# zkonduit/ezkl

Hardware: AMD Instinct MI355X
Metric: BN254 G1 MSM pts/s (2^20 points per GPU; NTT 2^22 elems/s in extra) (higher is better)
Workload: dtype u32x8 (254-bit modular integer, Montgomery); 1 GPU; configs[1]: standalone 2^20-point BN254 G1 MSM (uniform scalars, try-and-increment bases) + 2^22 scalar-field NTT per GPU; parallelism=points sharded across 1 rank(s); all_gather of 64-B partials + host fold

## Files before the change

### ezkl_amd/csrc/curve29.hpp

```cpp
#pragma once
#include "curve.hpp"
#include "field29.hpp"

namespace ezkl {

struct alignas(16) g1x29_t {
    f29_t x, y, zz, zzz;
};
struct g1a29_t {
    f29_t x, y;
};

EZ_D bool g1x29_is_id(const g1x29_t& p) { return Fq29::limbs_zero(p.zz); }
EZ_D g1x29_t g1x29_identity() {
    g1x29_t r;
    r.x = Fq29::zero(); r.y = Fq29::zero(); r.zz = Fq29::zero(); r.zzz = Fq29::zero();
    return r;
}
EZ_D g1a29_t g1a29_unpack(const g1a_t& p) {
    g1a29_t r;
    r.x = Fq29::unpack(p.x);
    r.y = Fq29::unpack(p.y);
    return r;
}
EZ_D bool g1a29_is_id(const g1a29_t& p) {
    uint32_t o = 0;
#pragma unroll
    for (int i = 0; i < 9; i++) o |= p.x.v[i] | p.y.v[i];
    return o == 0;
}

EZ_D g1x29_t g1x29_add_tail(const f29_t& u1, const f29_t& s1, const f29_t& p, const f29_t& r, const f29_t& zz, const f29_t& zzz) {
    g1x29_t o;
    const f29_t pp = Fq29::sqr(p);
    o.zz = Fq29::mul(zz, pp);
    const f29_t ppp = Fq29::mul(p, pp);
    o.zzz = Fq29::mul(zzz, ppp);
    const f29_t q = Fq29::mul(u1, pp);
#if !EZKL_FUSED_Y
    const f29_t e = Fq29::mul(s1, ppp);
#endif
    const f29_t rr = Fq29::sqr(r);
    const f29_t nq = Fq29::neg<1>(q);
    o.x = Fq29::normalize(Fq29::add(Fq29::add(rr, Fq29::neg<1>(ppp)), Fq29::add(nq, nq)));
    const f29_t d = Fq29::sub<3>(q, o.x);
#if EZKL_FUSED_Y
    o.y = Fq29::mul2add(r, d, Fq29::neg<3>(s1), ppp);
#else
    const f29_t rd = Fq29::mul(r, d);
    o.y = Fq29::normalize(Fq29::sub<1>(rd, e));
#endif
    return o;
}
EZ_D g1x29_t g1x29_double_affine(const g1a29_t& p) {
    const f29_t u = Fq29::add(p.y, p.y);
    const f29_t v = Fq29::sqr_cold(u);
    const f29_t w = Fq29::mul_cold(u, v);
    const f29_t s = Fq29::mul_cold(p.x, v);
    const f29_t xx = Fq29::sqr_cold(p.x);
    const f29_t m = Fq29::normalize(Fq29::add(Fq29::add(xx, xx), xx));
    const f29_t ns = Fq29::neg<1>(s);
    g1x29_t r;
    r.x = Fq29::normalize(Fq29::add(Fq29::sqr_cold(m), Fq29::add(ns, ns)));
    const f29_t d = Fq29::sub<3>(s, r.x);
    r.y = Fq29::normalize(Fq29::sub<1>(Fq29::mul_cold(m, d), Fq29::mul_cold(w, p.y)));
    r.zz = v;
    r.zzz = w;
    return r;
}
EZ_D g1x29_t g1x29_double(const g1x29_t& p) {
    if (g1x29_is_id(p)) return p;
    const f29_t u = Fq29::add(p.y, p.y);
    const f29_t v = Fq29::sqr_cold(u);
    const f29_t w = Fq29::mul_cold(u, v);
    const f29_t s = Fq29::mul_cold(p.x, v);
    const f29_t xx = Fq29::sqr_cold(p.x);
    const f29_t m = Fq29::normalize(Fq29::add(Fq29::add(xx, xx), xx));
    const f29_t ns = Fq29::neg<1>(s);
    g1x29_t r;
    r.x = Fq29::normalize(Fq29::add(Fq29::sqr_cold(m), Fq29::add(ns, ns)));
    const f29_t d = Fq29::sub<3>(s, r.x);
    r.y = Fq29::normalize(Fq29::sub<1>(Fq29::mul_cold(m, d), Fq29::mul_cold(w, p.y)));
    r.zz = Fq29::mul_cold(v, p.zz);
    r.zzz = Fq29::mul_cold(w, p.zzz);
    return r;
}
EZ_D g1x29_t g1x29_add_mixed(const g1x29_t& a, const g1a29_t& q, bool negate) {
    if (g1a29_is_id(q)) return a;
    const f29_t qy = negate ? Fq29::neg<0>(q.y) : q.y;
    if (g1x29_is_id(a)) {
        g1x29_t r;
        r.x = q.x;
        r.y = negate ? Fq29::normalize(qy) : q.y;
        r.zz = Fq29::one();
        r.zzz = Fq29::one();
        return r;
    }
    const f29_t u2 = Fq29::mul(q.x, a.zz);
    const f29_t s2 = Fq29::mul(qy, a.zzz);
    const f29_t p = Fq29::normalize(Fq29::sub<3>(u2, a.x));
    const f29_t r = Fq29::normalize(Fq29::sub<3>(s2, a.y));
    if (Fq29::is_zero_mod_p(p)) {
        if (Fq29::is_zero_mod_p(r)) {
            g1a29_t qq = q;
            if (negate) qq.y = Fq29::normalize(qy);
            return g1x29_double_affine(qq);
        }
        return g1x29_identity();
    }
    return g1x29_add_tail(a.x, a.y, p, r, a.zz, a.zzz);
}
EZ_D g1x29_t g1x29_add(const g1x29_t& a, const g1x29_t& b) {
    if (g1x29_is_id(a)) return b;
    if (g1x29_is_id(b)) return a;
    const f29_t u1 = Fq29::mul(a.x, b.zz), u2 = Fq29::mul(b.x, a.zz);
    const f29_t s1 = Fq29::mul(a.y, b.zzz), s2 = Fq29::mul(b.y, a.zzz);
    const f29_t p = Fq29::normalize(Fq29::sub<1>(u2, u1));
    const f29_t r = Fq29::normalize(Fq29::sub<1>(s2, s1));
    if (Fq29::is_zero_mod_p(p)) {
        if (Fq29::is_zero_mod_p(r)) return g1x29_double(a);
        return g1x29_identity();
    }
    return g1x29_add_tail(u1, s1, p, r, Fq29::mul(a.zz, b.zz), Fq29::mul(a.zzz, b.zzz));
}

EZ_D g1x29_t ld_g1x29(const g1x29_t* p) {
    g1x29_t r;
    const uint4* s = reinterpret_cast<const uint4*>(p);
    uint32_t* d = r.x.v;
#pragma unroll
    for (int k = 0; k < 9; k++) {
        const uint4 t = s[k];
        d[4 * k] = t.x; d[4 * k + 1] = t.y; d[4 * k + 2] = t.z; d[4 * k + 3] = t.w;
    }
    return r;
}
EZ_D void st_g1x29(g1x29_t* p, const g1x29_t& v) {
    uint4* d = reinterpret_cast<uint4*>(p);
    const uint32_t* s = v.x.v;
#pragma unroll
    for (int k = 0; k < 9; k++) d[k] = make_uint4(s[4 * k], s[4 * k + 1], s[4 * k + 2], s[4 * k + 3]);
}
EZ_D g1x29_t g1x29_shfl_xor(const g1x29_t& p, uint32_t mask) {
    g1x29_t r;
    const uint32_t* s = p.x.v;
    uint32_t* d = r.x.v;
#pragma unroll
    for (int k = 0; k < 36; k++) d[k] = __shfl_xor(s[k], mask);
    return r;
}
EZ_D g1x29_t g1x29_group_sum(g1x29_t acc, uint32_t width) {
#pragma unroll 1
    for (uint32_t s = width >> 1; s > 0; s >>= 1) acc = g1x29_add(acc, g1x29_shfl_xor(acc, s));
    return acc;
}

template <int S>
EZ_D f29_t f29_quad_bcast(const f29_t& x) {
    f29_t t = x, r;
    asm volatile("s_nop 1" : "+v"(t.v[0]), "+v"(t.v[1]), "+v"(t.v[2]), "+v"(t.v[3]), "+v"(t.v[4]), "+v"(t.v[5]), "+v"(t.v[6]), "+v"(t.v[7]), "+v"(t.v[8]));
#pragma unroll
    for (int i = 0; i < 9; i++) {
        r.v[i] = (uint32_t)__builtin_amdgcn_mov_dpp((int)t.v[i], S * 0x55, 0xf, 0xf, true);
        asm volatile("" : "+v"(r.v[i]));
    }
    return r;
}
EZ_D f29_t f29_sel(bool c, const f29_t& a, const f29_t& b) {
    f29_t r;
#pragma unroll
    for (int i = 0; i < 9; i++) r.v[i] = c ? a.v[i] : b.v[i];
    return r;
}
EZ_D f29_t f29_sel4(uint32_t q, const f29_t& x0, const f29_t& x1, const f29_t& x2, const f29_t& x3) {
    return f29_sel(q < 2, f29_sel(q == 0, x0, x1), f29_sel(q == 2, x2, x3));
}
template <int S>
EZ_D g1x29_t g1x29_quad_bcast(const g1x29_t& p) {
    g1x29_t r;
    r.x = f29_quad_bcast<S>(p.x); r.y = f29_quad_bcast<S>(p.y); r.zz = f29_quad_bcast<S>(p.zz); r.zzz = f29_quad_bcast<S>(p.zzz);
    return r;
}
EZ_D g1x29_t g1x29_add_quad(const g1x29_t& a, const g1x29_t& b, bool& special, uint32_t* dbg = nullptr) {
    const uint32_t q = threadIdx.x & 3u;
    g1x29_t o = a;
    special = __any(g1x29_is_id(a) || g1x29_is_id(b)) != 0;
    if (special) return o;
    const f29_t m1 = Fq29::mul(f29_sel4(q, a.x, b.x, a.y, b.y), f29_sel4(q, b.zz, a.zz, b.zzz, a.zzz));
    const f29_t u1 = f29_quad_bcast<0>(m1), s1 = f29_quad_bcast<2>(m1);
    const f29_t p = Fq29::normalize(Fq29::sub<1>(f29_quad_bcast<1>(m1), u1));
    const f29_t r = Fq29::normalize(Fq29::sub<1>(f29_quad_bcast<3>(m1), s1));
    special = __any(Fq29::is_zero_mod_p(p)) != 0;
    if (special) return o;
    const f29_t m2 = Fq29::mul(f29_sel4(q, a.zz, a.zzz, p, r), f29_sel4(q, b.zz, b.zzz, p, r));
    const f29_t pp = f29_quad_bcast<2>(m2), rr = f29_quad_bcast<3>(m2);
    const f29_t m3 = Fq29::mul(f29_sel(q == 1, p, f29_sel(q == 2, u1, m2)), pp);
    const f29_t ppp = f29_quad_bcast<1>(m3), qq = f29_quad_bcast<2>(m3);
    const f29_t nq = Fq29::neg<1>(qq);
    o.x = Fq29::normalize(Fq29::add(Fq29::add(rr, Fq29::neg<1>(ppp)), Fq29::add(nq, nq)));
    const f29_t d = Fq29::sub<3>(qq, o.x);
    const f29_t m4 = Fq29::mul(f29_sel(q == 2, r, f29_sel(q == 3, s1, m2)), f29_sel(q == 2, d, ppp));
    o.zz = f29_quad_bcast<0>(m3);
    o.zzz = f29_quad_bcast<1>(m4);
    o.y = Fq29::normalize(Fq29::sub<1>(f29_quad_bcast<2>(m4), f29_quad_bcast<3>(m4)));
    if (dbg) {
        const f29_t* t[14] = {&m1, &u1, &s1, &p, &r, &m2, &pp, &rr, &m3, &ppp, &qq, &o.x, &d, &m4};
        for (int k = 0; k < 14; k++)
            for (int i = 0; i < 9; i++) dbg[9 * k + i] = t[k]->v[i];
    }
    return o;
}
EZ_D g1x29_t g1x29_group_sum_coop(g1x29_t acc, uint32_t width) {
    const uint32_t nsteps = 3u + (31u - (uint32_t)__clz(width)) - 2u;
    g1x29_t t0 = acc;
#pragma unroll 1
    for (uint32_t k = 0; k < nsteps; k++) {
        g1x29_t a, b;
        if (k == 0) { a = g1x29_quad_bcast<0>(acc); b = g1x29_quad_bcast<1>(acc); }
        else if (k == 1) { a = g1x29_quad_bcast<2>(acc); b = g1x29_quad_bcast<3>(acc); }
        else if (k == 2) { a = t0; b = acc; }
        else { a = acc; b = g1x29_shfl_xor(acc, 4u << (k - 3u)); }
        bool special;
        g1x29_t r = g1x29_add_quad(a, b, special);
        if (special) r = g1x29_add(a, b);
        if (k == 0) t0 = r; else acc = r;
    }
    return acc;
}
EZ_D g1x29_t g1x29_block256_sum(g1x29_t acc, uint4* sh) {
    acc = g1x29_group_sum(acc, 64);
    if ((threadIdx.x & 63) == 0) {
        const uint32_t* s = acc.x.v;
#pragma unroll
        for (int k = 0; k < 9; k++) sh[k * 4 + (threadIdx.x >> 6)] = make_uint4(s[4 * k], s[4 * k + 1], s[4 * k + 2], s[4 * k + 3]);
    }
    __syncthreads();
    {
        uint32_t* d = acc.x.v;
#pragma unroll
        for (int k = 0; k < 9; k++) {
            const uint4 t = sh[k * 4 + (threadIdx.x & 3)];
            d[4 * k] = t.x; d[4 * k + 1] = t.y; d[4 * k + 2] = t.z; d[4 * k + 3] = t.w;
        }
    }
    __syncthreads();
    return g1x29_group_sum(acc, 4);
}
EZ_D g1x29_t g1x29_block256_sum_coop(const g1x29_t& acc0, uint4* sh) {
    g1x29_t acc = g1x29_group_sum_coop(acc0, 64);
    if ((threadIdx.x & 63) == 0) {
        const uint32_t* s = acc.x.v;
#pragma unroll
        for (int k = 0; k < 9; k++) sh[k * 4 + (threadIdx.x >> 6)] = make_uint4(s[4 * k], s[4 * k + 1], s[4 * k + 2], s[4 * k + 3]);
    }
    __syncthreads();
    {
        uint32_t* d = acc.x.v;
#pragma unroll
        for (int k = 0; k < 9; k++) {
            const uint4 t = sh[k * 4 + (threadIdx.x & 3)];
            d[4 * k] = t.x; d[4 * k + 1] = t.y; d[4 * k + 2] = t.z; d[4 * k + 3] = t.w;
        }
    }
// ... 27 lines not shown
```

### ezkl_amd/csrc/field29.hpp

```cpp
#pragma once
#include "field.hpp"
#include "montmul29_gen.hpp"

#ifndef EZKL_FQ29_ILP
#define EZKL_FQ29_ILP 0
#endif
#ifndef EZKL_FUSED_Y
#define EZKL_FUSED_Y 1
#endif
namespace ezkl {

struct f29_t {
    uint32_t v[9];
};
static constexpr uint32_t M29 = (1u << 29) - 1;

template <class CT, bool IS_FQ>
struct Field29 {
    typedef CT C;
    typedef uint32_t u32x9 __attribute__((ext_vector_type(9)));
    EZ_D static void mul_asm(const uint32_t (&a)[9], const uint32_t (&b)[9], uint32_t (&r)[9]) {
        if (IS_FQ) {
#if EZKL_FQ29_ILP
            mont_mul29i_fq(a, b, r);
#else
            mont_mul29_fq(a, b, r);
#endif
        } else mont_mul29_fr(a, b, r);
    }

    EZ_D static f29_t zero() {
        f29_t r;
#pragma unroll
        for (int i = 0; i < 9; i++) r.v[i] = 0;
        return r;
    }
    EZ_D static f29_t one() {
        f29_t r;
#pragma unroll
        for (int i = 0; i < 9; i++) r.v[i] = C::ONE[i];
        return r;
    }
    EZ_D static bool limbs_zero(const f29_t& a) {
        uint32_t o = 0;
#pragma unroll
        for (int i = 0; i < 9; i++) o |= a.v[i];
        return o == 0;
    }
    __device__ __attribute__((noinline)) static u32x9 mul_call(u32x9 a, u32x9 b) {
        uint32_t x[9], y[9], r[9];
#pragma unroll
        for (int i = 0; i < 9; i++) { x[i] = a[i]; y[i] = b[i]; }
        mul_asm(x, y, r);
        u32x9 o;
#pragma unroll
        for (int i = 0; i < 9; i++) o[i] = r[i];
        return o;
    }
    EZ_D static f29_t mul(const f29_t& a, const f29_t& b) {
        f29_t r;
        mul_asm(a.v, b.v, r.v);
        return r;
    }
    EZ_D static f29_t mul2add(const f29_t& a, const f29_t& b, const f29_t& c, const f29_t& d) {
        static_assert(IS_FQ, "generated for Fq only");
        f29_t r;
        mont_mul2add29_fq(a.v, b.v, c.v, d.v, r.v);
        return r;
    }
    EZ_D static f29_t mul_cold(const f29_t& a, const f29_t& b) {
        u32x9 x, y;
#pragma unroll
        for (int i = 0; i < 9; i++) { x[i] = a.v[i]; y[i] = b.v[i]; }
        u32x9 o = mul_call(x, y);
        f29_t r;
#pragma unroll
        for (int i = 0; i < 9; i++) r.v[i] = o[i];
        return r;
    }
    EZ_D static f29_t sqr(const f29_t& a) {
        f29_t r;
        if (IS_FQ) {
#if EZKL_FQ29_ILP
            mont_sqr29i_fq(a.v, r.v);
#else
            mont_sqr29_fq(a.v, r.v);
#endif
        } else mont_sqr29_fr(a.v, r.v);
        return r;
    }
    EZ_D static f29_t sqr_cold(const f29_t& a) { return mul_cold(a, a); }
    EZ_D static f29_t add(const f29_t& a, const f29_t& b) {
        f29_t r;
#pragma unroll
        for (int i = 0; i < 9; i++) r.v[i] = a.v[i] + b.v[i];
        return r;
    }
    template <int KI>
    EZ_D static f29_t sub(const f29_t& a, const f29_t& b) {
        f29_t r;
#pragma unroll
        for (int i = 0; i < 9; i++) r.v[i] = a.v[i] + (C::SUBC[KI][i] - b.v[i]);
        return r;
    }
    template <int KI>
    EZ_D static f29_t neg(const f29_t& b) {
        f29_t r;
#pragma unroll
        for (int i = 0; i < 9; i++) r.v[i] = C::SUBC[KI][i] - b.v[i];
        return r;
    }
    EZ_D static f29_t normalize(const f29_t& a) {
        f29_t r = a;
#pragma unroll
        for (int i = 0; i < 8; i++) {
            r.v[i + 1] += r.v[i] >> 29;
            r.v[i] &= M29;
        }
        return r;
    }
    EZ_D static bool is_zero_mod_p(const f29_t& a) {
        const uint32_t j = (a.v[0] * C::P0INV) & M29;
        if (j >= 32) return false;
        uint32_t carry = 0, diff = 0;
#pragma unroll
        for (int i = 0; i < 9; i++) {
            const uint64_t t = (uint64_t)j * C::P[i] + carry;
            const uint32_t limb = i < 8 ? ((uint32_t)t & M29) : (uint32_t)t;
            carry = i < 8 ? (uint32_t)(t >> 29) : 0;
            diff |= limb ^ a.v[i];
        }
        return diff == 0;
    }
    template <int KI>
    EZ_D static f29_t cond_sub(const f29_t& x) {
        f29_t t;
#pragma unroll
        for (int i = 0; i < 9; i++) t.v[i] = x.v[i] + C::CSUB[KI][i];
        t = normalize(t);
        const bool ge = (t.v[8] >> 29) != 0;
        t.v[8] &= M29;
        f29_t r;
#pragma unroll
        for (int i = 0; i < 9; i++) r.v[i] = ge ? t.v[i] : x.v[i];
        return r;
    }
    EZ_D static f29_t canonical(const f29_t& x) {
        constexpr uint32_t D = (uint32_t)(C::P[8] + 1u);
        constexpr uint64_t MAGIC = (((uint64_t)1 << 51) + D - 1) / D;
        const uint32_t q = (uint32_t)(((uint64_t)x.v[8] * MAGIC) >> 51);
        f29_t r;
        uint64_t acc = 0;
#pragma unroll
        for (int i = 0; i < 9; i++) {
            acc += (uint64_t)q * C::CSUB[0][i] + x.v[i];
            r.v[i] = (uint32_t)acc & M29;
            acc >>= 29;
        }
        return cond_sub<0>(r);
    }
    EZ_D static fe_t pack(const f29_t& a) {
        fe_t w;
#pragma unroll
        for (int j = 0; j < 8; j++) {
            const int bit = 32 * j, lo = bit / 29, sh = bit - 29 * lo;
            uint32_t acc = a.v[lo] >> sh;
            const int have = 29 - sh;
            if (lo + 1 < 9) acc |= a.v[lo + 1] << have;
            if (have + 29 < 32 && lo + 2 < 9) acc |= a.v[lo + 2] << (have + 29);
            w.v[j] = acc;
        }
        return w;
    }
    EZ_D static f29_t unpack(const fe_t& w) {
        f29_t r;
#pragma unroll
        for (int i = 0; i < 8; i++) {
            const int bit = 29 * i, word = bit >> 5, sh = bit & 31;
            const uint32_t lo = w.v[word], hi = word + 1 < 8 ? w.v[word + 1] : 0u;
            r.v[i] = (sh ? __builtin_amdgcn_alignbit(hi, lo, sh) : lo) & M29;
        }
        r.v[8] = w.v[7] >> 8;
        return r;
    }
};

typedef Field29<Fq29C, true> Fq29;
typedef Field29<Fr29C, false> Fr29;

EZ_D f29_t ld_f29(const f29_t* p) {
    f29_t r;
#pragma unroll
    for (int i = 0; i < 9; i++) r.v[i] = p->v[i];
    return r;
}
EZ_D void st_f29(f29_t* p, const f29_t& a) {
#pragma unroll
    for (int i = 0; i < 9; i++) p->v[i] = a.v[i];
}

}
```

### ezkl_amd/csrc/montmul29_gen.hpp

```cpp
#pragma once
#ifndef __HIPCC_RTC__
#include <stdint.h>
#endif
namespace ezkl {
struct Fq29C {
    static constexpr uint32_t P[9] = {0x187cfd47u, 0x010460b6u, 0x1c72a34fu, 0x02d522d0u, 0x1585d978u, 0x02db40c0u, 0x00a6e141u, 0x0e5c2634u, 0x0030644eu};
    static constexpr uint32_t ONE[9] = {0x157ccc21u, 0x141c2758u, 0x185230d3u, 0x014c0419u, 0x0aa36fb9u, 0x1d4240ceu, 0x11d54c07u, 0x052ac7a8u, 0x000dc836u};
    static constexpr uint32_t P0INV = 0x1b799c77u;
    static constexpr uint32_t SUBC[7][9] = {
        {0x30f9fa8eu, 0x2208c16cu, 0x38e5469du, 0x25aa45a0u, 0x2b0bb2efu, 0x25b68180u, 0x214dc281u, 0x3cb84c67u, 0x0060c89bu},
        {0x21f3f51cu, 0x241182dau, 0x31ca8d3bu, 0x2b548b42u, 0x361765dfu, 0x2b6d0301u, 0x229b8503u, 0x397098cfu, 0x00c19138u},
        {0x23e7ea38u, 0x282305b5u, 0x23951a77u, 0x36a91686u, 0x2c2ecbbfu, 0x36da0604u, 0x25370a07u, 0x32e1319fu, 0x01832272u},
        {0x27cfd470u, 0x30460b6bu, 0x272a34efu, 0x2d522d0du, 0x385d9780u, 0x2db40c09u, 0x2a6e1410u, 0x25c2633fu, 0x030644e6u},
        {0x2f9fa8e0u, 0x208c16d7u, 0x2e5469e0u, 0x3aa45a1bu, 0x30bb2f01u, 0x3b681814u, 0x34dc2821u, 0x2b84c67fu, 0x060c89cdu},
        {0x3f3f51c0u, 0x21182dafu, 0x3ca8d3c1u, 0x3548b437u, 0x21765e04u, 0x36d0302au, 0x29b85044u, 0x37098d00u, 0x0c19139bu},
        {0x3e7ea380u, 0x22305b60u, 0x3951a783u, 0x2a916870u, 0x22ecbc0au, 0x2da06055u, 0x3370a08au, 0x2e131a01u, 0x18322738u},
    };
    static constexpr uint32_t CSUB[4][9] = {
        {0x078302b9u, 0x1efb9f49u, 0x038d5cb0u, 0x1d2add2fu, 0x0a7a2687u, 0x1d24bf3fu, 0x1f591ebeu, 0x11a3d9cbu, 0x1fcf9bb1u},
        {0x0f060572u, 0x1df73e92u, 0x071ab961u, 0x1a55ba5eu, 0x14f44d0fu, 0x1a497e7eu, 0x1eb23d7du, 0x0347b397u, 0x1f9f3763u},
        {0x1e0c0ae4u, 0x1bee7d24u, 0x0e3572c3u, 0x14ab74bcu, 0x09e89a1fu, 0x1492fcfdu, 0x1d647afbu, 0x068f672fu, 0x1f3e6ec6u},
        {0x1c1815c8u, 0x17dcfa49u, 0x1c6ae587u, 0x0956e978u, 0x13d1343fu, 0x0925f9fau, 0x1ac8f5f7u, 0x0d1ece5fu, 0x1e7cdd8cu},
    };
    static constexpr uint32_t R261_32[8] = {0x157ccc21u, 0x4e8384ebu, 0x0ce148c3u, 0xfb90a602u, 0x819caa36u, 0x5301fa84u, 0x563d4475u, 0x0dc83629u};
};
struct Fr29C {
    static constexpr uint32_t P[9] = {0x10000001u, 0x1f0fac9fu, 0x0e5c2450u, 0x07d090f3u, 0x1585d283u, 0x02db40c0u, 0x00a6e141u, 0x0e5c2634u, 0x0030644eu};
    static constexpr uint32_t ONE[9] = {0x0fffff57u, 0x1ea70ab4u, 0x052c068bu, 0x17504f49u, 0x0aa8075bu, 0x1d4240ceu, 0x11d54c07u, 0x052ac7a8u, 0x000dc836u};
    static constexpr uint32_t P0INV = 0x10000001u;
    static constexpr uint32_t SUBC[7][9] = {
        {0x20000002u, 0x3e1f593eu, 0x3cb848a0u, 0x2fa121e5u, 0x2b0ba505u, 0x25b68180u, 0x214dc281u, 0x3cb84c67u, 0x0060c89bu},
        {0x20000004u, 0x3c3eb27du, 0x39709142u, 0x3f4243ccu, 0x36174a0bu, 0x2b6d0301u, 0x229b8503u, 0x397098cfu, 0x00c19138u},
        {0x20000008u, 0x387d64fbu, 0x32e12286u, 0x3e84879au, 0x2c2e9418u, 0x36da0604u, 0x25370a07u, 0x32e1319fu, 0x01832272u},
        {0x20000010u, 0x30fac9f7u, 0x25c2450eu, 0x3d090f36u, 0x385d2832u, 0x2db40c09u, 0x2a6e1410u, 0x25c2633fu, 0x030644e6u},
        {0x20000020u, 0x21f593efu, 0x2b848a1eu, 0x3a121e6du, 0x30ba5066u, 0x3b681814u, 0x34dc2821u, 0x2b84c67fu, 0x060c89cdu},
        {0x20000040u, 0x23eb27dfu, 0x3709143du, 0x34243cdbu, 0x2174a0ceu, 0x36d0302au, 0x29b85044u, 0x37098d00u, 0x0c19139bu},
        {0x20000080u, 0x27d64fbfu, 0x2e12287bu, 0x284879b8u, 0x22e9419eu, 0x2da06055u, 0x3370a08au, 0x2e131a01u, 0x18322738u},
    };
    static constexpr uint32_t CSUB[4][9] = {
        {0x0fffffffu, 0x00f05360u, 0x11a3dbafu, 0x182f6f0cu, 0x0a7a2d7cu, 0x1d24bf3fu, 0x1f591ebeu, 0x11a3d9cbu, 0x1fcf9bb1u},
        {0x1ffffffeu, 0x01e0a6c0u, 0x0347b75eu, 0x105ede19u, 0x14f45af9u, 0x1a497e7eu, 0x1eb23d7du, 0x0347b397u, 0x1f9f3763u},
        {0x1ffffffcu, 0x03c14d81u, 0x068f6ebcu, 0x00bdbc32u, 0x09e8b5f3u, 0x1492fcfdu, 0x1d647afbu, 0x068f672fu, 0x1f3e6ec6u},
        {0x1ffffff8u, 0x07829b03u, 0x0d1edd78u, 0x017b7864u, 0x13d16be6u, 0x0925f9fau, 0x1ac8f5f7u, 0x0d1ece5fu, 0x1e7cdd8cu},
    };
    static constexpr uint32_t R261_32[8] = {0x8fffff57u, 0x2fd4e156u, 0xa494b01au, 0x75bba827u, 0x819caa80u, 0x5301fa84u, 0x563d4475u, 0x0dc83629u};
};
__device__ __forceinline__ void mont_mul29_fq(const uint32_t (&a)[9], const uint32_t (&b)[9], uint32_t (&r)[9]) {
    asm("s_mov_b32 s16, 0x187cfd47\n\t"
        "s_mov_b32 s17, 0x010460b6\n\t"
        "s_mov_b32 s18, 0x1c72a34f\n\t"
        "s_mov_b32 s19, 0x02d522d0\n\t"
        "s_mov_b32 s20, 0x1585d978\n\t"
        "s_mov_b32 s21, 0x02db40c0\n\t"
        "s_mov_b32 s22, 0x00a6e141\n\t"
        "s_mov_b32 s23, 0x0e5c2634\n\t"
        "s_mov_b32 s24, 0x0030644e\n\t"
        "s_mov_b32 s25, 0x04866389\n\t"
        "s_mov_b32 s26, 0x1fffffff\n\t"
        "v_mad_u64_u32 v[16:17], vcc, %[a0], %[b0], 0\n\t"
        "v_mul_lo_u32 %[r0], v16, s25\n\t"
        "v_and_b32 %[r0], s26, %[r0]\n\t"
        "v_mad_u64_u32 v[16:17], vcc, %[r0], s16, v[16:17]\n\t"
        "v_lshrrev_b64 v[16:17], 29, v[16:17]\n\t"
        "v_mad_u64_u32 v[16:17], vcc, %[a0], %[b1], v[16:17]\n\t"
        "v_mad_u64_u32 v[16:17], vcc, %[a1], %[b0], v[16:17]\n\t"
        "v_mad_u64_u32 v[16:17], vcc, %[r0], s17, v[16:17]\n\t"
        "v_mul_lo_u32 %[r1], v16, s25\n\t"
        "v_and_b32 %[r1], s26, %[r1]\n\t"
        "v_mad_u64_u32 v[16:17], vcc, %[r1], s16, v[16:17]\n\t"
        "v_lshrrev_b64 v[16:17], 29, v[16:17]\n\t"
        "v_mad_u64_u32 v[16:17], vcc, %[a0], %[b2], v[16:17]\n\t"
        "v_mad_u64_u32 v[16:17], vcc, %[a1], %[b1], v[16:17]\n\t"
        "v_mad_u64_u32 v[16:17], vcc, %[a2], %[b0], v[16:17]\n\t"
        "v_mad_u64_u32 v[16:17], vcc, %[r0], s18, v[16:17]\n\t"
        "v_mad_u64_u32 v[16:17], vcc, %[r1], s17, v[16:17]\n\t"
        "v_mul_lo_u32 %[r2], v16, s25\n\t"
        "v_and_b32 %[r2], s26, %[r2]\n\t"
        "v_mad_u64_u32 v[16:17], vcc, %[r2], s16, v[16:17]\n\t"
        "v_lshrrev_b64 v[16:17], 29, v[16:17]\n\t"
        "v_mad_u64_u32 v[16:17], vcc, %[a0], %[b3], v[16:17]\n\t"
        "v_mad_u64_u32 v[16:17], vcc, %[a1], %[b2], v[16:17]\n\t"
        "v_mad_u64_u32 v[16:17], vcc, %[a2], %[b1], v[16:17]\n\t"
        "v_mad_u64_u32 v[16:17], vcc, %[a3], %[b0], v[16:17]\n\t"
        "v_mad_u64_u32 v[16:17], vcc, %[r0], s19, v[16:17]\n\t"
        "v_mad_u64_u32 v[16:17], vcc, %[r1], s18, v[16:17]\n\t"
        "v_mad_u64_u32 v[16:17], vcc, %[r2], s17, v[16:17]\n\t"
        "v_mul_lo_u32 %[r3], v16, s25\n\t"
        "v_and_b32 %[r3], s26, %[r3]\n\t"
        "v_mad_u64_u32 v[16:17], vcc, %[r3], s16, v[16:17]\n\t"
        "v_lshrrev_b64 v[16:17], 29, v[16:17]\n\t"
        "v_mad_u64_u32 v[16:17], vcc, %[a0], %[b4], v[16:17]\n\t"
        "v_mad_u64_u32 v[16:17], vcc, %[a1], %[b3], v[16:17]\n\t"
        "v_mad_u64_u32 v[16:17], vcc, %[a2], %[b2], v[16:17]\n\t"
        "v_mad_u64_u32 v[16:17], vcc, %[a3], %[b1], v[16:17]\n\t"
        "v_mad_u64_u32 v[16:17], vcc, %[a4], %[b0], v[16:17]\n\t"
        "v_mad_u64_u32 v[16:17], vcc, %[r0], s20, v[16:17]\n\t"
        "v_mad_u64_u32 v[16:17], vcc, %[r1], s19, v[16:17]\n\t"
        "v_mad_u64_u32 v[16:17], vcc, %[r2], s18, v[16:17]\n\t"
        "v_mad_u64_u32 v[16:17], vcc, %[r3], s17, v[16:17]\n\t"
        "v_mul_lo_u32 %[r4], v16, s25\n\t"
        "v_and_b32 %[r4], s26, %[r4]\n\t"
        "v_mad_u64_u32 v[16:17], vcc, %[r4], s16, v[16:17]\n\t"
        "v_lshrrev_b64 v[16:17], 29, v[16:17]\n\t"
        "v_mad_u64_u32 v[16:17], vcc, %[a0], %[b5], v[16:17]\n\t"
        "v_mad_u64_u32 v[16:17], vcc, %[a1], %[b4], v[16:17]\n\t"
        "v_mad_u64_u32 v[16:17], vcc, %[a2], %[b3], v[16:17]\n\t"
        "v_mad_u64_u32 v[16:17], vcc, %[a3], %[b2], v[16:17]\n\t"
        "v_mad_u64_u32 v[16:17], vcc, %[a4], %[b1], v[16:17]\n\t"
        "v_mad_u64_u32 v[16:17], vcc, %[a5], %[b0], v[16:17]\n\t"
        "v_mad_u64_u32 v[16:17], vcc, %[r0], s21, v[16:17]\n\t"
        "v_mad_u64_u32 v[16:17], vcc, %[r1], s20, v[16:17]\n\t"
        "v_mad_u64_u32 v[16:17], vcc, %[r2], s19, v[16:17]\n\t"
        "v_mad_u64_u32 v[16:17], vcc, %[r3], s18, v[16:17]\n\t"
        "v_mad_u64_u32 v[16:17], vcc, %[r4], s17, v[16:17]\n\t"
        "v_mul_lo_u32 %[r5], v16, s25\n\t"
        "v_and_b32 %[r5], s26, %[r5]\n\t"
        "v_mad_u64_u32 v[16:17], vcc, %[r5], s16, v[16:17]\n\t"
        "v_lshrrev_b64 v[16:17], 29, v[16:17]\n\t"
        "v_mad_u64_u32 v[16:17], vcc, %[a0], %[b6], v[16:17]\n\t"
        "v_mad_u64_u32 v[16:17], vcc, %[a1], %[b5], v[16:17]\n\t"
        "v_mad_u64_u32 v[16:17], vcc, %[a2], %[b4], v[16:17]\n\t"
        "v_mad_u64_u32 v[16:17], vcc, %[a3], %[b3], v[16:17]\n\t"
        "v_mad_u64_u32 v[16:17], vcc, %[a4], %[b2], v[16:17]\n\t"
        "v_mad_u64_u32 v[16:17], vcc, %[a5], %[b1], v[16:17]\n\t"
        "v_mad_u64_u32 v[16:17], vcc, %[a6], %[b0], v[16:17]\n\t"
        "v_mad_u64_u32 v[16:17], vcc, %[r0], s22, v[16:17]\n\t"
        "v_mad_u64_u32 v[16:17], vcc, %[r1], s21, v[16:17]\n\t"
        "v_mad_u64_u32 v[16:17], vcc, %[r2], s20, v[16:17]\n\t"
        "v_mad_u64_u32 v[16:17], vcc, %[r3], s19, v[16:17]\n\t"
        "v_mad_u64_u32 v[16:17], vcc, %[r4], s18, v[16:17]\n\t"
        "v_mad_u64_u32 v[16:17], vcc, %[r5], s17, v[16:17]\n\t"
        "v_mul_lo_u32 %[r6], v16, s25\n\t"
        "v_and_b32 %[r6], s26, %[r6]\n\t"
        "v_mad_u64_u32 v[16:17], vcc, %[r6], s16, v[16:17]\n\t"
        "v_lshrrev_b64 v[16:17], 29, v[16:17]\n\t"
        "v_mad_u64_u32 v[16:17], vcc, %[a0], %[b7], v[16:17]\n\t"
        "v_mad_u64_u32 v[16:17], vcc, %[a1], %[b6], v[16:17]\n\t"
        "v_mad_u64_u32 v[16:17], vcc, %[a2], %[b5], v[16:17]\n\t"
        "v_mad_u64_u32 v[16:17], vcc, %[a3], %[b4], v[16:17]\n\t"
        "v_mad_u64_u32 v[16:17], vcc, %[a4], %[b3], v[16:17]\n\t"
        "v_mad_u64_u32 v[16:17], vcc, %[a5], %[b2], v[16:17]\n\t"
        "v_mad_u64_u32 v[16:17], vcc, %[a6], %[b1], v[16:17]\n\t"
        "v_mad_u64_u32 v[16:17], vcc, %[a7], %[b0], v[16:17]\n\t"
        "v_mad_u64_u32 v[16:17], vcc, %[r0], s23, v[16:17]\n\t"
        "v_mad_u64_u32 v[16:17], vcc, %[r1], s22, v[16:17]\n\t"
        "v_mad_u64_u32 v[16:17], vcc, %[r2], s21, v[16:17]\n\t"
        "v_mad_u64_u32 v[16:17], vcc, %[r3], s20, v[16:17]\n\t"
        "v_mad_u64_u32 v[16:17], vcc, %[r4], s19, v[16:17]\n\t"
        "v_mad_u64_u32 v[16:17], vcc, %[r5], s18, v[16:17]\n\t"
        "v_mad_u64_u32 v[16:17], vcc, %[r6], s17, v[16:17]\n\t"
        "v_mul_lo_u32 %[r7], v16, s25\n\t"
        "v_and_b32 %[r7], s26, %[r7]\n\t"
        "v_mad_u64_u32 v[16:17], vcc, %[r7], s16, v[16:17]\n\t"
        "v_lshrrev_b64 v[16:17], 29, v[16:17]\n\t"
        "v_mad_u64_u32 v[16:17], vcc, %[a0], %[b8], v[16:17]\n\t"
        "v_mad_u64_u32 v[16:17], vcc, %[a1], %[b7], v[16:17]\n\t"
        "v_mad_u64_u32 v[16:17], vcc, %[a2], %[b6], v[16:17]\n\t"
        "v_mad_u64_u32 v[16:17], vcc, %[a3], %[b5], v[16:17]\n\t"
        "v_mad_u64_u32 v[16:17], vcc, %[a4], %[b4], v[16:17]\n\t"
        "v_mad_u64_u32 v[16:17], vcc, %[a5], %[b3], v[16:17]\n\t"
        "v_mad_u64_u32 v[16:17], vcc, %[a6], %[b2], v[16:17]\n\t"
        "v_mad_u64_u32 v[16:17], vcc, %[a7], %[b1], v[16:17]\n\t"
        "v_mad_u64_u32 v[16:17], vcc, %[a8], %[b0], v[16:17]\n\t"
        "v_mad_u64_u32 v[16:17], vcc, %[r0], s24, v[16:17]\n\t"
        "v_mad_u64_u32 v[16:17], vcc, %[r1], s23, v[16:17]\n\t"
        "v_mad_u64_u32 v[16:17], vcc, %[r2], s22, v[16:17]\n\t"
        "v_mad_u64_u32 v[16:17], vcc, %[r3], s21, v[16:17]\n\t"
        "v_mad_u64_u32 v[16:17], vcc, %[r4], s20, v[16:17]\n\t"
        "v_mad_u64_u32 v[16:17], vcc, %[r5], s19, v[16:17]\n\t"
        "v_mad_u64_u32 v[16:17], vcc, %[r6], s18, v[16:17]\n\t"
        "v_mad_u64_u32 v[16:17], vcc, %[r7], s17, v[16:17]\n\t"
        "v_mul_lo_u32 %[r8], v16, s25\n\t"
        "v_and_b32 %[r8], s26, %[r8]\n\t"
        "v_mad_u64_u32 v[16:17], vcc, %[r8], s16, v[16:17]\n\t"
        "v_lshrrev_b64 v[16:17], 29, v[16:17]\n\t"
        "v_mad_u64_u32 v[16:17], vcc, %[a1], %[b8], v[16:17]\n\t"
        "v_mad_u64_u32 v[16:17], vcc, %[a2], %[b7], v[16:17]\n\t"
        "v_mad_u64_u32 v[16:17], vcc, %[a3], %[b6], v[16:17]\n\t"
        "v_mad_u64_u32 v[16:17], vcc, %[a4], %[b5], v[16:17]\n\t"
        "v_mad_u64_u32 v[16:17], vcc, %[a5], %[b4], v[16:17]\n\t"
        "v_mad_u64_u32 v[16:17], vcc, %[a6], %[b3], v[16:17]\n\t"
        "v_mad_u64_u32 v[16:17], vcc, %[a7], %[b2], v[16:17]\n\t"
        "v_mad_u64_u32 v[16:17], vcc, %[a8], %[b1], v[16:17]\n\t"
        "v_mad_u64_u32 v[16:17], vcc, %[r1], s24, v[16:17]\n\t"
        "v_mad_u64_u32 v[16:17], vcc, %[r2], s23, v[16:17]\n\t"
        "v_mad_u64_u32 v[16:17], vcc, %[r3], s22, v[16:17]\n\t"
        "v_mad_u64_u32 v[16:17], vcc, %[r4], s21, v[16:17]\n\t"
        "v_mad_u64_u32 v[16:17], vcc, %[r5], s20, v[16:17]\n\t"
        "v_mad_u64_u32 v[16:17], vcc, %[r6], s19, v[16:17]\n\t"
        "v_mad_u64_u32 v[16:17], vcc, %[r7], s18, v[16:17]\n\t"
        "v_mad_u64_u32 v[16:17], vcc, %[r8], s17, v[16:17]\n\t"
// ... 1532 lines not shown
        "v_mad_u64_u32 v[18:19], vcc, %[a0], %[b7], 0\n\t"
        "v_mad_u64_u32 v[16:17], vcc, %[r0], s22, v[16:17]\n\t"
        "v_mad_u64_u32 v[18:19], vcc, %[a1], %[b6], v[18:19]\n\t"
        "v_mad_u64_u32 v[16:17], vcc, %[r1], s21, v[16:17]\n\t"
        "v_mad_u64_u32 v[18:19], vcc, %[a2], %[b5], v[18:19]\n\t"
        "v_mad_u64_u32 v[16:17], vcc, %[r2], s20, v[16:17]\n\t"
        "v_mad_u64_u32 v[18:19], vcc, %[a3], %[b4], v[18:19]\n\t"
        "v_mad_u64_u32 v[16:17], vcc, %[r3], s19, v[16:17]\n\t"
        "v_mad_u64_u32 v[18:19], vcc, %[a4], %[b3], v[18:19]\n\t"
        "v_mad_u64_u32 v[16:17], vcc, %[r4], s18, v[16:17]\n\t"
        "v_mad_u64_u32 v[18:19], vcc, %[a5], %[b2], v[18:19]\n\t"
        "v_mad_u64_u32 v[16:17], vcc, %[r5], s17, v[16:17]\n\t"
        "v_mad_u64_u32 v[18:19], vcc, %[a6], %[b1], v[18:19]\n\t"
        "v_mul_lo_u32 %[r6], v16, s25\n\t"
        "v_mad_u64_u32 v[18:19], vcc, %[a7], %[b0], v[18:19]\n\t"
        "v_and_b32 %[r6], s26, %[r6]\n\t"
        "v_mad_u64_u32 v[16:17], vcc, %[r6], s16, v[16:17]\n\t"
        "v_lshrrev_b64 v[16:17], 29, v[16:17]\n\t"
        "v_lshl_add_u64 v[16:17], v[18:19], 0, v[16:17]\n\t"
        "v_mad_u64_u32 v[18:19], vcc, %[a0], %[b8], 0\n\t"
        "v_mad_u64_u32 v[16:17], vcc, %[r0], s23, v[16:17]\n\t"
        "v_mad_u64_u32 v[18:19], vcc, %[a1], %[b7], v[18:19]\n\t"
        "v_mad_u64_u32 v[16:17], vcc, %[r1], s22, v[16:17]\n\t"
        "v_mad_u64_u32 v[18:19], vcc, %[a2], %[b6], v[18:19]\n\t"
        "v_mad_u64_u32 v[16:17], vcc, %[r2], s21, v[16:17]\n\t"
        "v_mad_u64_u32 v[18:19], vcc, %[a3], %[b5], v[18:19]\n\t"
        "v_mad_u64_u32 v[16:17], vcc, %[r3], s20, v[16:17]\n\t"
        "v_mad_u64_u32 v[18:19], vcc, %[a4], %[b4], v[18:19]\n\t"
        "v_mad_u64_u32 v[16:17], vcc, %[r4], s19, v[16:17]\n\t"
        "v_mad_u64_u32 v[18:19], vcc, %[a5], %[b3], v[18:19]\n\t"
        "v_mad_u64_u32 v[16:17], vcc, %[r5], s18, v[16:17]\n\t"
        "v_mad_u64_u32 v[18:19], vcc, %[a6], %[b2], v[18:19]\n\t"
        "v_mad_u64_u32 v[16:17], vcc, %[r6], s17, v[16:17]\n\t"
        "v_mad_u64_u32 v[18:19], vcc, %[a7], %[b1], v[18:19]\n\t"
        "v_mul_lo_u32 %[r7], v16, s25\n\t"
        "v_mad_u64_u32 v[18:19], vcc, %[a8], %[b0], v[18:19]\n\t"
        "v_and_b32 %[r7], s26, %[r7]\n\t"
        "v_mad_u64_u32 v[16:17], vcc, %[r7], s16, v[16:17]\n\t"
        "v_lshrrev_b64 v[16:17], 29, v[16:17]\n\t"
        "v_lshl_add_u64 v[16:17], v[18:19], 0, v[16:17]\n\t"
        "v_mad_u64_u32 v[18:19], vcc, %[a1], %[b8], 0\n\t"
        "v_mad_u64_u32 v[16:17], vcc, %[r0], s24, v[16:17]\n\t"
        "v_mad_u64_u32 v[18:19], vcc, %[a2], %[b7], v[18:19]\n\t"
        "v_mad_u64_u32 v[16:17], vcc, %[r1], s23, v[16:17]\n\t"
        "v_mad_u64_u32 v[18:19], vcc, %[a3], %[b6], v[18:19]\n\t"
        "v_mad_u64_u32 v[16:17], vcc, %[r2], s22, v[16:17]\n\t"
        "v_mad_u64_u32 v[18:19], vcc, %[a4], %[b5], v[18:19]\n\t"
        "v_mad_u64_u32 v[16:17], vcc, %[r3], s21, v[16:17]\n\t"
        "v_mad_u64_u32 v[18:19], vcc, %[a5], %[b4], v[18:19]\n\t"
        "v_mad_u64_u32 v[16:17], vcc, %[r4], s20, v[16:17]\n\t"
        "v_mad_u64_u32 v[18:19], vcc, %[a6], %[b3], v[18:19]\n\t"
        "v_mad_u64_u32 v[16:17], vcc, %[r5], s19, v[16:17]\n\t"
        "v_mad_u64_u32 v[18:19], vcc, %[a7], %[b2], v[18:19]\n\t"
        "v_mad_u64_u32 v[16:17], vcc, %[r6], s18, v[16:17]\n\t"
        "v_mad_u64_u32 v[18:19], vcc, %[a8], %[b1], v[18:19]\n\t"
        "v_mad_u64_u32 v[16:17], vcc, %[r7], s17, v[16:17]\n\t"
        "v_mul_lo_u32 %[r8], v16, s25\n\t"
        "v_and_b32 %[r8], s26, %[r8]\n\t"
        "v_mad_u64_u32 v[16:17], vcc, %[r8], s16, v[16:17]\n\t"
        "v_lshrrev_b64 v[16:17], 29, v[16:17]\n\t"
        "v_lshl_add_u64 v[16:17], v[18:19], 0, v[16:17]\n\t"
        "v_mad_u64_u32 v[18:19], vcc, %[a2], %[b8], 0\n\t"
        "v_mad_u64_u32 v[16:17], vcc, %[r1], s24, v[16:17]\n\t"
        "v_mad_u64_u32 v[18:19], vcc, %[a3], %[b7], v[18:19]\n\t"
        "v_mad_u64_u32 v[16:17], vcc, %[r2], s23, v[16:17]\n\t"
        "v_mad_u64_u32 v[18:19], vcc, %[a4], %[b6], v[18:19]\n\t"
        "v_mad_u64_u32 v[16:17], vcc, %[r3], s22, v[16:17]\n\t"
        "v_mad_u64_u32 v[18:19], vcc, %[a5], %[b5], v[18:19]\n\t"
        "v_mad_u64_u32 v[16:17], vcc, %[r4], s21, v[16:17]\n\t"
        "v_mad_u64_u32 v[18:19], vcc, %[a6], %[b4], v[18:19]\n\t"
        "v_mad_u64_u32 v[16:17], vcc, %[r5], s20, v[16:17]\n\t"
        "v_mad_u64_u32 v[18:19], vcc, %[a7], %[b3], v[18:19]\n\t"
        "v_mad_u64_u32 v[16:17], vcc, %[r6], s19, v[16:17]\n\t"
        "v_mad_u64_u32 v[18:19], vcc, %[a8], %[b2], v[18:19]\n\t"
        "v_mad_u64_u32 v[16:17], vcc, %[r7], s18, v[16:17]\n\t"
        "v_mad_u64_u32 v[16:17], vcc, %[r8], s17, v[16:17]\n\t"
        "v_and_b32 %[r0], s26, v16\n\t"
        "v_lshrrev_b64 v[16:17], 29, v[16:17]\n\t"
        "v_lshl_add_u64 v[16:17], v[18:19], 0, v[16:17]\n\t"
        "v_mad_u64_u32 v[18:19], vcc, %[a3], %[b8], 0\n\t"
        "v_mad_u64_u32 v[16:17], vcc, %[r2], s24, v[16:17]\n\t"
        "v_mad_u64_u32 v[18:19], vcc, %[a4], %[b7], v[18:19]\n\t"
        "v_mad_u64_u32 v[16:17], vcc, %[r3], s23, v[16:17]\n\t"
        "v_mad_u64_u32 v[18:19], vcc, %[a5], %[b6], v[18:19]\n\t"
        "v_mad_u64_u32 v[16:17], vcc, %[r4], s22, v[16:17]\n\t"
        "v_mad_u64_u32 v[18:19], vcc, %[a6], %[b5], v[18:19]\n\t"
        "v_mad_u64_u32 v[16:17], vcc, %[r5], s21, v[16:17]\n\t"
        "v_mad_u64_u32 v[18:19], vcc, %[a7], %[b4], v[18:19]\n\t"
        "v_mad_u64_u32 v[16:17], vcc, %[r6], s20, v[16:17]\n\t"
        "v_mad_u64_u32 v[18:19], vcc, %[a8], %[b3], v[18:19]\n\t"
        "v_mad_u64_u32 v[16:17], vcc, %[r7], s19, v[16:17]\n\t"
        "v_mad_u64_u32 v[16:17], vcc, %[r8], s18, v[16:17]\n\t"
        "v_and_b32 %[r1], s26, v16\n\t"
        "v_lshrrev_b64 v[16:17], 29, v[16:17]\n\t"
        "v_lshl_add_u64 v[16:17], v[18:19], 0, v[16:17]\n\t"
        "v_mad_u64_u32 v[18:19], vcc, %[a4], %[b8], 0\n\t"
        "v_mad_u64_u32 v[16:17], vcc, %[r3], s24, v[16:17]\n\t"
        "v_mad_u64_u32 v[18:19], vcc, %[a5], %[b7], v[18:19]\n\t"
        "v_mad_u64_u32 v[16:17], vcc, %[r4], s23, v[16:17]\n\t"
        "v_mad_u64_u32 v[18:19], vcc, %[a6], %[b6], v[18:19]\n\t"
        "v_mad_u64_u32 v[16:17], vcc, %[r5], s22, v[16:17]\n\t"
        "v_mad_u64_u32 v[18:19], vcc, %[a7], %[b5], v[18:19]\n\t"
        "v_mad_u64_u32 v[16:17], vcc, %[r6], s21, v[16:17]\n\t"
        "v_mad_u64_u32 v[18:19], vcc, %[a8], %[b4], v[18:19]\n\t"
        "v_mad_u64_u32 v[16:17], vcc, %[r7], s20, v[16:17]\n\t"
        "v_mad_u64_u32 v[16:17], vcc, %[r8], s19, v[16:17]\n\t"
        "v_and_b32 %[r2], s26, v16\n\t"
        "v_lshrrev_b64 v[16:17], 29, v[16:17]\n\t"
        "v_lshl_add_u64 v[16:17], v[18:19], 0, v[16:17]\n\t"
        "v_mad_u64_u32 v[18:19], vcc, %[a5], %[b8], 0\n\t"
        "v_mad_u64_u32 v[16:17], vcc, %[r4], s24, v[16:17]\n\t"
        "v_mad_u64_u32 v[18:19], vcc, %[a6], %[b7], v[18:19]\n\t"
        "v_mad_u64_u32 v[16:17], vcc, %[r5], s23, v[16:17]\n\t"
        "v_mad_u64_u32 v[18:19], vcc, %[a7], %[b6], v[18:19]\n\t"
        "v_mad_u64_u32 v[16:17], vcc, %[r6], s22, v[16:17]\n\t"
        "v_mad_u64_u32 v[18:19], vcc, %[a8], %[b5], v[18:19]\n\t"
        "v_mad_u64_u32 v[16:17], vcc, %[r7], s21, v[16:17]\n\t"
        "v_mad_u64_u32 v[16:17], vcc, %[r8], s20, v[16:17]\n\t"
        "v_and_b32 %[r3], s26, v16\n\t"
        "v_lshrrev_b64 v[16:17], 29, v[16:17]\n\t"
        "v_lshl_add_u64 v[16:17], v[18:19], 0, v[16:17]\n\t"
        "v_mad_u64_u32 v[18:19], vcc, %[a6], %[b8], 0\n\t"
        "v_mad_u64_u32 v[16:17], vcc, %[r5], s24, v[16:17]\n\t"
        "v_mad_u64_u32 v[18:19], vcc, %[a7], %[b7], v[18:19]\n\t"
        "v_mad_u64_u32 v[16:17], vcc, %[r6], s23, v[16:17]\n\t"
        "v_mad_u64_u32 v[18:19], vcc, %[a8], %[b6], v[18:19]\n\t"
        "v_mad_u64_u32 v[16:17], vcc, %[r7], s22, v[16:17]\n\t"
        "v_mad_u64_u32 v[16:17], vcc, %[r8], s21, v[16:17]\n\t"
        "v_and_b32 %[r4], s26, v16\n\t"
        "v_lshrrev_b64 v[16:17], 29, v[16:17]\n\t"
        "v_lshl_add_u64 v[16:17], v[18:19], 0, v[16:17]\n\t"
        "v_mad_u64_u32 v[18:19], vcc, %[a7], %[b8], 0\n\t"
        "v_mad_u64_u32 v[16:17], vcc, %[r6], s24, v[16:17]\n\t"
        "v_mad_u64_u32 v[18:19], vcc, %[a8], %[b7], v[18:19]\n\t"
        "v_mad_u64_u32 v[16:17], vcc, %[r7], s23, v[16:17]\n\t"
        "v_mad_u64_u32 v[16:17], vcc, %[r8], s22, v[16:17]\n\t"
        "v_and_b32 %[r5], s26, v16\n\t"
        "v_lshrrev_b64 v[16:17], 29, v[16:17]\n\t"
        "v_lshl_add_u64 v[16:17], v[18:19], 0, v[16:17]\n\t"
        "v_mad_u64_u32 v[18:19], vcc, %[a8], %[b8], 0\n\t"
        "v_mad_u64_u32 v[16:17], vcc, %[r7], s24, v[16:17]\n\t"
        "v_mad_u64_u32 v[16:17], vcc, %[r8], s23, v[16:17]\n\t"
        "v_and_b32 %[r6], s26, v16\n\t"
        "v_lshrrev_b64 v[16:17], 29, v[16:17]\n\t"
        "v_lshl_add_u64 v[16:17], v[18:19], 0, v[16:17]\n\t"
        "v_mad_u64_u32 v[16:17], vcc, %[r8], s24, v[16:17]\n\t"
        "v_and_b32 %[r7], s26, v16\n\t"
        "v_lshrrev_b64 v[16:17], 29, v[16:17]\n\t"
        "v_mov_b32 %[r8], v16\n\t"
        : [r0] "=&v"(r[0]), [r1] "=&v"(r[1]), [r2] "=&v"(r[2]), [r3] "=&v"(r[3]), [r4] "=&v"(r[4]), [r5] "=&v"(r[5]), [r6] "=&v"(r[6]), [r7] "=&v"(r[7]), [r8] "=&v"(r[8])
        : [a0] "v"(a[0]), [a1] "v"(a[1]), [a2] "v"(a[2]), [a3] "v"(a[3]), [a4] "v"(a[4]), [a5] "v"(a[5]), [a6] "v"(a[6]), [a7] "v"(a[7]), [a8] "v"(a[8]), [b0] "v"(b[0]), [b1] "v"(b[1]), [b2] "v"(b[2]), [b3] "v"(b[3]), [b4] "v"(b[4]), [b5] "v"(b[5]), [b6] "v"(b[6]), [b7] "v"(b[7]), [b8] "v"(b[8])
        : "v16", "v17", "v18", "v19", "s16", "s17", "s18", "s19", "s20", "s21", "s22", "s23", "s24", "s25", "s26", "vcc");
}
}
```

### ezkl_amd/csrc/msm.hip

```cpp
#include "common.hpp"
#include <deque>
#include <thread>
#include <chrono>
#include "curve.hpp"
#include "curve29.hpp"
#include "host64.hpp"
#include <string.h>

namespace ezkl {

static constexpr uint32_t MSM_MAX_PART_BITS = 12;
static constexpr uint32_t MSM_SPAN_HEAVY = 16;
static constexpr uint32_t MSM_PART_STAGE = 13312;
static constexpr uint32_t MSM_BINSORT_STAGE = 15360;
static constexpr uint32_t MSM_HEAVY_CHUNK = 256;
static constexpr uint32_t MSM_DIGIT_E = 8;
static constexpr uint32_t MSM_LMIN = 8;
static constexpr uint32_t MSM_MAX_BIG = 64;
static constexpr uint32_t MSM_BIG_BLOCKS = 64;
static constexpr uint32_t MSM_BIG_ROWS = 8;

__device__ __forceinline__ uint32_t msm_part_of(uint32_t bucket, uint32_t NP) { return bucket ? 1u + (bucket & (NP - 1u)) : 0u; }
__device__ __forceinline__ uint32_t msm_lane_len(const uint32_t* offsets, uint32_t nb, uint32_t nlanes, uint32_t lmin) {
    const uint32_t l = (uint32_t)(((uint64_t)offsets[nb] + nlanes - 1) / nlanes);
// ... 387 lines not shown
    uint32_t total;
    uint32_t run = msm_block_scan(s, tsum, total) - s;
#pragma unroll
    for (int q = 0; q < 4; q++) {
        uint32_t j = t * 4 + q;
        if (j < nbins) {
            cnt[j] = run;
            if (emit) {
                const bool b0 = (p == 0 && j == 0);
                offsets[(size_t)p * nbins + j] = b0 ? part_base[0] : beg + run;
                if (b0 ? part_base[1] == part_base[0] : loc[q] == 0) st_f29(&buckets[(size_t)p * nbins + j].zz, Fq29::zero());
            }
        }
        run += loc[q];
    }
    __syncthreads();
}
__device__ __forceinline__ void msm_bigsort_count_body(const uint2* entries, const uint32_t* part_base, uint32_t LB, const uint32_t* big_list,
                                                       const uint32_t* big_count, uint32_t* bin_total, uint32_t* block_off, uint32_t* cnt, uint32_t bx,
                                                       uint32_t by, uint32_t rows);
__global__ __launch_bounds__(512) void msm_binsort_kernel(const uint2* entries, const uint32_t* part_base, uint32_t LB, uint32_t NP,
                                                          const uint32_t* big_flag, uint32_t* offsets, uint32_t* vals, g1x29_t* buckets,
                                                          const uint32_t* big_list, const uint32_t* big_count, uint32_t* bin_total, uint32_t* block_off,
                                                          size_t bstride) {
    BOFF(); BSH(entries); BSH(part_base); BSH(big_flag); BSH(offsets); BSH(vals); BSH(buckets);
    __shared__ uint32_t cnt[2048];
    __shared__ uint32_t tsum[512];
    extern __shared__ uint32_t stage[];
    if (blockIdx.x >= NP) {
        BSH(big_list); BSH(big_count); BSH(bin_total); BSH(block_off);
        const uint32_t w = blockIdx.x - NP;
        msm_bigsort_count_body(entries, part_base, LB, big_list, big_count, bin_total, block_off, cnt, w % MSM_BIG_BLOCKS, w / MSM_BIG_BLOCKS, MSM_BIG_ROWS);
        return;
    }
    const uint32_t p = blockIdx.x, t = threadIdx.x, nbins = 1u << LB;
    const uint32_t beg = part_base[p + 1], end = part_base[p + 2];
    if (p == NP - 1 && t == 0) offsets[(size_t)NP * nbins] = end;
    if (big_flag[p]) return;
    const bool staged = (end - beg) <= MSM_BINSORT_STAGE;
    for (uint32_t j = t; j < nbins; j += 512) cnt[j] = 0;
    __syncthreads();
    if (staged) {
        constexpr int PER = MSM_BINSORT_STAGE / 512;
        uint2 v[PER];
#pragma unroll
        for (int q = 0; q < PER; q++) {
            const uint32_t e = beg + t + (uint32_t)q * 512u;
            v[q] = e < end ? entries[e] : make_uint2(0u, 0xffffffffu);
        }
#pragma unroll
        for (int q = 0; q < PER; q++)
            if (v[q].y != 0xffffffffu) atomicAdd(&cnt[v[q].y], 1u);
        __syncthreads();
        msm_bins_scan(cnt, tsum, nbins, p, beg, part_base, true, offsets, buckets);
#pragma unroll
        for (int q = 0; q < PER; q++)
            if (v[q].y != 0xffffffffu) stage[atomicAdd(&cnt[v[q].y], 1u)] = v[q].x;
        __syncthreads();
        for (uint32_t i = t; i < end - beg; i += 512) vals[beg + i] = stage[i];
    } else {
        for (uint32_t e = beg + t; e < end; e += 512) (void)msm_wave_rank(cnt, entries[e].y);
        __syncthreads();
        msm_bins_scan(cnt, tsum, nbins, p, beg, part_base, true, offsets, buckets);
        for (uint32_t e = beg + t; e < end; e += 512) {
            const uint2 v = entries[e];
            vals[beg + msm_wave_rank(cnt, v.y)] = v.x;
        }
    }
}
__device__ __forceinline__ void msm_big_slice(uint32_t beg, uint32_t end, uint32_t& s0, uint32_t& s1, uint32_t bx) {
    const uint32_t chunk = (end - beg + MSM_BIG_BLOCKS - 1) / MSM_BIG_BLOCKS;
    s0 = beg + bx * chunk;
    s1 = s0 + chunk < end ? s0 + chunk : end;
    if (s0 > end) s0 = end;
}
__device__ __forceinline__ void msm_bigsort_count_body(const uint2* entries, const uint32_t* part_base, uint32_t LB, const uint32_t* big_list,
                                                       const uint32_t* big_count, uint32_t* bin_total, uint32_t* block_off, uint32_t* cnt, uint32_t bx,
                                                       uint32_t by, uint32_t rows) {
    const uint32_t t = threadIdx.x, nbins = 1u << LB;
    const uint32_t nbig = big_count[0] < MSM_MAX_BIG ? big_count[0] : MSM_MAX_BIG;
    for (uint32_t y = by; y < nbig; y += rows) {
        const uint32_t p = big_list[y];
        uint32_t s0, s1;
        msm_big_slice(part_base[p + 1], part_base[p + 2], s0, s1, bx);
        for (uint32_t j = t; j < nbins; j += 512) cnt[j] = 0;
        __syncthreads();
        for (uint32_t e = s0 + t; e < s1; e += 512) (void)msm_wave_rank(cnt, entries[e].y);
        __syncthreads();
        for (uint32_t j = t; j < nbins; j += 512)
            block_off[((size_t)y * MSM_BIG_BLOCKS + bx) * nbins + j] = cnt[j] ? atomicAdd(&bin_total[(size_t)y * nbins + j], cnt[j]) : 0u;
        __syncthreads();
    }
}
__global__ __launch_bounds__(512) void msm_bigsort_scatter_kernel(const uint2* entries, const uint32_t* part_base, uint32_t LB, const uint32_t* big_list,
                                                                  const uint32_t* big_count, const uint32_t* bin_total, const uint32_t* block_off,
                                                                  uint32_t* offsets, uint32_t* vals, g1x29_t* buckets, size_t bstride) {
    BOFF(); BSH(entries); BSH(part_base); BSH(big_list); BSH(big_count); BSH(bin_total); BSH(block_off); BSH(offsets); BSH(vals); BSH(buckets);
    __shared__ uint32_t cnt[2048];
    __shared__ uint32_t tsum[512];
    const uint32_t t = threadIdx.x, nbins = 1u << LB;
    const uint32_t nbig = big_count[0] < MSM_MAX_BIG ? big_count[0] : MSM_MAX_BIG;
    for (uint32_t y = blockIdx.y; y < nbig; y += gridDim.y) {
        const uint32_t p = big_list[y], beg = part_base[p + 1];
        uint32_t s0, s1;
        msm_big_slice(beg, part_base[p + 2], s0, s1, blockIdx.x);
        for (uint32_t j = t; j < nbins; j += 512) cnt[j] = bin_total[(size_t)y * nbins + j];
        __syncthreads();
        msm_bins_scan(cnt, tsum, nbins, p, beg, part_base, blockIdx.x == 0, offsets, buckets);
        const uint32_t* mine = block_off + ((size_t)y * MSM_BIG_BLOCKS + blockIdx.x) * nbins;
        for (uint32_t j = t; j < nbins; j += 512) cnt[j] += mine[j];
        __syncthreads();
        for (uint32_t e = s0 + t; e < s1; e += 512) {
            const uint2 v = entries[e];
            vals[beg + msm_wave_rank(cnt, v.y)] = v.x;
        }
        __syncthreads();
    }
}

struct MsmRec {
    g1a_t p;
    bool neg;
};
__device__ __forceinline__ MsmRec msm_fetch(const g1a_t* tab, uint32_t v) {
    MsmRec r;
    r.p = ld_g1a(tab + (v & 0x7fffffffu));
    r.neg = (v >> 31) != 0;
    return r;
}
__global__ __launch_bounds__(256, 3) void msm_accumulate_kernel(const g1a_t* tab, const uint32_t* offsets, const uint32_t* vals,
                                                             uint32_t nb, uint32_t nlanes, g1x29_t* buckets, g1x29_t* head, g1x29_t* tail,
                                                             uint32_t* lane_first, uint32_t lmin, size_t bstride) {
    BOFF(); BSH(offsets); BSH(vals); BSH(buckets); BSH(head); BSH(tail); BSH(lane_first);
    const uint32_t t = blockIdx.x * blockDim.x + threadIdx.x;
    const uint32_t total = offsets[nb], L = msm_lane_len(offsets, nb, nlanes, lmin);
    const uint64_t k0w = (uint64_t)t * L;
    if (k0w >= total) return;
    const uint32_t k0 = (uint32_t)k0w;
    const uint32_t k1 = (uint64_t)k0 + L < total ? k0 + L : total;
    uint32_t lo = 0, hi = nb;
    while (hi - lo > 1) {
        uint32_t mid = (lo + hi) >> 1;
        if (offsets[mid] <= k0) lo = mid; else hi = mid;
    }
    uint32_t b = lo, bin_end = offsets[b + 1];
    uint32_t end_next = offsets[b + 2 <= nb ? b + 2 : nb];
    lane_first[t] = b;
    bool started_before = offsets[b] < k0;
    g1x29_t acc = g1x29_identity();
    MsmRec nxt = msm_fetch(tab, vals[k0]);
    uint32_t vn = k0 + 1 < k1 ? vals[k0 + 1] : 0u;
    for (uint32_t k = k0; k < k1; k++) {
        if (k == bin_end) {
            if (started_before) st_g1x29(head + t, acc); else st_g1x29(buckets + b, acc);
            acc.zz = Fq29::zero();
            started_before = false;
            b++;
            bin_end = end_next;
            if (bin_end == k) {
                uint32_t probes = 1;
                while (bin_end == k && probes < 4) { b++; bin_end = offsets[b + 1]; probes++; }
                if (bin_end == k) {
                    uint32_t lo2 = b + 1, hi2 = nb;
                    while (hi2 - lo2 > 1) {
                        uint32_t mid = (lo2 + hi2) >> 1;
                        if (offsets[mid] <= k) lo2 = mid; else hi2 = mid;
                    }
                    b = lo2;
                    bin_end = offsets[b + 1];
                }
            }
            end_next = offsets[b + 2 <= nb ? b + 2 : nb];
        }
        const MsmRec cur = nxt;
        nxt = msm_fetch(tab, vn);
        vn = k + 2 < k1 ? vals[k + 2] : 0u;
        acc = g1x29_add_mixed(acc, g1a29_unpack(cur.p), cur.neg);
    }
    if (k1 == bin_end) {
        if (started_before) st_g1x29(head + t, acc); else st_g1x29(buckets + b, acc);
    } else {
        if (started_before) st_g1x29(head + t, acc); else st_g1x29(tail + t, acc);
    }
}
EZ_D g1x29_t g1x29_shfl_down(const g1x29_t& p, uint32_t d) {
    g1x29_t r;
    const uint32_t* s = p.x.v;
    uint32_t* o = r.x.v;
#pragma unroll
    for (int k = 0; k < 36; k++) o[k] = __shfl_down(s[k], d);
    return r;
}
__global__ __launch_bounds__(256) void msm_fixup_boundary_tree_kernel(const uint32_t* offsets, uint32_t nb, uint32_t nlanes,
                                                                      const uint32_t* lane_first, const g1x29_t* head, const g1x29_t* tail, g1x29_t* buckets,
                                                                      uint32_t* heavy_list, uint32_t* heavy_count, uint32_t* chunk_list, uint32_t lmin,
                                                                      uint32_t span_heavy, size_t bstride) {
    BOFF(); BSH(offsets); BSH(lane_first); BSH(head); BSH(tail); BSH(buckets); BSH(heavy_list); BSH(heavy_count); BSH(chunk_list);
    const uint32_t t = blockIdx.x * blockDim.x + threadIdx.x + 1;
    const uint32_t lane = threadIdx.x & 63u;
    const uint32_t L = msm_lane_len(offsets, nb, nlanes, lmin);
    const uint64_t k0 = (uint64_t)t * L;
    bool cut = t < nlanes && k0 < offsets[nb];
    uint32_t b = 0, t1 = 0, t2 = 0;
    if (cut) {
        b = lane_first[t];
        const uint32_t beg = offsets[b], end = offsets[b + 1];
        cut = beg < k0;
        t1 = beg / L; t2 = (end - 1) / L;
    }
    if (cut && t2 - t1 > span_heavy) {
        if (t == t1 + 1 && t2 - t1 > MSM_HEAVY_CHUNK) heavy_list[atomicAdd(heavy_count, 1u)] = b;
        if ((t - t1 - 1) % MSM_HEAVY_CHUNK == 0) chunk_list[atomicAdd(heavy_count + 1, 1u)] = t;
        cut = false;
    }
    const uint32_t wave_last = t + (63u - lane);
    const uint32_t run = cut ? (t2 < wave_last ? t2 : wave_last) - t + 1u : 0u;
    uint32_t longest = run;
#pragma unroll
    for (uint32_t o = 32; o > 0; o >>= 1) {
        const uint32_t m = __shfl_xor(longest, o);
        longest = m > longest ? m : longest;
    }
    if (longest == 0) return;
    if (longest <= 2) {
        if (!cut || t != t1 + 1) return;
        g1x29_t acc = g1x29_add(ld_g1x29(tail + t1), ld_g1x29(head + t));
        for (uint32_t u = t + 1; u <= t2; u++) acc = g1x29_add(acc, ld_g1x29(head + u));
        st_g1x29(buckets + b, acc);
        return;
    }
    g1x29_t v = cut ? ld_g1x29(head + t) : g1x29_identity();
    uint32_t have = cut ? 1u : 0u;
#pragma unroll 1
    for (uint32_t d = 1; d < longest; d <<= 1) {
        const g1x29_t w = g1x29_shfl_down(v, d);
        const uint32_t hw = __shfl_down(have, d);
        if (have == d && run > d) {
            v = g1x29_add(v, w);
            have += hw;
        }
    }
    if (!cut || t != t1 + 1) return;
    g1x29_t acc = g1x29_add(ld_g1x29(tail + t1), v);
    for (uint32_t u = t + run; u <= t2; u++) acc = g1x29_add(acc, ld_g1x29(head + u));
    st_g1x29(buckets + b, acc);
}
__global__ __launch_bounds__(256) void msm_fixup_heavy1_kernel(const uint32_t* offsets, uint32_t nb, uint32_t nlanes, const uint32_t* lane_first, g1x29_t* head,
                                                               const g1x29_t* tail, g1x29_t* buckets, const uint32_t* chunk_list, const uint32_t* counts, uint32_t lmin,
                                                               uint32_t coop, size_t bstride) {
    BOFF(); BSH(offsets); BSH(lane_first); BSH(head); BSH(tail); BSH(buckets); BSH(chunk_list); BSH(counts);
    const uint32_t nchunks = counts[1], L = msm_lane_len(offsets, nb, nlanes, lmin);
    const uint32_t wave = threadIdx.x >> 6, lane = threadIdx.x & 63u;
    for (uint32_t ci = blockIdx.x * 4u + wave; ci < nchunks; ci += gridDim.x * 4u) {
        const uint32_t start = chunk_list[ci], b = lane_first[start];
        const uint32_t t2 = (offsets[b + 1] - 1) / L;
        const uint32_t stop = start + MSM_HEAVY_CHUNK - 1 < t2 ? start + MSM_HEAVY_CHUNK - 1 : t2;
        const uint32_t t1 = offsets[b] / L;
        const bool whole = t2 - t1 <= MSM_HEAVY_CHUNK;
        g1x29_t acc = (whole && lane == 63u) ? ld_g1x29(tail + t1) : g1x29_identity();
        for (uint32_t t = start + lane; t <= stop; t += 64) acc = g1x29_add(acc, ld_g1x29(head + t));
        acc = coop ? g1x29_group_sum_coop(acc, 64) : g1x29_group_sum(acc, 64);
        if (lane == 0) st_g1x29(whole ? buckets + b : head + start, acc);
    }
}
__global__ __launch_bounds__(256) void msm_fixup_heavy2_kernel(const uint32_t* offsets, uint32_t nb, uint32_t nlanes, const g1x29_t* head, const g1x29_t* tail,
                                                               const uint32_t* heavy_list, const uint32_t* counts, g1x29_t* buckets, uint32_t lmin, uint32_t coop, size_t bstride) {
    BOFF(); BSH(offsets); BSH(head); BSH(tail); BSH(heavy_list); BSH(counts); BSH(buckets);
    const uint32_t L = msm_lane_len(offsets, nb, nlanes, lmin);
    const uint32_t wave = threadIdx.x >> 6, lane = threadIdx.x & 63u;
    for (uint32_t h = blockIdx.x * 4u + wave; h < counts[0]; h += gridDim.x * 4u) {
        const uint32_t b = heavy_list[h];
        const uint32_t t1 = offsets[b] / L, t2 = (offsets[b + 1] - 1) / L;
        g1x29_t acc = lane == 63u ? ld_g1x29(tail + t1) : g1x29_identity();
        for (uint32_t t = t1 + 1 + lane * MSM_HEAVY_CHUNK; t <= t2; t += 64 * MSM_HEAVY_CHUNK) acc = g1x29_add(acc, ld_g1x29(head + t));
        acc = coop ? g1x29_group_sum_coop(acc, 64) : g1x29_group_sum(acc, 64);
        if (lane == 0) st_g1x29(buckets + b, acc);
    }
}

struct ReduceGeom {
    uint32_t wA, wB, wC;
    uint32_t wsA, wsB, wsC;
    uint32_t EA, GA, ET, GT;
};
__global__ __launch_bounds__(256, 2) void msm_reduce1_kernel(const g1x29_t* buckets, ReduceGeom g, g1x29_t* partA, g1x29_t* partT, size_t bstride) {
    BOFF(); BSH(buckets); BSH(partA); BSH(partT);
    const uint32_t idx = blockIdx.x * blockDim.x + threadIdx.x;
    g1x29_t acc = g1x29_identity();
    if (blockIdx.y == 0) {
        if (idx >= (g.GA << g.wA)) return;
        const uint32_t dA = idx & ((1u << g.wA) - 1u), grp = idx >> g.wA;
        for (uint32_t e = 0; e < g.EA; e++) acc = g1x29_add(acc, ld_g1x29(buckets + ((((size_t)grp * g.EA + e) << g.wA) | dA)));
        st_g1x29(partA + (size_t)dA * g.GA + grp, acc);
    } else {
        const uint32_t nT = 1u << (g.wB + g.wC);
        if (idx >= nT * g.GT) return;
        const uint32_t grp = idx % g.GT, t = idx / g.GT;
        for (uint32_t e = 0; e < g.ET; e++) acc = g1x29_add(acc, ld_g1x29(buckets + (((size_t)t << g.wA) | (e * g.GT + grp))));
        st_g1x29(partT + (size_t)t * g.GT + grp, acc);
    }
}
__global__ __launch_bounds__(64) void msm_reduce2_kernel(const g1x29_t* partA, const g1x29_t* partT, ReduceGeom g, g1x29_t* SA, g1x29_t* T, uint32_t lanesA,
                                                         uint32_t lanesT, uint32_t blocksA, uint32_t coop, size_t bstride) {
    BOFF(); BSH(partA); BSH(partT); BSH(SA); BSH(T);
    const bool isA = blockIdx.x < blocksA;
    const uint32_t lanes = isA ? lanesA : lanesT, per = 64 / lanes;
    const uint32_t o = (isA ? blockIdx.x : blockIdx.x - blocksA) * per + threadIdx.x / lanes, j = threadIdx.x % lanes;
    const uint32_t nout = isA ? (1u << g.wA) : (1u << (g.wB + g.wC)), G = isA ? g.GA : g.GT;
    g1x29_t acc = g1x29_identity();
    if (o < nout) {
        const g1x29_t* src = (isA ? partA : partT) + (size_t)o * G;
        for (uint32_t i = j; i < G; i += lanes) acc = g1x29_add(acc, ld_g1x29(src + i));
    }
    acc = (coop && lanes >= 4) ? g1x29_group_sum_coop(acc, lanes) : g1x29_group_sum(acc, lanes);
    if (j == 0 && o < nout) st_g1x29((isA ? SA : T) + o, acc);
}
__global__ __launch_bounds__(256) void msm_planes_kernel(const g1x29_t* SA, const g1x29_t* T, ReduceGeom g, g1x29_t* planes, g1x29_t* planes_host, uint32_t coop,
                                                         size_t bstride) {
    BOFF(); BSH(SA); BSH(T); BSH(planes);
    __shared__ uint4 sh[9 * 4];
    uint32_t id = blockIdx.x, field = 0, j = 0;
    if (id > 0) {
        id -= 1;
        if (id < g.wA) { field = 1; j = id; }
        else if (id < g.wA + g.wB) { field = 2; j = id - g.wA; }
        else { field = 3; j = id - g.wA - g.wB; }
    }
    const uint32_t nA = 1u << g.wA, nT = 1u << (g.wB + g.wC);
    g1x29_t acc = g1x29_identity();
    auto with_bit = [](uint32_t k, uint32_t bit) { return ((k >> bit) << (bit + 1)) | (1u << bit) | (k & ((1u << bit) - 1u)); };
// ... 798 lines not shown
```

### ezkl_amd/csrc/ubench.hip

```cpp
#include "common.hpp"
#include "curve.hpp"
#include "montmul29_gen.hpp"
#include "curve29.hpp"
#include "host64.hpp"
#include <string.h>
#include <vector>
#include <stdlib.h>

namespace ezkl {

template <int VARIANT>
__global__ __launch_bounds__(256) void ub_modmul_kernel(fe_t* io, int iters) {
    size_t i = (size_t)blockIdx.x * blockDim.x + threadIdx.x;
    fe_t a = ld_fe(io + i), b = a, c = Fr::add(a, a), d = c;
    b.v[0] ^= 5;  b = Fr::reduce_once(b);
    for (int k = 0; k < iters; k++) {
        if (VARIANT == 0) { a = Fr::mul(a, b); c = Fr::mul(c, d); b = Fr::mul(b, a); d = Fr::mul(d, c); }
        else if (VARIANT == 1) { a = Fr::mul_portable(a, b); c = Fr::mul_portable(c, d); b = Fr::mul_portable(b, a); d = Fr::mul_portable(d, c); }
        else { a = Fr::mul_inl(a, b); c = Fr::mul_inl(c, d); b = Fr::mul_inl(b, a); d = Fr::mul_inl(d, c); }
    }
    st_fe(io + i, Fr::add(Fr::add(a, b), Fr::add(c, d)));
}
__global__ __launch_bounds__(256) void ub_waveinv_kernel(fe_t* io, int iters) {
    size_t i = (size_t)blockIdx.x * blockDim.x + threadIdx.x;
// ... 26 lines not shown
        for (int q = 0; q < 8; q++) { before.v[q] = __shfl_up(pre.v[q], 1); after.v[q] = __shfl_down(suf.v[q], 1); }
        fe_t r = inv;
        if (lane > 0) r = Fr::mul(r, before);
        if (lane < 63) r = Fr::mul(r, after);
        x = Fr::add(r, x);
        if (Fr::is_zero(x)) x = Fr::one();
    }
    st_fe(io + i, x);
}
__global__ __launch_bounds__(256) void ub_addsub_kernel(fe_t* io, int iters) {
    size_t i = (size_t)blockIdx.x * blockDim.x + threadIdx.x;
    fe_t a = ld_fe(io + i), b = Fr::reduce_once(a), c = Fr::add(b, b), d = c;
    for (int k = 0; k < iters; k++) { b = Fr::add(b, c); c = Fr::sub(c, d); d = Fr::add(d, b); c = Fr::sub(c, b); }
    st_fe(io + i, Fr::add(Fr::add(a, b), Fr::add(c, d)));
}
__global__ __launch_bounds__(256) void ub_mad64_kernel(uint64_t* io, int iters) {
    size_t i = (size_t)blockIdx.x * blockDim.x + threadIdx.x;
    uint64_t x = io[i];
    uint64_t a0 = x, a1 = x + 1, a2 = x + 2, a3 = x + 3, a4 = x + 4, a5 = x + 5, a6 = x + 6, a7 = x + 7;
    uint32_t m = (uint32_t)x | 1u, q = (uint32_t)(x >> 32) | 3u;
    for (int k = 0; k < iters; k++) {
        a0 = mad_wide(m, (uint32_t)a0, a0); a1 = mad_wide(q, (uint32_t)a1, a1);
        a2 = mad_wide(m, (uint32_t)a2, a2); a3 = mad_wide(q, (uint32_t)a3, a3);
        a4 = mad_wide(m, (uint32_t)a4, a4); a5 = mad_wide(q, (uint32_t)a5, a5);
        a6 = mad_wide(m, (uint32_t)a6, a6); a7 = mad_wide(q, (uint32_t)a7, a7);
    }
    io[i] = a0 ^ a1 ^ a2 ^ a3 ^ a4 ^ a5 ^ a6 ^ a7;
}
__global__ __launch_bounds__(256) void ub_mullo_kernel(uint64_t* io, int iters) {
    size_t i = (size_t)blockIdx.x * blockDim.x + threadIdx.x;
    uint32_t x = (uint32_t)io[i];
    uint32_t a0 = x, a1 = x + 1, a2 = x + 2, a3 = x + 3, a4 = x + 4, a5 = x + 5, a6 = x + 6, a7 = x + 7, m = x | 1u;
    for (int k = 0; k < iters; k++) {
        asm volatile("v_mul_lo_u32 %0, %0, %8\n\tv_mul_lo_u32 %1, %1, %8\n\tv_mul_lo_u32 %2, %2, %8\n\tv_mul_lo_u32 %3, %3, %8\n\t"
                     "v_mul_lo_u32 %4, %4, %8\n\tv_mul_lo_u32 %5, %5, %8\n\tv_mul_lo_u32 %6, %6, %8\n\tv_mul_lo_u32 %7, %7, %8"
                     : "+v"(a0), "+v"(a1), "+v"(a2), "+v"(a3), "+v"(a4), "+v"(a5), "+v"(a6), "+v"(a7) : "v"(m));
    }
    io[i] = a0 ^ a1 ^ a2 ^ a3 ^ a4 ^ a5 ^ a6 ^ a7;
}
__global__ __launch_bounds__(256) void ub_dfma_kernel(double* io, int iters) {
    size_t i = (size_t)blockIdx.x * blockDim.x + threadIdx.x;
    double x = io[i];
    double a0 = x, a1 = x + 1, a2 = x + 2, a3 = x + 3, a4 = x + 4, a5 = x + 5, a6 = x + 6, a7 = x + 7;
    const double m = 1.0000001, q = 0.9999999;
    for (int k = 0; k < iters; k++) {
        a0 = __builtin_fma(a0, m, q); a1 = __builtin_fma(a1, q, m);
        a2 = __builtin_fma(a2, m, q); a3 = __builtin_fma(a3, q, m);
        a4 = __builtin_fma(a4, m, q); a5 = __builtin_fma(a5, q, m);
        a6 = __builtin_fma(a6, m, q); a7 = __builtin_fma(a7, q, m);
    }
    io[i] = a0 + a1 + a2 + a3 + a4 + a5 + a6 + a7;
}
__global__ __launch_bounds__(256) void ub_copy_kernel(const uint4* in, uint4* out, size_t n) {
    for (size_t i = (size_t)blockIdx.x * blockDim.x + threadIdx.x; i < n; i += (size_t)gridDim.x * blockDim.x) out[i] = in[i];
}

__global__ __launch_bounds__(256) void ub_gather_kernel(const uint4* table, uint32_t mask, uint4* out, int iters) {
    uint32_t tid = blockIdx.x * blockDim.x + threadIdx.x;
    uint32_t x = tid * 2654435761u + 12345u;
    uint4 acc = make_uint4(0, 0, 0, 0);
    for (int k = 0; k < iters; k++) {
        x ^= x << 13; x ^= x >> 17; x ^= x << 5;
        const uint4* p = table + (size_t)(x & mask) * 4;
        uint4 a = p[0], b = p[1], c = p[2], d = p[3];
        acc.x ^= a.x ^ b.y ^ c.z ^ d.w; acc.y += a.y + b.x; acc.z ^= c.x + d.y; acc.w += a.w ^ d.z;
    }
    out[tid] = acc;
}

__device__ __forceinline__ void mont_mul29_ref_fq(const uint32_t (&a)[9], const uint32_t (&b)[9], uint32_t (&r)[9]) {
    const uint32_t MASK = (1u << 29) - 1;
    uint32_t p[9];
    {
        uint64_t acc = 0; int bits = 0, w = 0;
        for (int i = 0; i < 9; i++) {
            while (bits < 29 && w < 8) { acc |= (uint64_t)FqP::MOD[w++] << bits; bits += 32; }
            p[i] = (uint32_t)acc & MASK; acc >>= 29; bits -= 29;
        }
    }
    uint32_t pinv = 1;
    for (int i = 0; i < 5; i++) pinv *= 2u - p[0] * pinv;
    pinv = (0u - pinv) & MASK;
    uint32_t m[9];
    uint64_t acc = 0;
    for (int k = 0; k < 17; k++) {
        for (int i = (k > 8 ? k - 8 : 0); i <= (k < 8 ? k : 8); i++) acc += (uint64_t)a[i] * b[k - i];
        for (int i = (k > 8 ? k - 8 : 0); i <= (k < 8 ? k : 8); i++)
            if (i < k || k >= 9) { if (i != k) acc += (uint64_t)m[i] * p[k - i]; }
        if (k < 9) {
            m[k] = ((uint32_t)acc * pinv) & MASK;
            acc += (uint64_t)m[k] * p[0];
        } else r[k - 9] = (uint32_t)acc & MASK;
        acc >>= 29;
    }
    r[8] = (uint32_t)acc;
}
__global__ __launch_bounds__(256) void ub_modmul29i_kernel(uint32_t* io, int iters, uint32_t* mismatches) {
    size_t t = (size_t)blockIdx.x * blockDim.x + threadIdx.x;
    uint32_t a[9], b[9], c[9], d[9], r[9];
    for (int i = 0; i < 9; i++) {
        uint32_t x = io[t * 8 + (i & 7)] * 2654435761u + i;
        a[i] = x & 0x1fffffffu; b[i] = (x >> 3) & 0x1fffffffu; c[i] = (x * 7u) & 0x1fffffffu; d[i] = (x * 13u) & 0x1fffffffu;
    }
    a[8] &= 0x3fffu; b[8] &= 0x3fffu; c[8] &= 0x3fffu; d[8] &= 0x3fffu;
    if (mismatches) {
        uint32_t want[9];
        bool bad = false;
        mont_mul29i_fq(a, b, r);
        mont_mul29_ref_fq(a, b, want);
        for (int i = 0; i < 9; i++) bad |= r[i] != want[i];
        mont_sqr29i_fq(c, r);
        mont_mul29_ref_fq(c, c, want);
        for (int i = 0; i < 9; i++) bad |= r[i] != want[i];
        mont_mul29i_fr(a, d, r);
        mont_mul29_fr(a, d, want);
        for (int i = 0; i < 9; i++) bad |= r[i] != want[i];
        if (bad) atomicAdd(mismatches, 1u);
    }
    for (int k = 0; k < iters; k++) {
        mont_mul29i_fq(a, b, r); for (int i = 0; i < 9; i++) a[i] = r[i];
        mont_mul29i_fq(c, d, r); for (int i = 0; i < 9; i++) c[i] = r[i];
        mont_mul29i_fq(b, a, r); for (int i = 0; i < 9; i++) b[i] = r[i];
        mont_mul29i_fq(d, c, r); for (int i = 0; i < 9; i++) d[i] = r[i];
    }
    uint32_t x = 0;
    for (int i = 0; i < 9; i++) x ^= a[i] ^ b[i] ^ c[i] ^ d[i];
    io[t * 8] = x;
}
__global__ __launch_bounds__(256) void ub_modmul29_kernel(uint32_t* io, int iters, uint32_t* mismatches) {
    size_t t = (size_t)blockIdx.x * blockDim.x + threadIdx.x;
    uint32_t a[9], b[9], c[9], d[9], r[9];
    for (int i = 0; i < 9; i++) {
        uint32_t x = io[t * 8 + (i & 7)] * 2654435761u + i;
        a[i] = x & 0x1fffffffu; b[i] = (x >> 3) & 0x1fffffffu; c[i] = (x * 7u) & 0x1fffffffu; d[i] = (x * 13u) & 0x1fffffffu;
    }
    a[8] &= 0x3fffu; b[8] &= 0x3fffu; c[8] &= 0x3fffu; d[8] &= 0x3fffu;
    if (mismatches) {
        uint32_t want[9];
        mont_mul29_fq(a, b, r);
        mont_mul29_ref_fq(a, b, want);
        bool bad = false;
        for (int i = 0; i < 9; i++) bad |= r[i] != want[i];
        if (bad) atomicAdd(mismatches, 1u);
    }
    for (int k = 0; k < iters; k++) {
        mont_mul29_fq(a, b, r); for (int i = 0; i < 9; i++) a[i] = r[i];
        mont_mul29_fq(c, d, r); for (int i = 0; i < 9; i++) c[i] = r[i];
        mont_mul29_fq(b, a, r); for (int i = 0; i < 9; i++) b[i] = r[i];
        mont_mul29_fq(d, c, r); for (int i = 0; i < 9; i++) d[i] = r[i];
    }
    uint32_t x = 0;
    for (int i = 0; i < 9; i++) x ^= a[i] ^ b[i] ^ c[i] ^ d[i];
    io[t * 8] = x;
}

template <int MODE>
__global__ __launch_bounds__(256) void ub_mix_kernel(uint64_t* io, int iters) {
    size_t i = (size_t)blockIdx.x * blockDim.x + threadIdx.x;
    uint64_t x = io[i];
    uint64_t a0 = x, a1 = x + 1, a2 = x + 2, a3 = x + 3, a4 = x + 4, a5 = x + 5, a6 = x + 6, a7 = x + 7;
    double d0 = (double)(x & 1023), d1 = d0 + 1, d2 = d0 + 2, d3 = d0 + 3, d4 = d0 + 4, d5 = d0 + 5, d6 = d0 + 6, d7 = d0 + 7;
    const double m = 1.0000001, q = 0.9999999;
    uint32_t mi = (uint32_t)x | 1u, qi = (uint32_t)(x >> 32) | 3u;
    for (int k = 0; k < iters; k++) {
        if (MODE == 0) {
            a0 = mad_wide(mi, (uint32_t)a0, a0); a1 = mad_wide(qi, (uint32_t)a1, a1); a2 = mad_wide(mi, (uint32_t)a2, a2); a3 = mad_wide(qi, (uint32_t)a3, a3);
            a4 = mad_wide(mi, (uint32_t)a4, a4); a5 = mad_wide(qi, (uint32_t)a5, a5); a6 = mad_wide(mi, (uint32_t)a6, a6); a7 = mad_wide(qi, (uint32_t)a7, a7);
        } else if (MODE == 1) {
            d0 = __builtin_fma(d0, m, q); d1 = __builtin_fma(d1, q, m); d2 = __builtin_fma(d2, m, q); d3 = __builtin_fma(d3, q, m);
            d4 = __builtin_fma(d4, m, q); d5 = __builtin_fma(d5, q, m); d6 = __builtin_fma(d6, m, q); d7 = __builtin_fma(d7, q, m);
        } else if (MODE == 2) {
            a0 = mad_wide(mi, (uint32_t)a0, a0); d4 = __builtin_fma(d4, m, q); a1 = mad_wide(qi, (uint32_t)a1, a1); d5 = __builtin_fma(d5, q, m);
            a2 = mad_wide(mi, (uint32_t)a2, a2); d6 = __builtin_fma(d6, m, q); a3 = mad_wide(qi, (uint32_t)a3, a3); d7 = __builtin_fma(d7, q, m);
        } else if (MODE == 3) {
            asm volatile("v_lshl_add_u64 %0, %0, 0, %1\n\tv_lshl_add_u64 %1, %1, 0, %2\n\tv_lshl_add_u64 %2, %2, 0, %3\n\tv_lshl_add_u64 %3, %3, 0, %4\n\t"
                         "v_lshl_add_u64 %4, %4, 0, %5\n\tv_lshl_add_u64 %5, %5, 0, %6\n\tv_lshl_add_u64 %6, %6, 0, %7\n\tv_lshl_add_u64 %7, %7, 0, %0"
                         : "+v"(a0), "+v"(a1), "+v"(a2), "+v"(a3), "+v"(a4), "+v"(a5), "+v"(a6), "+v"(a7));
        } else {
            asm volatile("v_add_f64 %0, %0, %8\n\tv_add_f64 %1, %1, %9\n\tv_add_f64 %2, %2, %8\n\tv_add_f64 %3, %3, %9\n\t"
                         "v_add_f64 %4, %4, %8\n\tv_add_f64 %5, %5, %9\n\tv_add_f64 %6, %6, %8\n\tv_add_f64 %7, %7, %9"
                         : "+v"(d0), "+v"(d1), "+v"(d2), "+v"(d3), "+v"(d4), "+v"(d5), "+v"(d6), "+v"(d7) : "v"(m), "v"(q));
        }
    }
    io[i] = a0 ^ a1 ^ a2 ^ a3 ^ a4 ^ a5 ^ a6 ^ a7 ^ (uint64_t)(d0 + d1 + d2 + d3 + d4 + d5 + d6 + d7);
}

struct Dfma52 {
    static constexpr uint64_t M52 = (1ull << 52) - 1;
    EZ_HD static constexpr uint64_t limb(int i) {
        uint64_t v = 0;
        for (int b = 0; b < 52; b++) {
            const int bit = 52 * i + b;
            if (bit < 256 && ((FqP::MOD[bit >> 5] >> (bit & 31)) & 1u)) v |= 1ull << b;
        }
        return v;
    }
    EZ_HD static constexpr uint64_t pinv() {
        uint64_t x = 1;
        for (int i = 0; i < 6; i++) x *= 2 - limb(0) * x;
        return (0 - x) & M52;
    }
};
__device__ __forceinline__ void dfma_hilo(double a, double b, uint64_t& hi_raw, uint64_t& lo_raw) {
    const double C1 = 0x1p104, C2 = 0x1p104 + 0x1p52;
    const double h = __builtin_fma(a, b, C1);
    const double s = C2 - h;
    const double l = __builtin_fma(a, b, s);
    hi_raw = (uint64_t)__double_as_longlong(h);
    lo_raw = (uint64_t)__double_as_longlong(l);
}
__device__ __forceinline__ void mont_mul52_dfma_fq(const double (&a)[5], const double (&b)[5], double (&r)[5]) {
    constexpr uint64_t HI_PAT = 0x4670000000000000ull, LO_PAT = 0x4330000000000000ull, M52 = Dfma52::M52;
    double m[5];
    double pd[5];
#pragma unroll
    for (int i = 0; i < 5; i++) pd[i] = (double)Dfma52::limb(i);
    const double pinv = (double)Dfma52::pinv();
    uint64_t carry = 0, nxt = 0;
#pragma unroll
    for (int k = 0; k < 10; k++) {
        uint64_t acc = carry + nxt, hi, lo;
        nxt = 0;
        int cnt = 0;
#pragma unroll
        for (int i = 0; i < 5; i++) {
            const int j = k - i;
            if (j < 0 || j > 4) continue;
            dfma_hilo(a[i], b[j], hi, lo);
            acc += lo; nxt += hi; cnt++;
            if (i < k && i < 5 && k < 5) {}
        }
#pragma unroll
        for (int i = 0; i < 5; i++) {
            const int j = k - i;
            if (j < 0 || j > 4) continue;
            if (k < 5 && i == k) continue;
            dfma_hilo(m[i], pd[j], hi, lo);
            acc += lo; nxt += hi; cnt++;
        }
        acc -= (uint64_t)cnt * LO_PAT;
        nxt -= (uint64_t)cnt * HI_PAT;
        if (k < 5) {
            const double t = __longlong_as_double((long long)(LO_PAT | (acc & M52))) - 0x1p52;
            dfma_hilo(t, pinv, hi, lo);
            m[k] = __longlong_as_double((long long)(LO_PAT | (lo & M52))) - 0x1p52;
            dfma_hilo(m[k], pd[0], hi, lo);
            acc += lo - LO_PAT; nxt += hi - HI_PAT;
            carry = acc >> 52;
        } else {
            r[k - 5] = __longlong_as_double((long long)(LO_PAT | (acc & M52))) - 0x1p52;
            carry = acc >> 52;
        }
    }
}
__device__ inline void mont_mul52_ref_fq(const uint64_t (&a)[5], const uint64_t (&b)[5], uint64_t (&r)[5]) {
    constexpr uint64_t M52 = Dfma52::M52;
    uint64_t m[5], p[5];
    for (int i = 0; i < 5; i++) p[i] = Dfma52::limb(i);
    const uint64_t pinv = Dfma52::pinv();
    unsigned __int128 acc = 0;
    for (int k = 0; k < 10; k++) {
        for (int i = 0; i < 5; i++) {
            const int j = k - i;
            if (j < 0 || j > 4) continue;
            acc += (unsigned __int128)a[i] * b[j];
            if (!(k < 5 && i == k)) acc += (unsigned __int128)m[i] * p[j];
        }
        if (k < 5) {
            m[k] = (((uint64_t)acc & M52) * pinv) & M52;
            acc += (unsigned __int128)m[k] * p[0];
        } else r[k - 5] = (uint64_t)acc & M52;
        acc >>= 52;
    }
}
__global__ __launch_bounds__(256) void ub_dfma52_kernel(uint32_t* io, int iters, uint32_t* mismatches) {
    asm volatile("s_setreg_imm32_b32 hwreg(HW_REG_MODE, 2, 2), 3");
    size_t t = (size_t)blockIdx.x * blockDim.x + threadIdx.x;
    uint64_t ai[5], bi[5], ci[5], di[5];
    for (int i = 0; i < 5; i++) {
        uint64_t x = ((uint64_t)io[t * 8 + (i & 7)] * 2654435761u + i) * 0x9e3779b97f4a7c15ull;
        ai[i] = x & Dfma52::M52; bi[i] = (x >> 7) & Dfma52::M52; ci[i] = (x * 7u) & Dfma52::M52; di[i] = (x * 13u) & Dfma52::M52;
    }
    ai[4] &= (1ull << 44) - 1; bi[4] &= (1ull << 44) - 1; ci[4] &= (1ull << 44) - 1; di[4] &= (1ull << 44) - 1;
    double a[5], b[5], c[5], d[5], r[5];
    for (int i = 0; i < 5; i++) { a[i] = (double)ai[i]; b[i] = (double)bi[i]; c[i] = (double)ci[i]; d[i] = (double)di[i]; }
    if (mismatches) {
        uint64_t want[5];
        bool bad = false;
        mont_mul52_dfma_fq(a, b, r);
        mont_mul52_ref_fq(ai, bi, want);
        for (int i = 0; i < 5; i++) bad |= (uint64_t)r[i] != want[i];
        mont_mul52_dfma_fq(c, d, r);
        mont_mul52_ref_fq(ci, di, want);
        for (int i = 0; i < 5; i++) bad |= (uint64_t)r[i] != want[i];
        if (bad) atomicAdd(mismatches, 1u);
    }
    for (int k = 0; k < iters; k++) {
        mont_mul52_dfma_fq(a, b, r); for (int i = 0; i < 5; i++) a[i] = r[i];
        mont_mul52_dfma_fq(c, d, r); for (int i = 0; i < 5; i++) c[i] = r[i];
        mont_mul52_dfma_fq(b, a, r); for (int i = 0; i < 5; i++) b[i] = r[i];
        mont_mul52_dfma_fq(d, c, r); for (int i = 0; i < 5; i++) d[i] = r[i];
    }
    double x = 0;
    for (int i = 0; i < 5; i++) x += a[i] + b[i] + c[i] + d[i];
    io[t * 8] = (uint32_t)(uint64_t)x;
}
// ... 40 lines not shown
    const g1x29_t a = g1x29_quad_bcast<0>(x), b = g1x29_quad_bcast<1>(x);
    const g1x29_t plain = g1x29_add(a, b);
    bool special;
    const g1x29_t coop = g1x29_add_quad(a, b, special, out + 64 * 160 + (size_t)l * 128);
    o[4] = special ? 1u : 0u;
    {
        const f29_t v = x.y;
        const f29_t b2 = f29_quad_bcast<2>(v), b3 = f29_quad_bcast<3>(v);
        const f29_t y1 = Fq29::sub<1>(b2, b3);
        f29_t c2 = b2, c3 = b3;
        for (int i = 0; i < 9; i++) { asm volatile("" : "+v"(c2.v[i])); asm volatile("" : "+v"(c3.v[i])); }
        const f29_t y2 = Fq29::sub<1>(c2, c3);
        f29_t s2, s3;
        for (int i = 0; i < 9; i++) { s2.v[i] = __shfl(v.v[i], (l & ~3u) | 2u); s3.v[i] = __shfl(v.v[i], (l & ~3u) | 3u); }
        const f29_t y3 = Fq29::sub<1>(s2, s3);
        uint32_t* e = out + 64 * 360 + (size_t)l * 36;
        for (int i = 0; i < 9; i++) { e[i] = y1.v[i]; e[9 + i] = y2.v[i]; e[18 + i] = y3.v[i]; e[27 + i] = v.v[i]; }
    }
    for (int i = 0; i < 36; i++) { out[64 * 160 + 64 * 128 + (size_t)l * 72 + i] = a.x.v[i]; out[64 * 160 + 64 * 128 + (size_t)l * 72 + 36 + i] = b.x.v[i]; }
    for (int i = 0; i < 36; i++) { o[8 + i] = plain.x.v[i]; o[44 + i] = coop.x.v[i]; }
    const g1x29_t s0 = g1x29_group_sum(x, 64), s1 = g1x29_group_sum_coop(x, 64);
    for (int i = 0; i < 36; i++) { o[80 + i] = s0.x.v[i]; o[116 + i] = s1.x.v[i]; }
}

__global__ __launch_bounds__(256) void ub_coopcheck2_kernel(const g1a_t* pts, uint32_t* out, int with_identities) {
    __shared__ uint4 sh[9 * 4];
    const uint32_t t = threadIdx.x;
    g1x29_t x = g1x29_add_mixed(g1x29_identity(), g1a29_unpack(ld_g1a(pts + t)), false);
    x = g1x29_add(x, g1x29_add_mixed(g1x29_identity(), g1a29_unpack(ld_g1a(pts + 256 + t)), false));
    if (with_identities && (t % 5 == 1 || (t >= 64 && t < 72))) x = g1x29_identity();
    uint32_t* o = out + (size_t)t * 216;
    const g1x29_t a0 = g1x29_group_sum(x, 32), a1 = g1x29_group_sum_coop(x, 32);
    const g1x29_t b0 = g1x29_group_sum(x, 8), b1 = g1x29_group_sum_coop(x, 8);
    if (t < 36) sh[t] = make_uint4(0, 0, 0, 0);
    __syncthreads();
    const g1x29_t c1 = g1x29_block256_sum_coop(x, sh);
    const g1x29_t c0 = g1x29_block256_sum(x, sh);
    for (int i = 0; i < 36; i++) { o[i] = a0.x.v[i]; o[36 + i] = a1.x.v[i]; o[72 + i] = b0.x.v[i]; o[108 + i] = b1.x.v[i]; o[144 + i] = c0.x.v[i]; o[180 + i] = c1.x.v[i]; }
}

int ubench(Ctx* c, const char* which, double* out) {
    hipStream_t st = c->stream;
    hipEvent_t e0, e1;
    int rc = ev_pair(c, "ubench", &e0, &e1);
    if (rc) return rc;
    const int blocks = c->num_cus * 16, threads = 256;
    const size_t nthreads = (size_t)blocks * threads;
    float ms = 0.f;
    const bool is_mm = !strncmp(which, "modmul", 6) && strncmp(which, "modmul29", 8);
    if (is_mm || !strcmp(which, "mad64") || !strcmp(which, "mullo") || !strcmp(which, "dfma") || !strcmp(which, "addsub")) {
        void* buf = nullptr;
        EZ_HIP(hipMalloc(&buf, nthreads * 32));
        EZ_HIP(hipMemsetAsync(buf, 0x11, nthreads * 32, st));
        const int iters = is_mm ? 256 : 4096;
        int blocks = c->num_cus * 16;
        if (const char* o = strstr(which, "_o")) blocks = c->num_cus * atoi(o + 2);
        const size_t nthreads = (size_t)blocks * threads;
        for (int rep = 0; rep < 2; rep++) {
            EZ_HIP(hipEventRecord(e0, st));
            if (!strncmp(which, "modmul_o", 8) || !strcmp(which, "modmul")) hipLaunchKernelGGL(ub_modmul_kernel<0>, dim3(blocks), dim3(threads), 0, st, (fe_t*)buf, iters);
            else if (!strcmp(which, "modmul_c")) hipLaunchKernelGGL(ub_modmul_kernel<1>, dim3(blocks), dim3(threads), 0, st, (fe_t*)buf, iters);
            else if (!strcmp(which, "modmul_inl")) hipLaunchKernelGGL(ub_modmul_kernel<2>, dim3(blocks), dim3(threads), 0, st, (fe_t*)buf, iters);
            else if (!strcmp(which, "addsub")) hipLaunchKernelGGL(ub_addsub_kernel, dim3(blocks), dim3(threads), 0, st, (fe_t*)buf, iters);
            else if (!strcmp(which, "mullo")) hipLaunchKernelGGL(ub_mullo_kernel, dim3(blocks), dim3(threads), 0, st, (uint64_t*)buf, iters);
            else if (!strcmp(which, "mad64")) hipLaunchKernelGGL(ub_mad64_kernel, dim3(blocks), dim3(threads), 0, st, (uint64_t*)buf, iters);
            else hipLaunchKernelGGL(ub_dfma_kernel, dim3(blocks), dim3(threads), 0, st, (double*)buf, iters);
            EZ_HIP(hipEventRecord(e1, st));
            EZ_HIP(hipStreamSynchronize(st));
            EZ_HIP(hipEventElapsedTime(&ms, e0, e1));
        }
        EZ_HIP(hipFree(buf));
        const double per_thread = (is_mm || !strcmp(which, "addsub")) ? 4.0 * iters : 8.0 * iters;
        *out = per_thread * (double)nthreads / (ms * 1e-3);
        return EZKL_OK;
    }
    if (!strcmp(which, "waveinv")) {
        const int threads = 256, blocks = c->num_cus * 16, iters = 16;
        const size_t nthreads = (size_t)threads * blocks;
        void* buf = nullptr;
        EZ_HIP(hipMalloc(&buf, nthreads * sizeof(fe_t)));
        std::vector<fe_t> init(nthreads);
        for (size_t t = 0; t < nthreads; t++) { init[t] = Fr::one(); init[t].v[0] = (uint32_t)(t * 2654435761u) | 1u; init[t].v[7] = 0; }
        EZ_HIP(hipMemcpy(buf, init.data(), nthreads * sizeof(fe_t), hipMemcpyHostToDevice));
        hipEvent_t e0, e1;
        EZ_HIP(hipEventCreate(&e0)); EZ_HIP(hipEventCreate(&e1));
        float ms = 0;
        for (int rep = 0; rep < 2; rep++) {
            EZ_HIP(hipEventRecord(e0, st));
            hipLaunchKernelGGL(ub_waveinv_kernel, dim3(blocks), dim3(threads), 0, st, (fe_t*)buf, iters);
            EZ_HIP(hipEventRecord(e1, st));
            EZ_HIP(hipEventSynchronize(e1));
            EZ_HIP(hipEventElapsedTime(&ms, e0, e1));
        }
        (void)hipEventDestroy(e0); (void)hipEventDestroy(e1);
        (void)hipFree(buf);
        *out = (double)nthreads * iters / (ms * 1e-3);
        return EZKL_OK;
    }
    if (!strncmp(which, "mix_", 4)) {
        void* buf = nullptr;
        int blocks = c->num_cus * 16;
        if (const char* o = strstr(which, "_o")) blocks = c->num_cus * atoi(o + 2);
        const size_t nthreads = (size_t)blocks * threads;
        EZ_HIP(hipMalloc(&buf, nthreads * 8));
        EZ_HIP(hipMemsetAsync(buf, 0x11, nthreads * 8, st));
        const int iters = 4096;
        for (int rep = 0; rep < 2; rep++) {
            EZ_HIP(hipEventRecord(e0, st));
            if (!strncmp(which, "mix_mad", 7)) hipLaunchKernelGGL(ub_mix_kernel<0>, dim3(blocks), dim3(threads), 0, st, (uint64_t*)buf, iters);
            else if (!strncmp(which, "mix_dfma", 8)) hipLaunchKernelGGL(ub_mix_kernel<1>, dim3(blocks), dim3(threads), 0, st, (uint64_t*)buf, iters);
            else if (!strncmp(which, "mix_both", 8)) hipLaunchKernelGGL(ub_mix_kernel<2>, dim3(blocks), dim3(threads), 0, st, (uint64_t*)buf, iters);
            else if (!strncmp(which, "mix_add64", 9)) hipLaunchKernelGGL(ub_mix_kernel<3>, dim3(blocks), dim3(threads), 0, st, (uint64_t*)buf, iters);
            else hipLaunchKernelGGL(ub_mix_kernel<4>, dim3(blocks), dim3(threads), 0, st, (uint64_t*)buf, iters);
            EZ_HIP(hipEventRecord(e1, st));
            EZ_HIP(hipStreamSynchronize(st));
            EZ_HIP(hipEventElapsedTime(&ms, e0, e1));
        }
        EZ_HIP(hipFree(buf));
        *out = 8.0 * iters * (double)nthreads / (ms * 1e-3);
        return EZKL_OK;
    }
    if (!strncmp(which, "dfma52", 6)) {
        void* buf = nullptr;
        uint32_t* mis = nullptr;
        const bool chk = strstr(which, "check") != nullptr;
        const int iters = chk ? 1 : 256;
        int blocks = c->num_cus * 16;
        if (const char* o = strstr(which, "_o")) blocks = c->num_cus * atoi(o + 2);
        const size_t nthreads = (size_t)blocks * threads;
        EZ_HIP(hipMalloc(&buf, nthreads * 32));
        EZ_HIP(hipMalloc((void**)&mis, 4));
        {
            std::vector<uint32_t> h(nthreads * 8);
            uint64_t x = 0x9e3779b97f4a7c15ull;
            for (auto& w : h) { x ^= x << 13; x ^= x >> 7; x ^= x << 17; w = (uint32_t)(x >> 16); }
            EZ_HIP(hipMemcpyAsync(buf, h.data(), nthreads * 32, hipMemcpyHostToDevice, st));
            EZ_HIP(hipStreamSynchronize(st));
        }
        EZ_HIP(hipMemsetAsync(mis, 0, 4, st));
        for (int rep = 0; rep < 2; rep++) {
            EZ_HIP(hipEventRecord(e0, st));
            hipLaunchKernelGGL(ub_dfma52_kernel, dim3(blocks), dim3(threads), 0, st, (uint32_t*)buf, iters, chk ? mis : nullptr);
            EZ_HIP(hipEventRecord(e1, st));
            EZ_HIP(hipStreamSynchronize(st));
            EZ_HIP(hipEventElapsedTime(&ms, e0, e1));
        }
        uint32_t hm = 0;
        EZ_HIP(hipMemcpy(&hm, mis, 4, hipMemcpyDeviceToHost));
        EZ_HIP(hipFree(buf));
        EZ_HIP(hipFree(mis));
        *out = chk ? (double)hm : 4.0 * iters * (double)nthreads / (ms * 1e-3);
        return EZKL_OK;
    }
    if (!strncmp(which, "modmul29", 8)) {
        void* buf = nullptr;
        uint32_t* mis = nullptr;
        EZ_HIP(hipMalloc(&buf, nthreads * 32));
        EZ_HIP(hipMalloc((void**)&mis, 4));
        EZ_HIP(hipMemsetAsync(buf, 0x5b, nthreads * 32, st));
        EZ_HIP(hipMemsetAsync(mis, 0, 4, st));
        const bool chk = strstr(which, "check") != nullptr;
        const int iters = chk ? 1 : 256;
        int blocks = c->num_cus * 16;
        if (const char* o = strstr(which, "_o")) blocks = c->num_cus * atoi(o + 2);
        const size_t nthreads = (size_t)blocks * threads;
        for (int rep = 0; rep < 2; rep++) {
            EZ_HIP(hipEventRecord(e0, st));
            if (!strncmp(which, "modmul29i", 9)) hipLaunchKernelGGL(ub_modmul29i_kernel, dim3(blocks), dim3(threads), 0, st, (uint32_t*)buf, iters, chk ? mis : nullptr);
            else hipLaunchKernelGGL(ub_modmul29_kernel, dim3(blocks), dim3(threads), 0, st, (uint32_t*)buf, iters, chk ? mis : nullptr);
            EZ_HIP(hipEventRecord(e1, st));
            EZ_HIP(hipStreamSynchronize(st));
            EZ_HIP(hipEventElapsedTime(&ms, e0, e1));
        }
        uint32_t hm = 0;
        EZ_HIP(hipMemcpy(&hm, mis, 4, hipMemcpyDeviceToHost));
        EZ_HIP(hipFree(buf));
        EZ_HIP(hipFree(mis));
        *out = chk ? (double)hm : 4.0 * iters * (double)nthreads / (ms * 1e-3);
        return EZKL_OK;
    }
    if (!strncmp(which, "ecadd", 5)) {
        const int iters = atoi(which + 5);
        const char mode = which[strlen(which) - 1];
        const bool full = mode == 'f';
        const int eb = full ? c->num_cus * 4 : mode == 'h' ? c->num_cus * 4 : mode == 'q' ? c->num_cus : 1, et = full ? 256 : 64;
        void* buf = nullptr;
        const size_t cnt = (size_t)eb * et + 1;
        EZ_HIP(hipMalloc(&buf, cnt * sizeof(g1x_t)));
        EZ_HIP(hipMemsetAsync(buf, 0, cnt * sizeof(g1x_t), st));
        {
            std::vector<g1x_t> h(cnt);
            g1x_t g;
            g.x = Fq::one(); g.y = Fq::add(Fq::one(), Fq::one()); g.zz = Fq::one(); g.zzz = Fq::one();
            for (size_t i = 0; i < cnt; i++) h[i] = g;
            for (size_t i = 0; i + 1 < cnt; i += 2) h[i] = g1x_double(g);
            EZ_HIP(hipMemcpyAsync(buf, h.data(), cnt * sizeof(g1x_t), hipMemcpyHostToDevice, st));
            EZ_HIP(hipStreamSynchronize(st));
        }
        for (int rep = 0; rep < 4; rep++) {
            EZ_HIP(hipEventRecord(e0, st));
            if (which[5] == 't') hipLaunchKernelGGL(ub_ectree_kernel, dim3(eb), dim3(64), 0, st, (g1x_t*)buf);
            else if (which[5] == 'u') hipLaunchKernelGGL(ub_ectree_u_kernel, dim3(eb), dim3(64), 0, st, (g1x_t*)buf);
            else if (which[5] == 'v') hipLaunchKernelGGL(ub_ectree_v_kernel, dim3(eb), dim3(64), 0, st, (g1x_t*)buf, 0u);
            else if (which[5] == 'x') hipLaunchKernelGGL(ub_ectree_v_kernel, dim3(eb), dim3(64), 0, st, (g1x_t*)buf, 64u);
            else hipLaunchKernelGGL(ub_ecadd_kernel, dim3(eb), dim3(et), 0, st, (g1x_t*)buf, iters);
            EZ_HIP(hipEventRecord(e1, st));
            EZ_HIP(hipStreamSynchronize(st));
            EZ_HIP(hipEventElapsedTime(&ms, e0, e1));
        }
        EZ_HIP(hipFree(buf));
        *out = ms * 1e3;
        return EZKL_OK;
    }
    if (!strcmp(which, "coopcheck")) {
        const Bases* dummy = nullptr; (void)dummy;
        g1a_t* pts = nullptr;
        uint32_t* o = nullptr;
        EZ_HIP(hipMalloc(&pts, 512 * sizeof(g1a_t)));
        EZ_HIP(hipMalloc(&o, 64 * (160 + 128 + 72 + 36) * 4));
        EZ_HIP(hipMemsetAsync(o, 0, 64 * (160 + 128 + 72 + 36) * 4, st));
        {
            std::vector<g1a_t> h(512);
            h64::aff g;
            memset(&g, 0, sizeof g);
            h64::fe one; { uint32_t w[8]; for (int q = 0; q < 8; q++) w[q] = Fq::one().v[q]; one = h64::from32(w); }
            g.x = one; g.y = h64::add(one, one);
            h64::xyzz acc = h64::from_affine(g), G = acc;
            h64::fe k261; { uint32_t w[8]; for (int q = 0; q < 8; q++) w[q] = Fq29C::R261_32[q]; k261 = h64::from32(w); }
            for (int i = 0; i < 512; i++) {
                h64::aff a = h64::to_affine(acc);
                h64::fe tx = h64::mul(a.x, k261), ty = h64::mul(a.y, k261);
                memcpy(&h[i].x, &tx, 32); memcpy(&h[i].y, &ty, 32);
                acc = h64::add(acc, G);
                acc = h64::add(acc, G);
                acc = h64::add(acc, G);
            }
            EZ_HIP(hipMemcpy(pts, h.data(), 512 * sizeof(g1a_t), hipMemcpyHostToDevice));
        }
        hipLaunchKernelGGL(ub_coopcheck_kernel, dim3(1), dim3(64), 0, st, pts, o);
        EZ_HIP(hipStreamSynchronize(st));
        std::vector<uint32_t> h(64 * (160 + 128 + 72 + 36));
        EZ_HIP(hipMemcpy(h.data(), o, h.size() * 4, hipMemcpyDeviceToHost));
        uint32_t mask = 0;
        {
            uint32_t* o2 = nullptr;
            EZ_HIP(hipMalloc(&o2, 256 * 216 * 4));
            std::vector<uint32_t> h2(256 * 216);
            for (int ident = 0; ident < 2; ident++) {
                hipLaunchKernelGGL(ub_coopcheck2_kernel, dim3(1), dim3(256), 0, st, pts, o2, ident);
                EZ_HIP(hipStreamSynchronize(st));
                EZ_HIP(hipMemcpy(h2.data(), o2, h2.size() * 4, hipMemcpyDeviceToHost));
                int bad[3] = {0, 0, 0};
                for (uint32_t t = 0; t < 256; t++)
                    for (int f = 0; f < 3; f++) {
                        const h64::aff p0 = h64::to_affine(h64::from_limbs29_point(h2.data() + (size_t)t * 216 + 72 * f));
                        const h64::aff p1 = h64::to_affine(h64::from_limbs29_point(h2.data() + (size_t)t * 216 + 72 * f + 36));
                        if (memcmp(&p0, &p1, 64)) { if (!bad[f]) fprintf(stderr, "[coopcheck] identities=%d form %d (0: width 32, 1: width 8, 2: block): thread %u differs\n", ident, f, t); bad[f]++; }
                    }
                fprintf(stderr, "[coopcheck] identities=%d: width 32: %d bad, width 8: %d bad, block of 256: %d bad\n", ident, bad[0], bad[1], bad[2]);
                if (bad[0] || bad[1] || bad[2]) mask |= 16u << ident;
            }
            EZ_HIP(hipFree(o2));
        }
        EZ_HIP(hipFree(pts)); EZ_HIP(hipFree(o));
        for (uint32_t l = 0; l < 64; l++) {
            const uint32_t* r = h.data() + (size_t)l * 160;
            for (uint32_t sidx = 0; sidx < 4; sidx++)
                if (r[sidx] != (l & ~3u) + sidx) { if (!(mask & 1)) fprintf(stderr, "[coopcheck] bcast<%u> lane %u got %u\n", sidx, l, r[sidx]); mask |= 1; }
            if (r[4]) { if (!(mask & 2)) fprintf(stderr, "[coopcheck] lane %u: special flag set\n", l); mask |= 2; }
            const h64::aff p0 = h64::to_affine(h64::from_limbs29_point(r + 8)), p1 = h64::to_affine(h64::from_limbs29_point(r + 44));
            if (memcmp(&p0, &p1, 64)) {
                if (!(mask & 4)) {
                    fprintf(stderr, "[coopcheck] lane %u: add_quad != add (x %s, y %s)\n", l, memcmp(&p0.x, &p1.x, 32) ? "differs" : "same", memcmp(&p0.y, &p1.y, 32) ? "differs" : "same");
                    for (int q = 0; q < 4; q++) {
                        const h64::fe c0 = h64::from_limbs29(r + 8 + 9 * q), c1 = h64::from_limbs29(r + 44 + 9 * q);
                        fprintf(stderr, "[coopcheck]   coordinate %d: %s\n", q, memcmp(&c0, &c1, 32) ? "differs" : "same residue");
                    }
                }
                mask |= 4;
            }
            const h64::aff t0 = h64::to_affine(h64::from_limbs29_point(r + 80)), t1 = h64::to_affine(h64::from_limbs29_point(r + 116));
            if (memcmp(&t0, &t1, 64)) { if (!(mask & 8)) fprintf(stderr, "[coopcheck] lane %u: cooperative butterfly sum != plain\n", l); mask |= 8; }
        }
        {
            int bad[3] = {0, 0, 0};
            static const uint32_t SUBC1[9] = {0x21f3f51cu, 0x241182dau, 0x31ca8d3bu, 0x2b548b42u, 0x361765dfu, 0x2b6d0301u, 0x229b8503u, 0x397098cfu, 0x00c19138u};
            for (uint32_t l = 0; l < 64; l++) {
                const uint32_t* e = h.data() + 64 * 360 + (size_t)l * 36;
                const uint32_t* v2 = h.data() + 64 * 360 + (size_t)((l & ~3u) | 2u) * 36 + 27;
                const uint32_t* v3 = h.data() + 64 * 360 + (size_t)((l & ~3u) | 3u) * 36 + 27;
                for (int f = 0; f < 3; f++)
                    for (int i = 0; i < 9; i++)
                        if (e[9 * f + i] != v2[i] + (SUBC1[i] - v3[i])) { if (!bad[f]) fprintf(stderr, "[coopcheck] form %d lane %u limb %d: got %08x want %08x\n", f, l, i, e[9 * f + i], v2[i] + (SUBC1[i] - v3[i])); bad[f]++; }
            }
            fprintf(stderr, "[coopcheck] broadcast-subtract: combined %d bad, kept apart %d bad, shfl %d bad\n", bad[0], bad[1], bad[2]);
        }
        if (mask & 4) {
            const uint32_t* r0 = h.data();
            fprintf(stderr, "[coopcheck] plain.y:"); for (int i = 0; i < 9; i++) fprintf(stderr, " %08x", r0[8 + 9 + i]); fprintf(stderr, "\n");
            fprintf(stderr, "[coopcheck] coop.y: "); for (int i = 0; i < 9; i++) fprintf(stderr, " %08x", r0[44 + 9 + i]); fprintf(stderr, "\n");
            for (uint32_t q = 0; q < 4; q++) { fprintf(stderr, "[coopcheck] lane %u coop.y:", q); for (int i = 0; i < 9; i++) fprintf(stderr, " %08x", h[(size_t)q * 160 + 44 + 9 + i]); fprintf(stderr, "\n"); }
            for (int k = 0; k < 14; k++) for (uint32_t q = 0; q < 4; q++) { fprintf(stderr, "[coopcheck] t%d[q%u]: ", k, q); for (int i = 0; i < 9; i++) fprintf(stderr, " %08x", h[64 * 160 + q * 128 + 9 * k + i]); fprintf(stderr, "\n"); }
            for (uint32_t q = 0; q < 4; q++) { fprintf(stderr, "[coopcheck] m4[q%u]: ", q); for (int i = 0; i < 9; i++) fprintf(stderr, " %08x", h[64 * 160 + q * 128 + 9 * 13 + i]); fprintf(stderr, "\n"); }
        }
        if (mask & 4) {
            static const char* names[14] = {"m1", "u1", "s1", "p", "r", "m2", "pp", "rr", "m3", "ppp", "qq", "x3", "d", "m4"};
// ... 63 lines not shown
```

Before: 800.8 million pts/s.

## Fuse add/sub into Montgomery multiply asm for in-place mixed bucket accumulation

```diff
diff --git a/ezkl_amd/csrc/curve29.hpp b/ezkl_amd/csrc/curve29.hpp
--- a/ezkl_amd/csrc/curve29.hpp
+++ b/ezkl_amd/csrc/curve29.hpp
@@ -85,30 +85,41 @@
     r.zzz = Fq29::mul_cold(w, p.zzz);
     return r;
 }
+EZ_D void g1x29_acc_mixed(g1x29_t& acc, const g1a29_t& q, bool negate) {
+    if (g1a29_is_id(q)) return;
+    const f29_t qy = negate ? Fq29::neg<0>(q.y) : q.y;
+    uint32_t rare = 1;
+    if (!g1x29_is_id(acc)) {
+        const f29_t tx = Fq29::neg<3>(acc.x);
+        const f29_t ty = Fq29::neg<3>(acc.y);
+        const f29_t p = Fq29::muladd(q.x, acc.zz, tx);
+        const f29_t r = Fq29::muladd(qy, acc.zzz, ty);
+        rare = 0;
+        if (Fq29::is_zero_mod_p(p)) rare = Fq29::is_zero_mod_p(r) ? 2 : 3;
+        else {
+            const f29_t pp = Fq29::sqr(p);
+            Fq29::mul_into(acc.zz, pp);
+            const f29_t ppp = Fq29::mul(p, pp);
+            Fq29::mul_into(acc.zzz, ppp);
+            const f29_t nq = Fq29::mul(tx, pp);
+            acc.x = Fq29::sqradd(r, Fq29::add(Fq29::neg<1>(ppp), Fq29::add(nq, nq)));
+            const f29_t d = Fq29::neg2_16p(nq, acc.x);
+            acc.y = Fq29::mul2add(r, d, ty, ppp);
+        }
+    }
+    if (rare) {
+        g1a29_t qq = q;
+        if (negate) qq.y = Fq29::normalize(qy);
+        if (rare == 1) {
+            acc.x = qq.x; acc.y = qq.y; acc.zz = Fq29::one(); acc.zzz = Fq29::one();
+        } else if (rare == 2) acc = g1x29_double_affine(qq);
+        else acc = g1x29_identity();
+    }
+}
 EZ_D g1x29_t g1x29_add_mixed(const g1x29_t& a, const g1a29_t& q, bool negate) {
-    if (g1a29_is_id(q)) return a;
-    const f29_t qy = negate ? Fq29::neg<0>(q.y) : q.y;
-    if (g1x29_is_id(a)) {
-        g1x29_t r;
-        r.x = q.x;
-        r.y = negate ? Fq29::normalize(qy) : q.y;
-        r.zz = Fq29::one();
-        r.zzz = Fq29::one();
-        return r;
-    }
-    const f29_t u2 = Fq29::mul(q.x, a.zz);
-    const f29_t s2 = Fq29::mul(qy, a.zzz);
-    const f29_t p = Fq29::normalize(Fq29::sub<3>(u2, a.x));
-    const f29_t r = Fq29::normalize(Fq29::sub<3>(s2, a.y));
-    if (Fq29::is_zero_mod_p(p)) {
-        if (Fq29::is_zero_mod_p(r)) {
-            g1a29_t qq = q;
-            if (negate) qq.y = Fq29::normalize(qy);
-            return g1x29_double_affine(qq);
-        }
-        return g1x29_identity();
-    }
-    return g1x29_add_tail(a.x, a.y, p, r, a.zz, a.zzz);
+    g1x29_t r = a;
+    g1x29_acc_mixed(r, q, negate);
+    return r;
 }
 EZ_D g1x29_t g1x29_add(const g1x29_t& a, const g1x29_t& b) {
     if (g1x29_is_id(a)) return b;
diff --git a/ezkl_amd/csrc/field29.hpp b/ezkl_amd/csrc/field29.hpp
--- a/ezkl_amd/csrc/field29.hpp
+++ b/ezkl_amd/csrc/field29.hpp
@@ -68,6 +68,22 @@
         mont_mul2add29_fq(a.v, b.v, c.v, d.v, r.v);
         return r;
     }
+    EZ_D static f29_t muladd(const f29_t& a, const f29_t& b, const f29_t& t) {
+        static_assert(IS_FQ, "generated for Fq only");
+        f29_t r;
+        mont_muladd29_fq(a.v, b.v, t.v, r.v);
+        return r;
+    }
+    EZ_D static f29_t sqradd(const f29_t& a, const f29_t& t) {
+        static_assert(IS_FQ, "generated for Fq only");
+        f29_t r;
+        mont_sqradd29_fq(a.v, t.v, r.v);
+        return r;
+    }
+    EZ_D static void mul_into(f29_t& b, const f29_t& a) {
+        static_assert(IS_FQ, "generated for Fq only");
+        mont_mulip29_fq(a.v, b.v);
+    }
     EZ_D static f29_t mul_cold(const f29_t& a, const f29_t& b) {
         u32x9 x, y;
 #pragma unroll
@@ -101,6 +117,12 @@
         f29_t r;
 #pragma unroll
         for (int i = 0; i < 9; i++) r.v[i] = a.v[i] + (C::SUBC[KI][i] - b.v[i]);
+        return r;
+    }
+    EZ_D static f29_t neg2_16p(const f29_t& b, const f29_t& c) {
+        f29_t r;
+#pragma unroll
+        for (int i = 0; i < 9; i++) r.v[i] = C::SUBC2_16P[i] - b.v[i] - c.v[i];
         return r;
     }
     template <int KI>
diff --git a/ezkl_amd/csrc/montmul29_gen.hpp b/ezkl_amd/csrc/montmul29_gen.hpp
--- a/ezkl_amd/csrc/montmul29_gen.hpp
+++ b/ezkl_amd/csrc/montmul29_gen.hpp
@@ -16,6 +16,7 @@
         {0x3f3f51c0u, 0x21182dafu, 0x3ca8d3c1u, 0x3548b437u, 0x21765e04u, 0x36d0302au, 0x29b85044u, 0x37098d00u, 0x0c19139bu},
         {0x3e7ea380u, 0x22305b60u, 0x3951a783u, 0x2a916870u, 0x22ecbc0au, 0x2da06055u, 0x3370a08au, 0x2e131a01u, 0x18322738u},
     };
+    static constexpr uint32_t SUBC2_16P[9] = {0x47cfd470u, 0x50460b6au, 0x472a34eeu, 0x4d522d0cu, 0x585d977fu, 0x4db40c08u, 0x4a6e140fu, 0x45c2633eu, 0x030644e5u};
     static constexpr uint32_t CSUB[4][9] = {
         {0x078302b9u, 0x1efb9f49u, 0x038d5cb0u, 0x1d2add2fu, 0x0a7a2687u, 0x1d24bf3fu, 0x1f591ebeu, 0x11a3d9cbu, 0x1fcf9bb1u},
         {0x0f060572u, 0x1df73e92u, 0x071ab961u, 0x1a55ba5eu, 0x14f44d0fu, 0x1a497e7eu, 0x1eb23d7du, 0x0347b397u, 0x1f9f3763u},
@@ -37,6 +38,7 @@
         {0x20000040u, 0x23eb27dfu, 0x3709143du, 0x34243cdbu, 0x2174a0ceu, 0x36d0302au, 0x29b85044u, 0x37098d00u, 0x0c19139bu},
         {0x20000080u, 0x27d64fbfu, 0x2e12287bu, 0x284879b8u, 0x22e9419eu, 0x2da06055u, 0x3370a08au, 0x2e131a01u, 0x18322738u},
     };
+    static constexpr uint32_t SUBC2_16P[9] = {0x40000010u, 0x50fac9f6u, 0x45c2450du, 0x5d090f35u, 0x585d2831u, 0x4db40c08u, 0x4a6e140fu, 0x45c2633eu, 0x030644e5u};
     static constexpr uint32_t CSUB[4][9] = {
         {0x0fffffffu, 0x00f05360u, 0x11a3dbafu, 0x182f6f0cu, 0x0a7a2d7cu, 0x1d24bf3fu, 0x1f591ebeu, 0x11a3d9cbu, 0x1fcf9bb1u},
         {0x1ffffffeu, 0x01e0a6c0u, 0x0347b75eu, 0x105ede19u, 0x14f45af9u, 0x1a497e7eu, 0x1eb23d7du, 0x0347b397u, 0x1f9f3763u},
@@ -1875,4 +1877,659 @@
         : [a0] "v"(a[0]), [a1] "v"(a[1]), [a2] "v"(a[2]), [a3] "v"(a[3]), [a4] "v"(a[4]), [a5] "v"(a[5]), [a6] "v"(a[6]), [a7] "v"(a[7]), [a8] "v"(a[8]), [b0] "v"(b[0]), [b1] "v"(b[1]), [b2] "v"(b[2]), [b3] "v"(b[3]), [b4] "v"(b[4]), [b5] "v"(b[5]), [b6] "v"(b[6]), [b7] "v"(b[7]), [b8] "v"(b[8])
         : "v16", "v17", "v18", "v19", "s16", "s17", "s18", "s19", "s20", "s21", "s22", "s23", "s24", "s25", "s26", "vcc");
 }
+__device__ __forceinline__ void mont_muladd29_fq(const uint32_t (&a)[9], const uint32_t (&b)[9], const uint32_t (&t)[9], uint32_t (&r)[9]) {
+    asm("s_mov_b32 s16, 0x187cfd47\n\t"
+        "s_mov_b32 s17, 0x010460b6\n\t"
+        "s_mov_b32 s18, 0x1c72a34f\n\t"
+        "s_mov_b32 s19, 0x02d522d0\n\t"
+        "s_mov_b32 s20, 0x1585d978\n\t"
+        "s_mov_b32 s21, 0x02db40c0\n\t"
+        "s_mov_b32 s22, 0x00a6e141\n\t"
+        "s_mov_b32 s23, 0x0e5c2634\n\t"
+        "s_mov_b32 s24, 0x0030644e\n\t"
+        "s_mov_b32 s25, 0x04866389\n\t"
+        "s_mov_b32 s26, 0x1fffffff\n\t"
+        "v_mad_u64_u32 v[16:17], vcc, %[a0], %[b0], 0\n\t"
+        "v_mul_lo_u32 %[r0], v16, s25\n\t"
+        "v_and_b32 %[r0], s26, %[r0]\n\t"
+        "v_mad_u64_u32 v[16:17], vcc, %[r0], s16, v[16:17]\n\t"
+        "v_lshrrev_b64 v[16:17], 29, v[16:17]\n\t"
+        "v_mad_u64_u32 v[16:17], vcc, %[a0], %[b1], v[16:17]\n\t"
+        "v_mad_u64_u32 v[16:17], vcc, %[a1], %[b0], v[16:17]\n\t"
+        "v_mad_u64_u32 v[16:17], vcc, %[r0], s17, v[16:17]\n\t"
+        "v_mul_lo_u32 %[r1], v16, s25\n\t"
+        "v_and_b32 %[r1], s26, %[r1]\n\t"
+        "v_mad_u64_u32 v[16:17], vcc, %[r1], s16, v[16:17]\n\t"
+        "v_lshrrev_b64 v[16:17], 29, v[16:17]\n\t"
+        "v_mad_u64_u32 v[16:17], vcc, %[a0], %[b2], v[16:17]\n\t"
+        "v_mad_u64_u32 v[16:17], vcc, %[a1], %[b1], v[16:17]\n\t"
+        "v_mad_u64_u32 v[16:17], vcc, %[a2], %[b0], v[16:17]\n\t"
+        "v_mad_u64_u32 v[16:17], vcc, %[r0], s18, v[16:17]\n\t"
+        "v_mad_u64_u32 v[16:17], vcc, %[r1], s17, v[16:17]\n\t"
+        "v_mul_lo_u32 %[r2], v16, s25\n\t"
+        "v_and_b32 %[r2], s26, %[r2]\n\t"
+        "v_mad_u64_u32 v[16:17], vcc, %[r2], s16, v[16:17]\n\t"
+        "v_lshrrev_b64 v[16:17], 29, v[16:17]\n\t"
+        "v_mad_u64_u32 v[16:17], vcc, %[a0], %[b3], v[16:17]\n\t"
+        "v_mad_u64_u32 v[16:17], vcc, %[a1], %[b2], v[16:17]\n\t"
+        "v_mad_u64_u32 v[16:17], vcc, %[a2], %[b1], v[16:17]\n\t"
+        "v_mad_u64_u32 v[16:17], vcc, %[a3], %[b0], v[16:17]\n\t"
+        "v_mad_u64_u32 v[16:17], vcc, %[r0], s19, v[16:17]\n\t"
+        "v_mad_u64_u32 v[16:17], vcc, %[r1], s18, v[16:17]\n\t"
+        "v_mad_u64_u32 v[16:17], vcc, %[r2], s17, v[16:17]\n\t"
+        "v_mul_lo_u32 %[r3], v16, s25\n\t"
+        "v_and_b32 %[r3], s26, %[r3]\n\t"
+        "v_mad_u64_u32 v[16:17], vcc, %[r3], s16, v[16:17]\n\t"
+        "v_lshrrev_b64 v[16:17], 29, v[16:17]\n\t"
+        "v_mad_u64_u32 v[16:17], vcc, %[a0], %[b4], v[16:17]\n\t"
+        "v_mad_u64_u32 v[16:17], vcc, %[a1], %[b3], v[16:17]\n\t"
+        "v_mad_u64_u32 v[16:17], vcc, %[a2], %[b2], v[16:17]\n\t"
+        "v_mad_u64_u32 v[16:17], vcc, %[a3], %[b1], v[16:17]\n\t"
+        "v_mad_u64_u32 v[16:17], vcc, %[a4], %[b0], v[16:17]\n\t"
+        "v_mad_u64_u32 v[16:17], vcc, %[r0], s20, v[16:17]\n\t"
+        "v_mad_u64_u32 v[16:17], vcc, %[r1], s19, v[16:17]\n\t"
+        "v_mad_u64_u32 v[16:17], vcc, %[r2], s18, v[16:17]\n\t"
+        "v_mad_u64_u32 v[16:17], vcc, %[r3], s17, v[16:17]\n\t"
+        "v_mul_lo_u32 %[r4], v16, s25\n\t"
+        "v_and_b32 %[r4], s26, %[r4]\n\t"
+        "v_mad_u64_u32 v[16:17], vcc, %[r4], s16, v[16:17]\n\t"
+        "v_lshrrev_b64 v[16:17], 29, v[16:17]\n\t"
+        "v_mad_u64_u32 v[16:17], vcc, %[a0], %[b5], v[16:17]\n\t"
+        "v_mad_u64_u32 v[16:17], vcc, %[a1], %[b4], v[16:17]\n\t"
+        "v_mad_u64_u32 v[16:17], vcc, %[a2], %[b3], v[16:17]\n\t"
+        "v_mad_u64_u32 v[16:17], vcc, %[a3], %[b2], v[16:17]\n\t"
+        "v_mad_u64_u32 v[16:17], vcc, %[a4], %[b1], v[16:17]\n\t"
+        "v_mad_u64_u32 v[16:17], vcc, %[a5], %[b0], v[16:17]\n\t"
+        "v_mad_u64_u32 v[16:17], vcc, %[r0], s21, v[16:17]\n\t"
+        "v_mad_u64_u32 v[16:17], vcc, %[r1], s20, v[16:17]\n\t"
+        "v_mad_u64_u32 v[16:17], vcc, %[r2], s19, v[16:17]\n\t"
+        "v_mad_u64_u32 v[16:17], vcc, %[r3], s18, v[16:17]\n\t"
+        "v_mad_u64_u32 v[16:17], vcc, %[r4], s17, v[16:17]\n\t"
+        "v_mul_lo_u32 %[r5], v16, s25\n\t"
+        "v_and_b32 %[r5], s26, %[r5]\n\t"
+        "v_mad_u64_u32 v[16:17], vcc, %[r5], s16, v[16:17]\n\t"
+        "v_lshrrev_b64 v[16:17], 29, v[16:17]\n\t"
+        "v_mad_u64_u32 v[16:17], vcc, %[a0], %[b6], v[16:17]\n\t"
+        "v_mad_u64_u32 v[16:17], vcc, %[a1], %[b5], v[16:17]\n\t"
+        "v_mad_u64_u32 v[16:17], vcc, %[a2], %[b4], v[16:17]\n\t"
+        "v_mad_u64_u32 v[16:17], vcc, %[a3], %[b3], v[16:17]\n\t"
+        "v_mad_u64_u32 v[16:17], vcc, %[a4], %[b2], v[16:17]\n\t"
+        "v_mad_u64_u32 v[16:17], vcc, %[a5], %[b1], v[16:17]\n\t"
+        "v_mad_u64_u32 v[16:17], vcc, %[a6], %[b0], v[16:17]\n\t"
+        "v_mad_u64_u32 v[16:17], vcc, %[r0], s22, v[16:17]\n\t"
+        "v_mad_u64_u32 v[16:17], vcc, %[r1], s21, v[16:17]\n\t"
+        "v_mad_u64_u32 v[16:17], vcc, %[r2], s20, v[16:17]\n\t"
+        "v_mad_u64_u32 v[16:17], vcc, %[r3], s19, v[16:17]\n\t"
+        "v_mad_u64_u32 v[16:17], vcc, %[r4], s18, v[16:17]\n\t"
+        "v_mad_u64_u32 v[16:17], vcc, %[r5], s17, v[16:17]\n\t"
+        "v_mul_lo_u32 %[r6], v16, s25\n\t"
+        "v_and_b32 %[r6], s26, %[r6]\n\t"
+        "v_mad_u64_u32 v[16:17], vcc, %[r6], s16, v[16:17]\n\t"
+        "v_lshrrev_b64 v[16:17], 29, v[16:17]\n\t"
+        "v_mad_u64_u32 v[16:17], vcc, %[a0], %[b7], v[16:17]\n\t"
+        "v_mad_u64_u32 v[16:17], vcc, %[a1], %[b6], v[16:17]\n\t"
+        "v_mad_u64_u32 v[16:17], vcc, %[a2], %[b5], v[16:17]\n\t"
+        "v_mad_u64_u32 v[16:17], vcc, %[a3], %[b4], v[16:17]\n\t"
+        "v_mad_u64_u32 v[16:17], vcc, %[a4], %[b3], v[16:17]\n\t"
+        "v_mad_u64_u32 v[16:17], vcc, %[a5], %[b2], v[16:17]\n\t"
+        "v_mad_u64_u32 v[16:17], vcc, %[a6], %[b1], v[16:17]\n\t"
+        "v_mad_u64_u32 v[16:17], vcc, %[a7], %[b0], v[16:17]\n\t"
+        "v_mad_u64_u32 v[16:17], vcc, %[r0], s23, v[16:17]\n\t"
+        "v_mad_u64_u32 v[16:17], vcc, %[r1], s22, v[16:17]\n\t"
+        "v_mad_u64_u32 v[16:17], vcc, %[r2], s21, v[16:17]\n\t"
+        "v_mad_u64_u32 v[16:17], vcc, %[r3], s20, v[16:17]\n\t"
+        "v_mad_u64_u32 v[16:17], vcc, %[r4], s19, v[16:17]\n\t"
+        "v_mad_u64_u32 v[16:17], vcc, %[r5], s18, v[16:17]\n\t"
+        "v_mad_u64_u32 v[16:17], vcc, %[r6], s17, v[16:17]\n\t"
+        "v_mul_lo_u32 %[r7], v16, s25\n\t"
+        "v_and_b32 %[r7], s26, %[r7]\n\t"
+        "v_mad_u64_u32 v[16:17], vcc, %[r7], s16, v[16:17]\n\t"
+        "v_lshrrev_b64 v[16:17], 29, v[16:17]\n\t"
+        "v_mad_u64_u32 v[16:17], vcc, %[a0], %[b8], v[16:17]\n\t"
+        "v_mad_u64_u32 v[16:17], vcc, %[a1], %[b7], v[16:17]\n\t"
+        "v_mad_u64_u32 v[16:17], vcc, %[a2], %[b6], v[16:17]\n\t"
+        "v_mad_u64_u32 v[16:17], vcc, %[a3], %[b5], v[16:17]\n\t"
+        "v_mad_u64_u32 v[16:17], vcc, %[a4], %[b4], v[16:17]\n\t"
+        "v_mad_u64_u32 v[16:17], vcc, %[a5], %[b3], v[16:17]\n\t"
+        "v_mad_u64_u32 v[16:17], vcc, %[a6], %[b2], v[16:17]\n\t"
+        "v_mad_u64_u32 v[16:17], vcc, %[a7], %[b1], v[16:17]\n\t"
+        "v_mad_u64_u32 v[16:17], vcc, %[a8], %[b0], v[16:17]\n\t"
+        "v_mad_u64_u32 v[16:17], vcc, %[r0], s24, v[16:17]\n\t"
+        "v_mad_u64_u32 v[16:17], vcc, %[r1], s23, v[16:17]\n\t"
+        "v_mad_u64_u32 v[16:17], vcc, %[r2], s22, v[16:17]\n\t"
+        "v_mad_u64_u32 v[16:17], vcc, %[r3], s21, v[16:17]\n\t"
+        "v_mad_u64_u32 v[16:17], vcc, %[r4], s20, v[16:17]\n\t"
+        "v_mad_u64_u32 v[16:17], vcc, %[r5], s19, v[16:17]\n\t"
+        "v_mad_u64_u32 v[16:17], vcc, %[r6], s18, v[16:17]\n\t"
+        "v_mad_u64_u32 v[16:17], vcc, %[r7], s17, v[16:17]\n\t"
+        "v_mul_lo_u32 %[r8], v16, s25\n\t"
+        "v_and_b32 %[r8], s26, %[r8]\n\t"
+        "v_mad_u64_u32 v[16:17], vcc, %[r8], s16, v[16:17]\n\t"
+        "v_lshrrev_b64 v[16:17], 29, v[16:17]\n\t"
+        "v_mad_u64_u32 v[16:17], vcc, %[a1], %[b8], v[16:17]\n\t"
+        "v_mad_u64_u32 v[16:17], vcc, %[a2], %[b7], v[16:17]\n\t"
+        "v_mad_u64_u32 v[16:17], vcc, %[a3], %[b6], v[16:17]\n\t"
+        "v_mad_u64_u32 v[16:17], vcc, %[a4], %[b5], v[16:17]\n\t"
+        "v_mad_u64_u32 v[16:17], vcc, %[a5], %[b4], v[16:17]\n\t"
+        "v_mad_u64_u32 v[16:17], vcc, %[a6], %[b3], v[16:17]\n\t"
+        "v_mad_u64_u32 v[16:17], vcc, %[a7], %[b2], v[16:17]\n\t"
+        "v_mad_u64_u32 v[16:17], vcc, %[a8], %[b1], v[16:17]\n\t"
+        "v_mad_u64_u32 v[16:17], vcc, %[r1], s24, v[16:17]\n\t"
+        "v_mad_u64_u32 v[16:17], vcc, %[r2], s23, v[16:17]\n\t"
+        "v_mad_u64_u32 v[16:17], vcc, %[r3], s22, v[16:17]\n\t"
+        "v_mad_u64_u32 v[16:17], vcc, %[r4], s21, v[16:17]\n\t"
+        "v_mad_u64_u32 v[16:17], vcc, %[r5], s20, v[16:17]\n\t"
+        "v_mad_u64_u32 v[16:17], vcc, %[r6], s19, v[16:17]\n\t"
+        "v_mad_u64_u32 v[16:17], vcc, %[r7], s18, v[16:17]\n\t"
+        "v_mad_u64_u32 v[16:17], vcc, %[r8], s17, v[16:17]\n\t"
+        "v_mad_u64_u32 v[16:17], vcc, %[t0], 1, v[16:17]\n\t"
+        "v_and_b32 %[r0], s26, v16\n\t"
+        "v_lshrrev_b64 v[16:17], 29, v[16:17]\n\t"
+        "v_mad_u64_u32 v[16:17], vcc, %[a2], %[b8], v[16:17]\n\t"
+        "v_mad_u64_u32 v[16:17], vcc, %[a3], %[b7], v[16:17]\n\t"
+        "v_mad_u64_u32 v[16:17], vcc, %[a4], %[b6], v[16:17]\n\t"
+        "v_mad_u64_u32 v[16:17], vcc, %[a5], %[b5], v[16:17]\n\t"
+        "v_mad_u64_u32 v[16:17], vcc, %[a6], %[b4], v[16:17]\n\t"
+        "v_mad_u64_u32 v[16:17], vcc, %[a7], %[b3], v[16:17]\n\t"
+        "v_mad_u64_u32 v[16:17], vcc, %[a8], %[b2], v[16:17]\n\t"
+        "v_mad_u64_u32 v[16:17], vcc, %[r2], s24, v[16:17]\n\t"
+        "v_mad_u64_u32 v[16:17], vcc, %[r3], s23, v[16:17]\n\t"
+        "v_mad_u64_u32 v[16:17], vcc, %[r4], s22, v[16:17]\n\t"
+        "v_mad_u64_u32 v[16:17], vcc, %[r5], s21, v[16:17]\n\t"
+        "v_mad_u64_u32 v[16:17], vcc, %[r6], s20, v[16:17]\n\t"
+        "v_mad_u64_u32 v[16:17], vcc, %[r7], s19, v[16:17]\n\t"
+        "v_mad_u64_u32 v[16:17], vcc, %[r8], s18, v[16:17]\n\t"
+        "v_mad_u64_u32 v[16:17], vcc, %[t1], 1, v[16:17]\n\t"
+        "v_and_b32 %[r1], s26, v16\n\t"
+        "v_lshrrev_b64 v[16:17], 29, v[16:17]\n\t"
+        "v_mad_u64_u32 v[16:17], vcc, %[a3], %[b8], v[16:17]\n\t"
+        "v_mad_u64_u32 v[16:17], vcc, %[a4], %[b7], v[16:17]\n\t"
+        "v_mad_u64_u32 v[16:17], vcc, %[a5], %[b6], v[16:17]\n\t"
+        "v_mad_u64_u32 v[16:17], vcc, %[a6], %[b5], v[16:17]\n\t"
+        "v_mad_u64_u32 v[16:17], vcc, %[a7], %[b4], v[16:17]\n\t"
+        "v_mad_u64_u32 v[16:17], vcc, %[a8], %[b3], v[16:17]\n\t"
+        "v_mad_u64_u32 v[16:17], vcc, %[r3], s24, v[16:17]\n\t"
+        "v_mad_u64_u32 v[16:17], vcc, %[r4], s23, v[16:17]\n\t"
+        "v_mad_u64_u32 v[16:17], vcc, %[r5], s22, v[16:17]\n\t"
+        "v_mad_u64_u32 v[16:17], vcc, %[r6], s21, v[16:17]\n\t"
+        "v_mad_u64_u32 v[16:17], vcc, %[r7], s20, v[16:17]\n\t"
+        "v_mad_u64_u32 v[16:17], vcc, %[r8], s19, v[16:17]\n\t"
+        "v_mad_u64_u32 v[16:17], vcc, %[t2], 1, v[16:17]\n\t"
+        "v_and_b32 %[r2], s26, v16\n\t"
+        "v_lshrrev_b64 v[16:17], 29, v[16:17]\n\t"
+        "v_mad_u64_u32 v[16:17], vcc, %[a4], %[b8], v[16:17]\n\t"
+        "v_mad_u64_u32 v[16:17], vcc, %[a5], %[b7], v[16:17]\n\t"
+        "v_mad_u64_u32 v[16:17], vcc, %[a6], %[b6], v[16:17]\n\t"
+        "v_mad_u64_u32 v[16:17], vcc, %[a7], %[b5], v[16:17]\n\t"
+        "v_mad_u64_u32 v[16:17], vcc, %[a8], %[b4], v[16:17]\n\t"
+        "v_mad_u64_u32 v[16:17], vcc, %[r4], s24, v[16:17]\n\t"
+        "v_mad_u64_u32 v[16:17], vcc, %[r5], s23, v[16:17]\n\t"
+        "v_mad_u64_u32 v[16:17], vcc, %[r6], s22, v[16:17]\n\t"
+        "v_mad_u64_u32 v[16:17], vcc, %[r7], s21, v[16:17]\n\t"
+        "v_mad_u64_u32 v[16:17], vcc, %[r8], s20, v[16:17]\n\t"
+        "v_mad_u64_u32 v[16:17], vcc, %[t3], 1, v[16:17]\n\t"
+        "v_and_b32 %[r3], s26, v16\n\t"
+        "v_lshrrev_b64 v[16:17], 29, v[16:17]\n\t"
+        "v_mad_u64_u32 v[16:17], vcc, %[a5], %[b8], v[16:17]\n\t"
+        "v_mad_u64_u32 v[16:17], vcc, %[a6], %[b7], v[16:17]\n\t"
+        "v_mad_u64_u32 v[16:17], vcc, %[a7], %[b6], v[16:17]\n\t"
+        "v_mad_u64_u32 v[16:17], vcc, %[a8], %[b5], v[16:17]\n\t"
+        "v_mad_u64_u32 v[16:17], vcc, %[r5], s24, v[16:17]\n\t"
+        "v_mad_u64_u32 v[16:17], vcc, %[r6], s23, v[16:17]\n\t"
+        "v_mad_u64_u32 v[16:17], vcc, %[r7], s22, v[16:17]\n\t"
+        "v_mad_u64_u32 v[16:17], vcc, %[r8], s21, v[16:17]\n\t"
+        "v_mad_u64_u32 v[16:17], vcc, %[t4], 1, v[16:17]\n\t"
+        "v_and_b32 %[r4], s26, v16\n\t"
+        "v_lshrrev_b64 v[16:17], 29, v[16:17]\n\t"
+        "v_mad_u64_u32 v[16:17], vcc, %[a6], %[b8], v[16:17]\n\t"
+        "v_mad_u64_u32 v[16:17], vcc, %[a7], %[b7], v[16:17]\n\t"
+        "v_mad_u64_u32 v[16:17], vcc, %[a8], %[b6], v[16:17]\n\t"
+        "v_mad_u64_u32 v[16:17], vcc, %[r6], s24, v[16:17]\n\t"
+        "v_mad_u64_u32 v[16:17], vcc, %[r7], s23, v[16:17]\n\t"
+        "v_mad_u64_u32 v[16:17], vcc, %[r8], s22, v[16:17]\n\t"
+        "v_mad_u64_u32 v[16:17], vcc, %[t5], 1, v[16:17]\n\t"
+        "v_and_b32 %[r5], s26, v16\n\t"
+        "v_lshrrev_b64 v[16:17], 29, v[16:17]\n\t"
+        "v_mad_u64_u32 v[16:17], vcc, %[a7], %[b8], v[16:17]\n\t"
+        "v_mad_u64_u32 v[16:17], vcc, %[a8], %[b7], v[16:17]\n\t"
+        "v_mad_u64_u32 v[16:17], vcc, %[r7], s24, v[16:17]\n\t"
+        "v_mad_u64_u32 v[16:17], vcc, %[r8], s23, v[16:17]\n\t"
+        "v_mad_u64_u32 v[16:17], vcc, %[t6], 1, v[16:17]\n\t"
+        "v_and_b32 %[r6], s26, v16\n\t"
+        "v_lshrrev_b64 v[16:17], 29, v[16:17]\n\t"
+        "v_mad_u64_u32 v[16:17], vcc, %[a8], %[b8], v[16:17]\n\t"
+        "v_mad_u64_u32 v[16:17], vcc, %[r8], s24, v[16:17]\n\t"
+        "v_mad_u64_u32 v[16:17], vcc, %[t7], 1, v[16:17]\n\t"
+        "v_and_b32 %[r7], s26, v16\n\t"
+        "v_lshrrev_b64 v[16:17], 29, v[16:17]\n\t"
+        "v_add_u32 %[r8], v16, %[t8]\n\t"
+        : [r0] "=&v"(r[0]), [r1] "=&v"(r[1]), [r2] "=&v"(r[2]), [r3] "=&v"(r[3]), [r4] "=&v"(r[4]), [r5] "=&v"(r[5]), [r6] "=&v"(r[6]), [r7] "=&v"(r[7]), [r8] "=&v"(r[8])
+        : [a0] "v"(a[0]), [a1] "v"(a[1]), [a2] "v"(a[2]), [a3] "v"(a[3]), [a4] "v"(a[4]), [a5] "v"(a[5]), [a6] "v"(a[6]), [a7] "v"(a[7]), [a8] "v"(a[8]), [b0] "v"(b[0]), [b1] "v"(b[1]), [b2] "v"(b[2]), [b3] "v"(b[3]), [b4] "v"(b[4]), [b5] "v"(b[5]), [b6] "v"(b[6]), [b7] "v"(b[7]), [b8] "v"(b[8]), [t0] "v"(t[0]), [t1] "v"(t[1]), [t2] "v"(t[2]), [t3] "v"(t[3]), [t4] "v"(t[4]), [t5] "v"(t[5]), [t6] "v"(t[6]), [t7] "v"(t[7]), [t8] "v"(t[8])
+        : "v16", "v17", "s16", "s17", "s18", "s19", "s20", "s21", "s22", "s23", "s24", "s25", "s26", "vcc");
 }
+__device__ __forceinline__ void mont_sqradd29_fq(const uint32_t (&a)[9], const uint32_t (&t)[9], uint32_t (&r)[9]) {
+    uint32_t d[8];
+    asm("s_mov_b32 s16, 0x187cfd47\n\t"
+        "s_mov_b32 s17, 0x010460b6\n\t"
+        "s_mov_b32 s18, 0x1c72a34f\n\t"
+        "s_mov_b32 s19, 0x02d522d0\n\t"
+        "s_mov_b32 s20, 0x1585d978\n\t"
+        "s_mov_b32 s21, 0x02db40c0\n\t"
+        "s_mov_b32 s22, 0x00a6e141\n\t"
+        "s_mov_b32 s23, 0x0e5c2634\n\t"
+        "s_mov_b32 s24, 0x0030644e\n\t"
+        "s_mov_b32 s25, 0x04866389\n\t"
+        "s_mov_b32 s26, 0x1fffffff\n\t"
+        "v_lshlrev_b32 %[d0], 1, %[a0]\n\t"
+        "v_lshlrev_b32 %[d1], 1, %[a1]\n\t"
+        "v_lshlrev_b32 %[d2], 1, %[a2]\n\t"
+        "v_lshlrev_b32 %[d3], 1, %[a3]\n\t"
+        "v_lshlrev_b32 %[d4], 1, %[a4]\n\t"
+        "v_lshlrev_b32 %[d5], 1, %[a5]\n\t"
+        "v_lshlrev_b32 %[d6], 1, %[a6]\n\t"
+        "v_lshlrev_b32 %[d7], 1, %[a7]\n\t"
+        "v_mad_u64_u32 v[16:17], vcc, %[a0], %[a0], 0\n\t"
+        "v_mul_lo_u32 %[r0], v16, s25\n\t"
+        "v_and_b32 %[r0], s26, %[r0]\n\t"
+        "v_mad_u64_u32 v[16:17], vcc, %[r0], s16, v[16:17]\n\t"
+        "v_lshrrev_b64 v[16:17], 29, v[16:17]\n\t"
+        "v_mad_u64_u32 v[16:17], vcc, %[d0], %[a1], v[16:17]\n\t"
+        "v_mad_u64_u32 v[16:17], vcc, %[r0], s17, v[16:17]\n\t"
+        "v_mul_lo_u32 %[r1], v16, s25\n\t"
+        "v_and_b32 %[r1], s26, %[r1]\n\t"
+        "v_mad_u64_u32 v[16:17], vcc, %[r1], s16, v[16:17]\n\t"
+        "v_lshrrev_b64 v[16:17], 29, v[16:17]\n\t"
+        "v_mad_u64_u32 v[16:17], vcc, %[d0], %[a2], v[16:17]\n\t"
+        "v_mad_u64_u32 v[16:17], vcc, %[a1], %[a1], v[16:17]\n\t"
+        "v_mad_u64_u32 v[16:17], vcc, %[r0], s18, v[16:17]\n\t"
+        "v_mad_u64_u32 v[16:17], vcc, %[r1], s17, v[16:17]\n\t"
+        "v_mul_lo_u32 %[r2], v16, s25\n\t"
+        "v_and_b32 %[r2], s26, %[r2]\n\t"
+        "v_mad_u64_u32 v[16:17], vcc, %[r2], s16, v[16:17]\n\t"
+        "v_lshrrev_b64 v[16:17], 29, v[16:17]\n\t"
+        "v_mad_u64_u32 v[16:17], vcc, %[d0], %[a3], v[16:17]\n\t"
+        "v_mad_u64_u32 v[16:17], vcc, %[d1], %[a2], v[16:17]\n\t"
+        "v_mad_u64_u32 v[16:17], vcc, %[r0], s19, v[16:17]\n\t"
+        "v_mad_u64_u32 v[16:17], vcc, %[r1], s18, v[16:17]\n\t"
+        "v_mad_u64_u32 v[16:17], vcc, %[r2], s17, v[16:17]\n\t"
+        "v_mul_lo_u32 %[r3], v16, s25\n\t"
+        "v_and_b32 %[r3], s26, %[r3]\n\t"
+        "v_mad_u64_u32 v[16:17], vcc, %[r3], s16, v[16:17]\n\t"
+        "v_lshrrev_b64 v[16:17], 29, v[16:17]\n\t"
+        "v_mad_u64_u32 v[16:17], vcc, %[d0], %[a4], v[16:17]\n\t"
+        "v_mad_u64_u32 v[16:17], vcc, %[d1], %[a3], v[16:17]\n\t"
+        "v_mad_u64_u32 v[16:17], vcc, %[a2], %[a2], v[16:17]\n\t"
+        "v_mad_u64_u32 v[16:17], vcc, %[r0], s20, v[16:17]\n\t"
+        "v_mad_u64_u32 v[16:17], vcc, %[r1], s19, v[16:17]\n\t"
+        "v_mad_u64_u32 v[16:17], vcc, %[r2], s18, v[16:17]\n\t"
+        "v_mad_u64_u32 v[16:17], vcc, %[r3], s17, v[16:17]\n\t"
+        "v_mul_lo_u32 %[r4], v16, s25\n\t"
+        "v_and_b32 %[r4], s26, %[r4]\n\t"
+        "v_mad_u64_u32 v[16:17], vcc, %[r4], s16, v[16:17]\n\t"
+        "v_lshrrev_b64 v[16:17], 29, v[16:17]\n\t"
+        "v_mad_u64_u32 v[16:17], vcc, %[d0], %[a5], v[16:17]\n\t"
+        "v_mad_u64_u32 v[16:17], vcc, %[d1], %[a4], v[16:17]\n\t"
+        "v_mad_u64_u32 v[16:17], vcc, %[d2], %[a3], v[16:17]\n\t"
+        "v_mad_u64_u32 v[16:17], vcc, %[r0], s21, v[16:17]\n\t"
+        "v_mad_u64_u32 v[16:17], vcc, %[r1], s20, v[16:17]\n\t"
+        "v_mad_u64_u32 v[16:17], vcc, %[r2], s19, v[16:17]\n\t"
+        "v_mad_u64_u32 v[16:17], vcc, %[r3], s18, v[16:17]\n\t"
+        "v_mad_u64_u32 v[16:17], vcc, %[r4], s17, v[16:17]\n\t"
+        "v_mul_lo_u32 %[r5], v16, s25\n\t"
+        "v_and_b32 %[r5], s26, %[r5]\n\t"
+        "v_mad_u64_u32 v[16:17], vcc, %[r5], s16, v[16:17]\n\t"
+        "v_lshrrev_b64 v[16:17], 29, v[16:17]\n\t"
+        "v_mad_u64_u32 v[16:17], vcc, %[d0], %[a6], v[16:17]\n\t"
+        "v_mad_u64_u32 v[16:17], vcc, %[d1], %[a5], v[16:17]\n\t"
+        "v_mad_u64_u32 v[16:17], vcc, %[d2], %[a4], v[16:17]\n\t"
+        "v_mad_u64_u32 v[16:17], vcc, %[a3], %[a3], v[16:17]\n\t"
+        "v_mad_u64_u32 v[16:17], vcc, %[r0], s22, v[16:17]\n\t"
+        "v_mad_u64_u32 v[16:17], vcc, %[r1], s21, v[16:17]\n\t"
+        "v_mad_u64_u32 v[16:17], vcc, %[r2], s20, v[16:17]\n\t"
+        "v_mad_u64_u32 v[16:17], vcc, %[r3], s19, v[16:17]\n\t"
+        "v_mad_u64_u32 v[16:17], vcc, %[r4], s18, v[16:17]\n\t"
+        "v_mad_u64_u32 v[16:17], vcc, %[r5], s17, v[16:17]\n\t"
+        "v_mul_lo_u32 %[r6], v16, s25\n\t"
+        "v_and_b32 %[r6], s26, %[r6]\n\t"
+        "v_mad_u64_u32 v[16:17], vcc, %[r6], s16, v[16:17]\n\t"
+        "v_lshrrev_b64 v[16:17], 29, v[16:17]\n\t"
+        "v_mad_u64_u32 v[16:17], vcc, %[d0], %[a7], v[16:17]\n\t"
+        "v_mad_u64_u32 v[16:17], vcc, %[d1], %[a6], v[16:17]\n\t"
+        "v_mad_u64_u32 v[16:17], vcc, %[d2], %[a5], v[16:17]\n\t"
+        "v_mad_u64_u32 v[16:17], vcc, %[d3], %[a4], v[16:17]\n\t"
+        "v_mad_u64_u32 v[16:17], vcc, %[r0], s23, v[16:17]\n\t"
+        "v_mad_u64_u32 v[16:17], vcc, %[r1], s22, v[16:17]\n\t"
+        "v_mad_u64_u32 v[16:17], vcc, %[r2], s21, v[16:17]\n\t"
+        "v_mad_u64_u32 v[16:17], vcc, %[r3], s20, v[16:17]\n\t"
+        "v_mad_u64_u32 v[16:17], vcc, %[r4], s19, v[16:17]\n\t"
+        "v_mad_u64_u32 v[16:17], vcc, %[r5], s18, v[16:17]\n\t"
+        "v_mad_u64_u32 v[16:17], vcc, %[r6], s17, v[16:17]\n\t"
+        "v_mul_lo_u32 %[r7], v16, s25\n\t"
+        "v_and_b32 %[r7], s26, %[r7]\n\t"
+        "v_mad_u64_u32 v[16:17], vcc, %[r7], s16, v[16:17]\n\t"
+        "v_lshrrev_b64 v[16:17], 29, v[16:17]\n\t"
+        "v_mad_u64_u32 v[16:17], vcc, %[d0], %[a8], v[16:17]\n\t"
+        "v_mad_u64_u32 v[16:17], vcc, %[d1], %[a7], v[16:17]\n\t"
+        "v_mad_u64_u32 v[16:17], vcc, %[d2], %[a6], v[16:17]\n\t"
+        "v_mad_u64_u32 v[16:17], vcc, %[d3], %[a5], v[16:17]\n\t"
+        "v_mad_u64_u32 v[16:17], vcc, %[a4], %[a4], v[16:17]\n\t"
+        "v_mad_u64_u32 v[16:17], vcc, %[r0], s24, v[16:17]\n\t"
+        "v_mad_u64_u32 v[16:17], vcc, %[r1], s23, v[16:17]\n\t"
+        "v_mad_u64_u32 v[16:17], vcc, %[r2], s22, v[16:17]\n\t"
+        "v_mad_u64_u32 v[16:17], vcc, %[r3], s21, v[16:17]\n\t"
+        "v_mad_u64_u32 v[16:17], vcc, %[r4], s20, v[16:17]\n\t"
+        "v_mad_u64_u32 v[16:17], vcc, %[r5], s19, v[16:17]\n\t"
+        "v_mad_u64_u32 v[16:17], vcc, %[r6], s18, v[16:17]\n\t"
+        "v_mad_u64_u32 v[16:17], vcc, %[r7], s17, v[16:17]\n\t"
+        "v_mul_lo_u32 %[r8], v16, s25\n\t"
+        "v_and_b32 %[r8], s26, %[r8]\n\t"
+        "v_mad_u64_u32 v[16:17], vcc, %[r8], s16, v[16:17]\n\t"
+        "v_lshrrev_b64 v[16:17], 29, v[16:17]\n\t"
+        "v_mad_u64_u32 v[16:17], vcc, %[d1], %[a8], v[16:17]\n\t"
+        "v_mad_u64_u32 v[16:17], vcc, %[d2], %[a7], v[16:17]\n\t"
+        "v_mad_u64_u32 v[16:17], vcc, %[d3], %[a6], v[16:17]\n\t"
+        "v_mad_u64_u32 v[16:17], vcc, %[d4], %[a5], v[16:17]\n\t"
+        "v_mad_u64_u32 v[16:17], vcc, %[r1], s24, v[16:17]\n\t"
+        "v_mad_u64_u32 v[16:17], vcc, %[r2], s23, v[16:17]\n\t"
+        "v_mad_u64_u32 v[16:17], vcc, %[r3], s22, v[16:17]\n\t"
+        "v_mad_u64_u32 v[16:17], vcc, %[r4], s21, v[16:17]\n\t"
+        "v_mad_u64_u32 v[16:17], vcc, %[r5], s20, v[16:17]\n\t"
+        "v_mad_u64_u32 v[16:17], vcc, %[r6], s19, v[16:17]\n\t"
+        "v_mad_u64_u32 v[16:17], vcc, %[r7], s18, v[16:17]\n\t"
+        "v_mad_u64_u32 v[16:17], vcc, %[r8], s17, v[16:17]\n\t"
+        "v_mad_u64_u32 v[16:17], vcc, %[t0], 1, v[16:17]\n\t"
+        "v_and_b32 %[r0], s26, v16\n\t"
+        "v_lshrrev_b64 v[16:17], 29, v[16:17]\n\t"
+        "v_mad_u64_u32 v[16:17], vcc, %[d2], %[a8], v[16:17]\n\t"
+        "v_mad_u64_u32 v[16:17], vcc, %[d3], %[a7], v[16:17]\n\t"
+        "v_mad_u64_u32 v[16:17], vcc, %[d4], %[a6], v[16:17]\n\t"
+        "v_mad_u64_u32 v[16:17], vcc, %[a5], %[a5], v[16:17]\n\t"
+        "v_mad_u64_u32 v[16:17], vcc, %[r2], s24, v[16:17]\n\t"
+        "v_mad_u64_u32 v[16:17], vcc, %[r3], s23, v[16:17]\n\t"
+        "v_mad_u64_u32 v[16:17], vcc, %[r4], s22, v[16:17]\n\t"
+        "v_mad_u64_u32 v[16:17], vcc, %[r5], s21, v[16:17]\n\t"
+        "v_mad_u64_u32 v[16:17], vcc, %[r6], s20, v[16:17]\n\t"
+        "v_mad_u64_u32 v[16:17], vcc, %[r7], s19, v[16:17]\n\t"
+        "v_mad_u64_u32 v[16:17], vcc, %[r8], s18, v[16:17]\n\t"
+        "v_mad_u64_u32 v[16:17], vcc, %[t1], 1, v[16:17]\n\t"
+        "v_and_b32 %[r1], s26, v16\n\t"
+        "v_lshrrev_b64 v[16:17], 29, v[16:17]\n\t"
+        "v_mad_u64_u32 v[16:17], vcc, %[d3], %[a8], v[16:17]\n\t"
+        "v_mad_u64_u32 v[16:17], vcc, %[d4], %[a7], v[16:17]\n\t"
+        "v_mad_u64_u32 v[16:17], vcc, %[d5], %[a6], v[16:17]\n\t"
+        "v_mad_u64_u32 v[16:17], vcc, %[r3], s24, v[16:17]\n\t"
+        "v_mad_u64_u32 v[16:17], vcc, %[r4], s23, v[16:17]\n\t"
+        "v_mad_u64_u32 v[16:17], vcc, %[r5], s22, v[16:17]\n\t"
+        "v_mad_u64_u32 v[16:17], vcc, %[r6], s21, v[16:17]\n\t"
+        "v_mad_u64_u32 v[16:17], vcc, %[r7], s20, v[16:17]\n\t"
+        "v_mad_u64_u32 v[16:17], vcc, %[r8], s19, v[16:17]\n\t"
+        "v_mad_u64_u32 v[16:17], vcc, %[t2], 1, v[16:17]\n\t"
+        "v_and_b32 %[r2], s26, v16\n\t"
+        "v_lshrrev_b64 v[16:17], 29, v[16:17]\n\t"
+        "v_mad_u64_u32 v[16:17], vcc, %[d4], %[a8], v[16:17]\n\t"
+        "v_mad_u64_u32 v[16:17], vcc, %[d5], %[a7], v[16:17]\n\t"
+        "v_mad_u64_u32 v[16:17], vcc, %[a6], %[a6], v[16:17]\n\t"
+        "v_mad_u64_u32 v[16:17], vcc, %[r4], s24, v[16:17]\n\t"
+        "v_mad_u64_u32 v[16:17], vcc, %[r5], s23, v[16:17]\n\t"
+        "v_mad_u64_u32 v[16:17], vcc, %[r6], s22, v[16:17]\n\t"
+        "v_mad_u64_u32 v[16:17], vcc, %[r7], s21, v[16:17]\n\t"
+        "v_mad_u64_u32 v[16:17], vcc, %[r8], s20, v[16:17]\n\t"
+        "v_mad_u64_u32 v[16:17], vcc, %[t3], 1, v[16:17]\n\t"
+        "v_and_b32 %[r3], s26, v16\n\t"
+        "v_lshrrev_b64 v[16:17], 29, v[16:17]\n\t"
+        "v_mad_u64_u32 v[16:17], vcc, %[d5], %[a8], v[16:17]\n\t"
+        "v_mad_u64_u32 v[16:17], vcc, %[d6], %[a7], v[16:17]\n\t"
+        "v_mad_u64_u32 v[16:17], vcc, %[r5], s24, v[16:17]\n\t"
+        "v_mad_u64_u32 v[16:17], vcc, %[r6], s23, v[16:17]\n\t"
+        "v_mad_u64_u32 v[16:17], vcc, %[r7], s22, v[16:17]\n\t"
+        "v_mad_u64_u32 v[16:17], vcc, %[r8], s21, v[16:17]\n\t"
+        "v_mad_u64_u32 v[16:17], vcc, %[t4], 1, v[16:17]\n\t"
+        "v_and_b32 %[r4], s26, v16\n\t"
+        "v_lshrrev_b64 v[16:17], 29, v[16:17]\n\t"
+        "v_mad_u64_u32 v[16:17], vcc, %[d6], %[a8], v[16:17]\n\t"
+        "v_mad_u64_u32 v[16:17], vcc, %[a7], %[a7], v[16:17]\n\t"
+        "v_mad_u64_u32 v[16:17], vcc, %[r6], s24, v[16:17]\n\t"
+        "v_mad_u64_u32 v[16:17], vcc, %[r7], s23, v[16:17]\n\t"
+        "v_mad_u64_u32 v[16:17], vcc, %[r8], s22, v[16:17]\n\t"
+        "v_mad_u64_u32 v[16:17], vcc, %[t5], 1, v[16:17]\n\t"
+        "v_and_b32 %[r5], s26, v16\n\t"
+        "v_lshrrev_b64 v[16:17], 29, v[16:17]\n\t"
+        "v_mad_u64_u32 v[16:17], vcc, %[d7], %[a8], v[16:17]\n\t"
+        "v_mad_u64_u32 v[16:17], vcc, %[r7], s24, v[16:17]\n\t"
+        "v_mad_u64_u32 v[16:17], vcc, %[r8], s23, v[16:17]\n\t"
+        "v_mad_u64_u32 v[16:17], vcc, %[t6], 1, v[16:17]\n\t"
+        "v_and_b32 %[r6], s26, v16\n\t"
+        "v_lshrrev_b64 v[16:17], 29, v[16:17]\n\t"
+        "v_mad_u64_u32 v[16:17], vcc, %[a8], %[a8], v[16:17]\n\t"
+        "v_mad_u64_u32 v[16:17], vcc, %[r8], s24, v[16:17]\n\t"
+        "v_mad_u64_u32 v[16:17], vcc, %[t7], 1, v[16:17]\n\t"
+        "v_and_b32 %[r7], s26, v16\n\t"
+        "v_lshrrev_b64 v[16:17], 29, v[16:17]\n\t"
+        "v_add_u32 %[r8], v16, %[t8]\n\t"
+        : [r0] "=&v"(r[0]), [r1] "=&v"(r[1]), [r2] "=&v"(r[2]), [r3] "=&v"(r[3]), [r4] "=&v"(r[4]), [r5] "=&v"(r[5]), [r6] "=&v"(r[6]), [r7] "=&v"(r[7]), [r8] "=&v"(r[8]), [d0] "=&v"(d[0]), [d1] "=&v"(d[1]), [d2] "=&v"(d[2]), [d3] "=&v"(d[3]), [d4] "=&v"(d[4]), [d5] "=&v"(d[5]), [d6] "=&v"(d[6]), [d7] "=&v"(d[7])
+        : [a0] "v"(a[0]), [a1] "v"(a[1]), [a2] "v"(a[2]), [a3] "v"(a[3]), [a4] "v"(a[4]), [a5] "v"(a[5]), [a6] "v"(a[6]), [a7] "v"(a[7]), [a8] "v"(a[8]), [t0] "v"(t[0]), [t1] "v"(t[1]), [t2] "v"(t[2]), [t3] "v"(t[3]), [t4] "v"(t[4]), [t5] "v"(t[5]), [t6] "v"(t[6]), [t7] "v"(t[7]), [t8] "v"(t[8])
+        : "v16", "v17", "s16", "s17", "s18", "s19", "s20", "s21", "s22", "s23", "s24", "s25", "s26", "vcc");
+}
+__device__ __forceinline__ void mont_mulip29_fq(const uint32_t (&a)[9], uint32_t (&b)[9]) {
+    uint32_t m[9];
+    asm("s_mov_b32 s16, 0x187cfd47\n\t"
+        "s_mov_b32 s17, 0x010460b6\n\t"
+        "s_mov_b32 s18, 0x1c72a34f\n\t"
+        "s_mov_b32 s19, 0x02d522d0\n\t"
+        "s_mov_b32 s20, 0x1585d978\n\t"
+        "s_mov_b32 s21, 0x02db40c0\n\t"
+        "s_mov_b32 s22, 0x00a6e141\n\t"
+        "s_mov_b32 s23, 0x0e5c2634\n\t"
+        "s_mov_b32 s24, 0x0030644e\n\t"
+        "s_mov_b32 s25, 0x04866389\n\t"
+        "s_mov_b32 s26, 0x1fffffff\n\t"
+        "v_mad_u64_u32 v[16:17], vcc, %[a0], %[b0], 0\n\t"
+        "v_mul_lo_u32 %[m0], v16, s25\n\t"
+        "v_and_b32 %[m0], s26, %[m0]\n\t"
+        "v_mad_u64_u32 v[16:17], vcc, %[m0], s16, v[16:17]\n\t"
+        "v_lshrrev_b64 v[16:17], 29, v[16:17]\n\t"
+        "v_mad_u64_u32 v[16:17], vcc, %[a0], %[b1], v[16:17]\n\t"
+        "v_mad_u64_u32 v[16:17], vcc, %[a1], %[b0], v[16:17]\n\t"
+        "v_mad_u64_u32 v[16:17], vcc, %[m0], s17, v[16:17]\n\t"
+        "v_mul_lo_u32 %[m1], v16, s25\n\t"
+        "v_and_b32 %[m1], s26, %[m1]\n\t"
+        "v_mad_u64_u32 v[16:17], vcc, %[m1], s16, v[16:17]\n\t"
+        "v_lshrrev_b64 v[16:17], 29, v[16:17]\n\t"
+        "v_mad_u64_u32 v[16:17], vcc, %[a0], %[b2], v[16:17]\n\t"
+        "v_mad_u64_u32 v[16:17], vcc, %[a1], %[b1], v[16:17]\n\t"
+        "v_mad_u64_u32 v[16:17], vcc, %[a2], %[b0], v[16:17]\n\t"
+        "v_mad_u64_u32 v[16:17], vcc, %[m0], s18, v[16:17]\n\t"
+        "v_mad_u64_u32 v[16:17], vcc, %[m1], s17, v[16:17]\n\t"
+        "v_mul_lo_u32 %[m2], v16, s25\n\t"
+        "v_and_b32 %[m2], s26, %[m2]\n\t"
+        "v_mad_u64_u32 v[16:17], vcc, %[m2], s16, v[16:17]\n\t"
+        "v_lshrrev_b64 v[16:17], 29, v[16:17]\n\t"
+        "v_mad_u64_u32 v[16:17], vcc, %[a0], %[b3], v[16:17]\n\t"
+        "v_mad_u64_u32 v[16:17], vcc, %[a1], %[b2], v[16:17]\n\t"
+        "v_mad_u64_u32 v[16:17], vcc, %[a2], %[b1], v[16:17]\n\t"
+        "v_mad_u64_u32 v[16:17], vcc, %[a3], %[b0], v[16:17]\n\t"
+        "v_mad_u64_u32 v[16:17], vcc, %[m0], s19, v[16:17]\n\t"
+        "v_mad_u64_u32 v[16:17], vcc, %[m1], s18, v[16:17]\n\t"
+        "v_mad_u64_u32 v[16:17], vcc, %[m2], s17, v[16:17]\n\t"
+        "v_mul_lo_u32 %[m3], v16, s25\n\t"
+        "v_and_b32 %[m3], s26, %[m3]\n\t"
+        "v_mad_u64_u32 v[16:17], vcc, %[m3], s16, v[16:17]\n\t"
+        "v_lshrrev_b64 v[16:17], 29, v[16:17]\n\t"
+        "v_mad_u64_u32 v[16:17], vcc, %[a0], %[b4], v[16:17]\n\t"
+        "v_mad_u64_u32 v[16:17], vcc, %[a1], %[b3], v[16:17]\n\t"
+        "v_mad_u64_u32 v[16:17], vcc, %[a2], %[b2], v[16:17]\n\t"
+        "v_mad_u64_u32 v[16:17], vcc, %[a3], %[b1], v[16:17]\n\t"
+        "v_mad_u64_u32 v[16:17], vcc, %[a4], %[b0], v[16:17]\n\t"
+        "v_mad_u64_u32 v[16:17], vcc, %[m0], s20, v[16:17]\n\t"
+        "v_mad_u64_u32 v[16:17], vcc, %[m1], s19, v[16:17]\n\t"
+        "v_mad_u64_u32 v[16:17], vcc, %[m2], s18, v[16:17]\n\t"
+        "v_mad_u64_u32 v[16:17], vcc, %[m3], s17, v[16:17]\n\t"
+        "v_mul_lo_u32 %[m4], v16, s25\n\t"
+        "v_and_b32 %[m4], s26, %[m4]\n\t"
+        "v_mad_u64_u32 v[16:17], vcc, %[m4], s16, v[16:17]\n\t"
+        "v_lshrrev_b64 v[16:17], 29, v[16:17]\n\t"
+        "v_mad_u64_u32 v[16:17], vcc, %[a0], %[b5], v[16:17]\n\t"
+        "v_mad_u64_u32 v[16:17], vcc, %[a1], %[b4], v[16:17]\n\t"
+        "v_mad_u64_u32 v[16:17], vcc, %[a2], %[b3], v[16:17]\n\t"
+        "v_mad_u64_u32 v[16:17], vcc, %[a3], %[b2], v[16:17]\n\t"
+        "v_mad_u64_u32 v[16:17], vcc, %[a4], %[b1], v[16:17]\n\t"
+        "v_mad_u64_u32 v[16:17], vcc, %[a5], %[b0], v[16:17]\n\t"
+        "v_mad_u64_u32 v[16:17], vcc, %[m0], s21, v[16:17]\n\t"
+        "v_mad_u64_u32 v[16:17], vcc, %[m1], s20, v[16:17]\n\t"
+        "v_mad_u64_u32 v[16:17], vcc, %[m2], s19, v[16:17]\n\t"
+        "v_mad_u64_u32 v[16:17], vcc, %[m3], s18, v[16:17]\n\t"
+        "v_mad_u64_u32 v[16:17], vcc, %[m4], s17, v[16:17]\n\t"
+        "v_mul_lo_u32 %[m5], v16, s25\n\t"
+        "v_and_b32 %[m5], s26, %[m5]\n\t"
+        "v_mad_u64_u32 v[16:17], vcc, %[m5], s16, v[16:17]\n\t"
+        "v_lshrrev_b64 v[16:17], 29, v[16:17]\n\t"
+        "v_mad_u64_u32 v[16:17], vcc, %[a0], %[b6], v[16:17]\n\t"
+        "v_mad_u64_u32 v[16:17], vcc, %[a1], %[b5], v[16:17]\n\t"
+        "v_mad_u64_u32 v[16:17], vcc, %[a2], %[b4], v[16:17]\n\t"
+        "v_mad_u64_u32 v[16:17], vcc, %[a3], %[b3], v[16:17]\n\t"
+        "v_mad_u64_u32 v[16:17], vcc, %[a4], %[b2], v[16:17]\n\t"
+        "v_mad_u64_u32 v[16:17], vcc, %[a5], %[b1], v[16:17]\n\t"
+        "v_mad_u64_u32 v[16:17], vcc, %[a6], %[b0], v[16:17]\n\t"
+        "v_mad_u64_u32 v[16:17], vcc, %[m0], s22, v[16:17]\n\t"
+        "v_mad_u64_u32 v[16:17], vcc, %[m1], s21, v[16:17]\n\t"
+        "v_mad_u64_u32 v[16:17], vcc, %[m2], s20, v[16:17]\n\t"
+        "v_mad_u64_u32 v[16:17], vcc, %[m3], s19, v[16:17]\n\t"
+        "v_mad_u64_u32 v[16:17], vcc, %[m4], s18, v[16:17]\n\t"
+        "v_mad_u64_u32 v[16:17], vcc, %[m5], s17, v[16:17]\n\t"
+        "v_mul_lo_u32 %[m6], v16, s25\n\t"
+        "v_and_b32 %[m6], s26, %[m6]\n\t"
+        "v_mad_u64_u32 v[16:17], vcc, %[m6], s16, v[16:17]\n\t"
+        "v_lshrrev_b64 v[16:17], 29, v[16:17]\n\t"
+        "v_mad_u64_u32 v[16:17], vcc, %[a0], %[b7], v[16:17]\n\t"
+        "v_mad_u64_u32 v[16:17], vcc, %[a1], %[b6], v[16:17]\n\t"
+        "v_mad_u64_u32 v[16:17], vcc, %[a2], %[b5], v[16:17]\n\t"
+        "v_mad_u64_u32 v[16:17], vcc, %[a3], %[b4], v[16:17]\n\t"
+        "v_mad_u64_u32 v[16:17], vcc, %[a4], %[b3], v[16:17]\n\t"
+        "v_mad_u64_u32 v[16:17], vcc, %[a5], %[b2], v[16:17]\n\t"
+        "v_mad_u64_u32 v[16:17], vcc, %[a6], %[b1], v[16:17]\n\t"
+        "v_mad_u64_u32 v[16:17], vcc, %[a7], %[b0], v[16:17]\n\t"
+        "v_mad_u64_u32 v[16:17], vcc, %[m0], s23, v[16:17]\n\t"
+        "v_mad_u64_u32 v[16:17], vcc, %[m1], s22, v[16:17]\n\t"
+        "v_mad_u64_u32 v[16:17], vcc, %[m2], s21, v[16:17]\n\t"
+        "v_mad_u64_u32 v[16:17], vcc, %[m3], s20, v[16:17]\n\t"
+        "v_mad_u64_u32 v[16:17], vcc, %[m4], s19, v[16:17]\n\t"
+        "v_mad_u64_u32 v[16:17], vcc, %[m5], s18, v[16:17]\n\t"
+        "v_mad_u64_u32 v[16:17], vcc, %[m6], s17, v[16:17]\n\t"
+        "v_mul_lo_u32 %[m7], v16, s25\n\t"
+        "v_and_b32 %[m7], s26, %[m7]\n\t"
+        "v_mad_u64_u32 v[16:17], vcc, %[m7], s16, v[16:17]\n\t"
+        "v_lshrrev_b64 v[16:17], 29, v[16:17]\n\t"
+        "v_mad_u64_u32 v[16:17], vcc, %[a0], %[b8], v[16:17]\n\t"
+        "v_mad_u64_u32 v[16:17], vcc, %[a1], %[b7], v[16:17]\n\t"
+        "v_mad_u64_u32 v[16:17], vcc, %[a2], %[b6], v[16:17]\n\t"
+        "v_mad_u64_u32 v[16:17], vcc, %[a3], %[b5], v[16:17]\n\t"
+        "v_mad_u64_u32 v[16:17], vcc, %[a4], %[b4], v[16:17]\n\t"
+        "v_mad_u64_u32 v[16:17], vcc, %[a5], %[b3], v[16:17]\n\t"
+        "v_mad_u64_u32 v[16:17], vcc, %[a6], %[b2], v[16:17]\n\t"
+        "v_mad_u64_u32 v[16:17], vcc, %[a7], %[b1], v[16:17]\n\t"
+        "v_mad_u64_u32 v[16:17], vcc, %[a8], %[b0], v[16:17]\n\t"
+        "v_mad_u64_u32 v[16:17], vcc, %[m0], s24, v[16:17]\n\t"
+        "v_mad_u64_u32 v[16:17], vcc, %[m1], s23, v[16:17]\n\t"
+        "v_mad_u64_u32 v[16:17], vcc, %[m2], s22, v[16:17]\n\t"
+        "v_mad_u64_u32 v[16:17], vcc, %[m3], s21, v[16:17]\n\t"
+        "v_mad_u64_u32 v[16:17], vcc, %[m4], s20, v[16:17]\n\t"
+        "v_mad_u64_u32 v[16:17], vcc, %[m5], s19, v[16:17]\n\t"
+        "v_mad_u64_u32 v[16:17], vcc, %[m6], s18, v[16:17]\n\t"
+        "v_mad_u64_u32 v[16:17], vcc, %[m7], s17, v[16:17]\n\t"
+        "v_mul_lo_u32 %[m8], v16, s25\n\t"
+        "v_and_b32 %[m8], s26, %[m8]\n\t"
+        "v_mad_u64_u32 v[16:17], vcc, %[m8], s16, v[16:17]\n\t"
+        "v_lshrrev_b64 v[16:17], 29, v[16:17]\n\t"
+        "v_mad_u64_u32 v[16:17], vcc, %[a1], %[b8], v[16:17]\n\t"
+        "v_mad_u64_u32 v[16:17], vcc, %[a2], %[b7], v[16:17]\n\t"
+        "v_mad_u64_u32 v[16:17], vcc, %[a3], %[b6], v[16:17]\n\t"
+        "v_mad_u64_u32 v[16:17], vcc, %[a4], %[b5], v[16:17]\n\t"
+        "v_mad_u64_u32 v[16:17], vcc, %[a5], %[b4], v[16:17]\n\t"
+        "v_mad_u64_u32 v[16:17], vcc, %[a6], %[b3], v[16:17]\n\t"
+        "v_mad_u64_u32 v[16:17], vcc, %[a7], %[b2], v[16:17]\n\t"
+        "v_mad_u64_u32 v[16:17], vcc, %[a8], %[b1], v[16:17]\n\t"
+        "v_mad_u64_u32 v[16:17], vcc, %[m1], s24, v[16:17]\n\t"
+        "v_mad_u64_u32 v[16:17], vcc, %[m2], s23, v[16:17]\n\t"
+        "v_mad_u64_u32 v[16:17], vcc, %[m3], s22, v[16:17]\n\t"
+        "v_mad_u64_u32 v[16:17], vcc, %[m4], s21, v[16:17]\n\t"
+        "v_mad_u64_u32 v[16:17], vcc, %[m5], s20, v[16:17]\n\t"
+        "v_mad_u64_u32 v[16:17], vcc, %[m6], s19, v[16:17]\n\t"
+        "v_mad_u64_u32 v[16:17], vcc, %[m7], s18, v[16:17]\n\t"
+        "v_mad_u64_u32 v[16:17], vcc, %[m8], s17, v[16:17]\n\t"
+        "v_and_b32 %[b0], s26, v16\n\t"
+        "v_lshrrev_b64 v[16:17], 29, v[16:17]\n\t"
+        "v_mad_u64_u32 v[16:17], vcc, %[a2], %[b8], v[16:17]\n\t"
+        "v_mad_u64_u32 v[16:17], vcc, %[a3], %[b7], v[16:17]\n\t"
+        "v_mad_u64_u32 v[16:17], vcc, %[a4], %[b6], v[16:17]\n\t"
+        "v_mad_u64_u32 v[16:17], vcc, %[a5], %[b5], v[16:17]\n\t"
+        "v_mad_u64_u32 v[16:17], vcc, %[a6], %[b4], v[16:17]\n\t"
+        "v_mad_u64_u32 v[16:17], vcc, %[a7], %[b3], v[16:17]\n\t"
+        "v_mad_u64_u32 v[16:17], vcc, %[a8], %[b2], v[16:17]\n\t"
+        "v_mad_u64_u32 v[16:17], vcc, %[m2], s24, v[16:17]\n\t"
+        "v_mad_u64_u32 v[16:17], vcc, %[m3], s23, v[16:17]\n\t"
+        "v_mad_u64_u32 v[16:17], vcc, %[m4], s22, v[16:17]\n\t"
+        "v_mad_u64_u32 v[16:17], vcc, %[m5], s21, v[16:17]\n\t"
+        "v_mad_u64_u32 v[16:17], vcc, %[m6], s20, v[16:17]\n\t"
+        "v_mad_u64_u32 v[16:17], vcc, %[m7], s19, v[16:17]\n\t"
+        "v_mad_u64_u32 v[16:17], vcc, %[m8], s18, v[16:17]\n\t"
+        "v_and_b32 %[b1], s26, v16\n\t"
+        "v_lshrrev_b64 v[16:17], 29, v[16:17]\n\t"
+        "v_mad_u64_u32 v[16:17], vcc, %[a3], %[b8], v[16:17]\n\t"
+        "v_mad_u64_u32 v[16:17], vcc, %[a4], %[b7], v[16:17]\n\t"
+        "v_mad_u64_u32 v[16:17], vcc, %[a5], %[b6], v[16:17]\n\t"
+        "v_mad_u64_u32 v[16:17], vcc, %[a6], %[b5], v[16:17]\n\t"
+        "v_mad_u64_u32 v[16:17], vcc, %[a7], %[b4], v[16:17]\n\t"
+        "v_mad_u64_u32 v[16:17], vcc, %[a8], %[b3], v[16:17]\n\t"
+        "v_mad_u64_u32 v[16:17], vcc, %[m3], s24, v[16:17]\n\t"
+        "v_mad_u64_u32 v[16:17], vcc, %[m4], s23, v[16:17]\n\t"
+        "v_mad_u64_u32 v[16:17], vcc, %[m5], s22, v[16:17]\n\t"
+        "v_mad_u64_u32 v[16:17], vcc, %[m6], s21, v[16:17]\n\t"
+        "v_mad_u64_u32 v[16:17], vcc, %[m7], s20, v[16:17]\n\t"
+        "v_mad_u64_u32 v[16:17], vcc, %[m8], s19, v[16:17]\n\t"
+        "v_and_b32 %[b2], s26, v16\n\t"
+        "v_lshrrev_b64 v[16:17], 29, v[16:17]\n\t"
+        "v_mad_u64_u32 v[16:17], vcc, %[a4], %[b8], v[16:17]\n\t"
+        "v_mad_u64_u32 v[16:17], vcc, %[a5], %[b7], v[16:17]\n\t"
+        "v_mad_u64_u32 v[16:17], vcc, %[a6], %[b6], v[16:17]\n\t"
+        "v_mad_u64_u32 v[16:17], vcc, %[a7], %[b5], v[16:17]\n\t"
+        "v_mad_u64_u32 v[16:17], vcc, %[a8], %[b4], v[16:17]\n\t"
+        "v_mad_u64_u32 v[16:17], vcc, %[m4], s24, v[16:17]\n\t"
+        "v_mad_u64_u32 v[16:17], vcc, %[m5], s23, v[16:17]\n\t"
+        "v_mad_u64_u32 v[16:17], vcc, %[m6], s22, v[16:17]\n\t"
+        "v_mad_u64_u32 v[16:17], vcc, %[m7], s21, v[16:17]\n\t"
+        "v_mad_u64_u32 v[16:17], vcc, %[m8], s20, v[16:17]\n\t"
+        "v_and_b32 %[b3], s26, v16\n\t"
+        "v_lshrrev_b64 v[16:17], 29, v[16:17]\n\t"
+        "v_mad_u64_u32 v[16:17], vcc, %[a5], %[b8], v[16:17]\n\t"
+        "v_mad_u64_u32 v[16:17], vcc, %[a6], %[b7], v[16:17]\n\t"
+        "v_mad_u64_u32 v[16:17], vcc, %[a7], %[b6], v[16:17]\n\t"
+        "v_mad_u64_u32 v[16:17], vcc, %[a8], %[b5], v[16:17]\n\t"
+        "v_mad_u64_u32 v[16:17], vcc, %[m5], s24, v[16:17]\n\t"
+        "v_mad_u64_u32 v[16:17], vcc, %[m6], s23, v[16:17]\n\t"
+        "v_mad_u64_u32 v[16:17], vcc, %[m7], s22, v[16:17]\n\t"
+        "v_mad_u64_u32 v[16:17], vcc, %[m8], s21, v[16:17]\n\t"
+        "v_and_b32 %[b4], s26, v16\n\t"
+        "v_lshrrev_b64 v[16:17], 29, v[16:17]\n\t"
+        "v_mad_u64_u32 v[16:17], vcc, %[a6], %[b8], v[16:17]\n\t"
+        "v_mad_u64_u32 v[16:17], vcc, %[a7], %[b7], v[16:17]\n\t"
+        "v_mad_u64_u32 v[16:17], vcc, %[a8], %[b6], v[16:17]\n\t"
+        "v_mad_u64_u32 v[16:17], vcc, %[m6], s24, v[16:17]\n\t"
+        "v_mad_u64_u32 v[16:17], vcc, %[m7], s23, v[16:17]\n\t"
+        "v_mad_u64_u32 v[16:17], vcc, %[m8], s22, v[16:17]\n\t"
+        "v_and_b32 %[b5], s26, v16\n\t"
+        "v_lshrrev_b64 v[16:17], 29, v[16:17]\n\t"
+        "v_mad_u64_u32 v[16:17], vcc, %[a7], %[b8], v[16:17]\n\t"
+        "v_mad_u64_u32 v[16:17], vcc, %[a8], %[b7], v[16:17]\n\t"
+        "v_mad_u64_u32 v[16:17], vcc, %[m7], s24, v[16:17]\n\t"
+        "v_mad_u64_u32 v[16:17], vcc, %[m8], s23, v[16:17]\n\t"
+        "v_and_b32 %[b6], s26, v16\n\t"
+        "v_lshrrev_b64 v[16:17], 29, v[16:17]\n\t"
+        "v_mad_u64_u32 v[16:17], vcc, %[a8], %[b8], v[16:17]\n\t"
+        "v_mad_u64_u32 v[16:17], vcc, %[m8], s24, v[16:17]\n\t"
+        "v_and_b32 %[b7], s26, v16\n\t"
+        "v_alignbit_b32 %[b8], v17, v16, 29\n\t"
+        : [b0] "+&v"(b[0]), [b1] "+&v"(b[1]), [b2] "+&v"(b[2]), [b3] "+&v"(b[3]), [b4] "+&v"(b[4]), [b5] "+&v"(b[5]), [b6] "+&v"(b[6]), [b7] "+&v"(b[7]), [b8] "+&v"(b[8]), [m0] "=&v"(m[0]), [m1] "=&v"(m[1]), [m2] "=&v"(m[2]), [m3] "=&v"(m[3]), [m4] "=&v"(m[4]), [m5] "=&v"(m[5]), [m6] "=&v"(m[6]), [m7] "=&v"(m[7]), [m8] "=&v"(m[8])
+        : [a0] "v"(a[0]), [a1] "v"(a[1]), [a2] "v"(a[2]), [a3] "v"(a[3]), [a4] "v"(a[4]), [a5] "v"(a[5]), [a6] "v"(a[6]), [a7] "v"(a[7]), [a8] "v"(a[8])
+        : "v16", "v17", "s16", "s17", "s18", "s19", "s20", "s21", "s22", "s23", "s24", "s25", "s26", "vcc");
+}
+}
diff --git a/ezkl_amd/csrc/msm.hip b/ezkl_amd/csrc/msm.hip
--- a/ezkl_amd/csrc/msm.hip
+++ b/ezkl_amd/csrc/msm.hip
@@ -563,7 +563,7 @@
     uint32_t vn = k0 + 1 < k1 ? vals[k0 + 1] : 0u;
     for (uint32_t k = k0; k < k1; k++) {
         if (k == bin_end) {
-            if (started_before) st_g1x29(head + t, acc); else st_g1x29(buckets + b, acc);
+            st_g1x29(started_before ? head + t : buckets + b, acc);
             acc.zz = Fq29::zero();
             started_before = false;
             b++;
@@ -583,10 +583,14 @@
             }
             end_next = offsets[b + 2 <= nb ? b + 2 : nb];
         }
-        const MsmRec cur = nxt;
+        g1a29_t cur = g1a29_unpack(nxt.p);
+        const bool cur_neg = nxt.neg;
+        asm volatile("" : "+v"(cur.x.v[0]), "+v"(cur.x.v[1]), "+v"(cur.x.v[2]), "+v"(cur.x.v[3]), "+v"(cur.x.v[4]), "+v"(cur.x.v[5]), "+v"(cur.x.v[6]),
+                          "+v"(cur.x.v[7]), "+v"(cur.x.v[8]), "+v"(cur.y.v[0]), "+v"(cur.y.v[1]), "+v"(cur.y.v[2]), "+v"(cur.y.v[3]), "+v"(cur.y.v[4]),
+                          "+v"(cur.y.v[5]), "+v"(cur.y.v[6]), "+v"(cur.y.v[7]), "+v"(cur.y.v[8]) : : "memory");
         nxt = msm_fetch(tab, vn);
         vn = k + 2 < k1 ? vals[k + 2] : 0u;
-        acc = g1x29_add_mixed(acc, g1a29_unpack(cur.p), cur.neg);
+        g1x29_acc_mixed(acc, cur, cur_neg);
     }
     if (k1 == bin_end) {
         if (started_before) st_g1x29(head + t, acc); else st_g1x29(buckets + b, acc);
diff --git a/ezkl_amd/csrc/ubench.hip b/ezkl_amd/csrc/ubench.hip
--- a/ezkl_amd/csrc/ubench.hip
+++ b/ezkl_amd/csrc/ubench.hip
@@ -202,6 +202,31 @@
     uint32_t x = 0;
     for (int i = 0; i < 9; i++) x ^= a[i] ^ b[i] ^ c[i] ^ d[i];
     io[t * 8] = x;
+}
+__global__ __launch_bounds__(256) void ub_fused29_check_kernel(const uint32_t* io, uint32_t* mismatches) {
+    size_t t = (size_t)blockIdx.x * blockDim.x + threadIdx.x;
+    uint32_t a[9], b[9], c[9], r[9], want[9];
+    for (int i = 0; i < 9; i++) {
+        uint32_t x = (io[t * 8 + (i & 7)] + (uint32_t)t) * 2654435761u + i;
+        a[i] = x & 0x3fffffffu; b[i] = (x >> 3) & 0x1fffffffu; c[i] = (x * 7u) & 0x7fffffffu;
+    }
+    a[8] &= 0x3ffffffu; b[8] &= 0x3ffffffu; c[8] &= 0x3ffffffu;
+    bool bad = false;
+    mont_muladd29_fq(a, b, c, r);
+    mont_mul29_ref_fq(a, b, want);
+    for (int i = 0; i < 9; i++) want[i] += c[i];
+    for (int i = 0; i < 8; i++) { want[i + 1] += want[i] >> 29; want[i] &= 0x1fffffffu; }
+    for (int i = 0; i < 9; i++) bad |= r[i] != want[i];
+    mont_sqradd29_fq(a, c, r);
+    mont_mul29_ref_fq(a, a, want);
+    for (int i = 0; i < 9; i++) want[i] += c[i];
+    for (int i = 0; i < 8; i++) { want[i + 1] += want[i] >> 29; want[i] &= 0x1fffffffu; }
+    for (int i = 0; i < 9; i++) bad |= r[i] != want[i];
+    mont_mul29_ref_fq(a, b, want);
+    for (int i = 0; i < 9; i++) r[i] = b[i];
+    mont_mulip29_fq(a, r);
+    for (int i = 0; i < 9; i++) bad |= r[i] != want[i];
+    if (bad) atomicAdd(mismatches, 1u);
 }
 
 template <int MODE>
@@ -548,6 +573,24 @@
         *out = chk ? (double)hm : 4.0 * iters * (double)nthreads / (ms * 1e-3);
         return EZKL_OK;
     }
+    if (!strcmp(which, "fused29_check")) {
+        void* buf = nullptr;
+        uint32_t* mis = nullptr;
+        const int threads = 256, blocks = c->num_cus * 4;
+        const size_t nthreads = (size_t)blocks * threads;
+        EZ_HIP(hipMalloc(&buf, nthreads * 32));
+        EZ_HIP(hipMalloc((void**)&mis, 4));
+        EZ_HIP(hipMemsetAsync(buf, 0x5b, nthreads * 32, st));
+        EZ_HIP(hipMemsetAsync(mis, 0, 4, st));
+        hipLaunchKernelGGL(ub_fused29_check_kernel, dim3(blocks), dim3(threads), 0, st, (const uint32_t*)buf, mis);
+        EZ_HIP(hipStreamSynchronize(st));
+        uint32_t hm = 0;
+        EZ_HIP(hipMemcpy(&hm, mis, 4, hipMemcpyDeviceToHost));
+        EZ_HIP(hipFree(buf));
+        EZ_HIP(hipFree(mis));
+        *out = (double)hm;
+        return EZKL_OK;
+    }
     if (!strncmp(which, "modmul29", 8)) {
         void* buf = nullptr;
         uint32_t* mis = nullptr;
```

Result: no change. 806.1 million pts/s, median of 5 (+0.7%).
